# CVlab315/Domain-Adaptative-Hand-Pose-Estimation

Measured on AMD Instinct MI355X. Metric: images/sec (unique source+target images per A+B+C training iteration, 2*B*N/t_iter), higher is better.
Workload: dtype bf16; 1 GPU; RHD->H3D domain-adaptation iteration (steps A+B+C), resnet50 + 3-deconv neck + main head + 3 adversarial multiscale-fusion heads, 256x256, batch 64 source + 64 target per GPU, random init, synthetic batches; arch=resnet50, image_size=256, per_gpu_batch=64, global_batch=64, parallelism=dp1, hip_graphs=True, gradient_exchange=none (one rank)

## Files before the change

domain-adaptative-hand-pose-estimation_amd/csrc/bn.hip:

```cpp
#include "common.h"
#include "fp8_common.h"
#include <stdlib.h>
#include <string>

struct BnPlan { int cpr, TX, TY, colgroups, nslices, rows_per_slice; };

static BnPlan bn_plan(long rows, int C, int CH, long slice_cap_override = 0) {
  BnPlan p; p.cpr = C / CH;
  p.TX = p.cpr < 256 ? p.cpr : 256;
  while (256 % p.TX) --p.TX;
  p.TY = 256 / p.TX;
  p.colgroups = cdiv(p.cpr, p.TX);
  long want = rows / ((long)p.TY * 8); if (want < 1) want = 1;
  static const long slice_cap = getenv("MI355_BN_SLICES") ? atol(getenv("MI355_BN_SLICES")) : 1024;
  long cap = (slice_cap_override ? slice_cap_override : slice_cap) / p.colgroups; if (cap < 1) cap = 1;
  if (want > cap) want = cap;
  long rps = (rows + want - 1) / want; rps = ((rps + p.TY - 1) / p.TY) * p.TY;
  p.rows_per_slice = (int)rps; p.nslices = (int)((rows + rps - 1) / rps);
  return p;
}

static long bwd_slices() { static const long v = getenv("MI355_BN_BWD_SLICES") ? atol(getenv("MI355_BN_BWD_SLICES")) : 768; return v; }
extern "C" size_t mi355_bn_workspace(long rows, int C) {
  int ns = 0;
// ... 96 lines not shown
  }
  if (running_mean && repeats > 0) running_mean[c] = rm;
  if (running_var && repeats > 0) running_var[c] = rv;
  const float sc = g * invstd;
  scale_shift[c] = sc; scale_shift[C + c] = b - mean * sc;
}

__global__ __launch_bounds__(256) void bn_finalize_wide_kernel(const float* __restrict__ partial, int nslices, int C, const float* __restrict__ gamma,
                                        const float* __restrict__ beta, float* running_mean, float* running_var,
                                        int64_t* nbt, float* save_mean, float* save_invstd, float* scale_shift, float eps,
                                        float momentum, int repeats) {
  __shared__ float red[4][3];
  const int c = blockIdx.x, t = threadIdx.x, lane = t & 63, wave = t >> 6;
  if (c == 0 && t == 0 && nbt) *nbt += repeats;
  const float g = gamma[c], b = beta[c];
  float rm = running_mean ? running_mean[c] : 0.f, rv = running_var ? running_var[c] : 0.f;
  float n = 0.f, mean = 0.f, m2 = 0.f;
  for (int base = 0; base < nslices; base += 2048) {
    float qn[8], qm[8], qv[8];
#pragma unroll
    for (int j = 0; j < 8; ++j) {
      const int s = base + t + 256 * j;
      if (s < nslices) { const float* q = partial + ((size_t)s * C + c) * 3; qn[j] = q[0]; qm[j] = q[1]; qv[j] = q[2]; }
      else { qn[j] = 0.f; qm[j] = 0.f; qv[j] = 0.f; }
    }
#pragma unroll
    for (int j = 0; j < 8; ++j) chan_combine(n, mean, m2, qn[j], qm[j], qv[j]);
  }
#pragma unroll
  for (int o = 32; o > 0; o >>= 1) {
    const float nb = __shfl_down(n, o, 64), mb = __shfl_down(mean, o, 64), vb = __shfl_down(m2, o, 64);
    chan_combine(n, mean, m2, nb, mb, vb);
  }
  if (lane == 0) { red[wave][0] = n; red[wave][1] = mean; red[wave][2] = m2; }
  __syncthreads();
  if (t != 0) return;
  n = red[0][0]; mean = red[0][1]; m2 = red[0][2];
#pragma unroll
  for (int w = 1; w < 4; ++w) chan_combine(n, mean, m2, red[w][0], red[w][1], red[w][2]);
  const float var = m2 / n;
  const float invstd = 1.0f / sqrtf(var + eps);
  save_mean[c] = mean; save_invstd[c] = invstd;
  const float uvar = n > 1.f ? m2 / (n - 1.f) : var;
  for (int r = 0; r < repeats; ++r) {
    rm = (1.f - momentum) * rm + momentum * mean;
    rv = (1.f - momentum) * rv + momentum * uvar;
  }
  if (running_mean && repeats > 0) running_mean[c] = rm;
  if (running_var && repeats > 0) running_var[c] = rv;
  const float sc = g * invstd;
  scale_shift[c] = sc; scale_shift[C + c] = b - mean * sc;
}

template <typename T, bool EVAL, bool Q8 = false>
__global__ __launch_bounds__(256) void bn_apply_kernel(const T* __restrict__ x, const T* __restrict__ res, T* __restrict__ y,
                                                        const float* __restrict__ scale_shift, const float* __restrict__ gamma,
                                                        const float* __restrict__ beta, const float* __restrict__ rm,
                                                        const float* __restrict__ rv, float eps, long rows, int C, int TX, int relu,
                                                        unsigned char* __restrict__ mask, unsigned char* __restrict__ q8 = nullptr,
                                                        float* __restrict__ q8_state = nullptr) {
  constexpr int CH = Chunk<T>::N;
  static_assert(!Q8 || CH == 8, "fp8 side output: bf16 activations only");
  const int TY = 256 / TX;
  const int tx = threadIdx.x % TX, ty = threadIdx.x / TX;
  const int chunk = blockIdx.x * TX + tx;
  const bool colok = chunk * CH < C;
  if (!colok && !Q8) return;
  const int cpr = C / CH;
  float sc[CH], sh[CH];
#pragma unroll
  for (int e = 0; e < CH; ++e) {
    const int c = chunk * CH + e;
    if (!colok) { sc[e] = 0.f; sh[e] = 0.f; }
    else if (EVAL) { sc[e] = gamma[c] / sqrtf(rv[c] + eps); sh[e] = beta[c] - rm[c] * sc[e]; }
    else { sc[e] = scale_shift[c]; sh[e] = scale_shift[C + c]; }
  }
  float qscale = 0.f, amax = 0.f; unsigned seen = 0;
  if constexpr (Q8) { qscale = q8_state[0]; seen = fp8_amax_seen(q8_state); }
  for (long r = (long)blockIdx.y * TY + ty; colok && r < rows; r += (long)gridDim.y * TY) {
    const size_t off = (size_t)r * C + (size_t)chunk * CH;
    float v[CH]; Chunk<T>::load(x + off, v);
#pragma unroll
    for (int e = 0; e < CH; ++e) v[e] = v[e] * sc[e] + sh[e];
    if (res) { float w[CH]; Chunk<T>::load(res + off, w);
#pragma unroll
      for (int e = 0; e < CH; ++e) v[e] += w[e]; }
    if (mask) {
      unsigned m = 0;
#pragma unroll
      for (int e = 0; e < CH; ++e) m |= (v[e] > 0.f ? 1u : 0u) << e;
      mask[(size_t)r * cpr + chunk] = (unsigned char)m;
    }
    if (relu) {
#pragma unroll
      for (int e = 0; e < CH; ++e) v[e] = v[e] < 0.f ? 0.f : v[e]; }
    Chunk<T>::store(y + off, v);
    if constexpr (Q8) {
      float w[8];
#pragma unroll
      for (int e = 0; e < 8; ++e) { w[e] = (float)(T)v[e]; amax = fmaxf(amax, fabsf(w[e])); }
      const uint2 o = pack8_fp8<false>(w, qscale);
      const unsigned nx = __shfl_down(o.x, 1, 64), ny = __shfl_down(o.y, 1, 64);
      if ((tx & 1) == 0) *reinterpret_cast<uint4*>(q8 + off) = make_uint4(o.x, o.y, nx, ny);
    }
  }
  if constexpr (Q8) fp8_record_amax(amax, q8_state, seen);
}

template <typename T, bool XHAT, int RELU>
__global__ __launch_bounds__(256) void bn_bwd_reduce_kernel(const T* __restrict__ dy, const T* __restrict__ x, const T* __restrict__ y,
                                                             const float* __restrict__ mean, const float* __restrict__ invstd,
                                                             const float* __restrict__ gamma, const float* __restrict__ beta,
                                                             float* __restrict__ partial, long rows, int C, int TX, int rows_per_slice,
                                                             const unsigned char* __restrict__ mask) {
  constexpr int relu = RELU;
  constexpr int CH = Chunk<T>::N;
  __shared__ float sh[256 * CH * 2];
  const int cpr = C / CH;
  const int TY = 256 / TX;
  const int tx = threadIdx.x % TX, ty = threadIdx.x / TX;
  const int chunk = blockIdx.x * TX + tx;
  const bool colok = chunk * CH < C;
  const long r0 = (long)blockIdx.y * rows_per_slice;
  long r1 = r0 + rows_per_slice; if (r1 > rows) r1 = rows;
  float s1[CH], s2[CH], mu[CH], is[CH], sc[CH], sft[CH];
#pragma unroll
  for (int e = 0; e < CH; ++e) { s1[e] = 0.f; s2[e] = 0.f; mu[e] = 0.f; is[e] = 0.f; sc[e] = 0.f; sft[e] = 0.f; }
  if (colok && XHAT) {
#pragma unroll
    for (int e = 0; e < CH; ++e) { mu[e] = mean[chunk * CH + e]; is[e] = invstd[chunk * CH + e]; }
    if (relu == 2) {
#pragma unroll
      for (int e = 0; e < CH; ++e) { sc[e] = gamma[chunk * CH + e] * is[e]; sft[e] = beta[chunk * CH + e] - mu[e] * sc[e]; }
    }
  }
  auto fold = [&](float (&g)[CH], const float (&v)[CH], const float (&o)[CH], unsigned mb) {
    if (relu == 1) {
#pragma unroll
      for (int e = 0; e < CH; ++e) g[e] = o[e] > 0.f ? g[e] : 0.f; }
    else if (relu == 3) {
#pragma unroll
      for (int e = 0; e < CH; ++e) g[e] = ((mb >> e) & 1u) ? g[e] : 0.f; }
    if (XHAT) {
      if (relu == 2) {
#pragma unroll
        for (int e = 0; e < CH; ++e) g[e] = (v[e] * sc[e] + sft[e]) > 0.f ? g[e] : 0.f; }
#pragma unroll
      for (int e = 0; e < CH; ++e) { s1[e] += g[e]; s2[e] += g[e] * ((v[e] - mu[e]) * is[e]); }
    } else {
#pragma unroll
      for (int e = 0; e < CH; ++e) s1[e] += g[e];
    }
  };
  if (colok) {
    long r = r0 + ty;
    for (; r + TY < r1; r += 2 * TY) {
      const size_t off0 = (size_t)r * C + (size_t)chunk * CH, off1 = off0 + (size_t)TY * C;
      float g0[CH], v0[CH], o0[CH], g1[CH], v1[CH], o1[CH];
      Chunk<T>::load(dy + off0, g0); Chunk<T>::load(dy + off1, g1);
      if (XHAT) { Chunk<T>::load(x + off0, v0); Chunk<T>::load(x + off1, v1); }
      if (relu == 1) { Chunk<T>::load(y + off0, o0); Chunk<T>::load(y + off1, o1); }
      unsigned m0 = 0, m1 = 0;
      if (relu == 3) { m0 = mask[(size_t)r * cpr + chunk]; m1 = mask[(size_t)(r + TY) * cpr + chunk]; }
      fold(g0, v0, o0, m0); fold(g1, v1, o1, m1);
    }
    if (r < r1) {
      const size_t off = (size_t)r * C + (size_t)chunk * CH;
      float g[CH], v[CH], o[CH]; Chunk<T>::load(dy + off, g);
      if (XHAT) Chunk<T>::load(x + off, v);
      if (relu == 1) Chunk<T>::load(y + off, o);
      fold(g, v, o, relu == 3 ? (unsigned)mask[(size_t)r * cpr + chunk] : 0u);
    }
  }
#pragma unroll
  for (int e = 0; e < CH; ++e) { sh[threadIdx.x * CH + e] = s1[e]; sh[256 * CH + threadIdx.x * CH + e] = s2[e]; }
  __syncthreads();
  if (ty == 0 && colok) {
    for (int j = 1; j < TY; ++j) {
      const int o = j * TX + tx;
#pragma unroll
      for (int e = 0; e < CH; ++e) { s1[e] += sh[o * CH + e]; s2[e] += sh[256 * CH + o * CH + e]; }
    }
    float* out = partial + ((size_t)blockIdx.y * C + (size_t)chunk * CH) * 2;
#pragma unroll
    for (int e = 0; e < CH; ++e) { out[e * 2] = s1[e]; out[e * 2 + 1] = s2[e]; }
  }
}

__global__ __launch_bounds__(256) void bn_bwd_finalize_kernel(const float* __restrict__ partial, int nslices, int C, float inv_rows,
                                       const float* __restrict__ gamma, const float* __restrict__ invstd, float* dgamma,
                                       float* dbeta, int accumulate, float* coeff) {
  const int lane = threadIdx.x & 63;
  const int c = blockIdx.x * 4 + (threadIdx.x >> 6);
  if (c >= C) return;
  const float g = coeff ? gamma[c] : 0.f, is = coeff ? invstd[c] : 0.f;
  const float db0 = (accumulate && dbeta) ? dbeta[c] : 0.f, dg0 = (accumulate && dgamma) ? dgamma[c] : 0.f;
  float s1 = 0.f, s2 = 0.f;
  for (int base = 0; base < nslices; base += 1024) {
    float q1[16], q2[16];
#pragma unroll
    for (int j = 0; j < 16; ++j) {
      const int s = base + lane + 64 * j;
      if (s < nslices) { const float* q = partial + ((size_t)s * C + c) * 2; q1[j] = q[0]; q2[j] = q[1]; } else { q1[j] = 0.f; q2[j] = 0.f; }
    }
#pragma unroll
    for (int j = 0; j < 16; ++j) { s1 += q1[j]; s2 += q2[j]; }
  }
#pragma unroll
  for (int o = 32; o > 0; o >>= 1) { s1 += __shfl_down(s1, o, 64); s2 += __shfl_down(s2, o, 64); }
  if (lane != 0) return;
  if (dbeta) dbeta[c] = db0 + s1;
  if (dgamma) dgamma[c] = dg0 + s2;
  if (coeff) { coeff[c] = g * is; coeff[C + c] = s1 * inv_rows; coeff[2 * C + c] = s2 * inv_rows; }
}

template <typename T, int RELU, bool Q8 = false>
__global__ __launch_bounds__(256) void bn_bwd_apply_kernel(const T* __restrict__ dy, const T* __restrict__ x, const T* __restrict__ y,
                                                            const float* __restrict__ mean, const float* __restrict__ invstd,
                                                            const float* __restrict__ coeff, const float* __restrict__ beta,
                                                            T* __restrict__ dx, T* __restrict__ dres,
                                                            long rows, int C, int TX, const unsigned char* __restrict__ mask,
                                                            unsigned char* __restrict__ q8 = nullptr, float* __restrict__ q8_state = nullptr) {
  constexpr int CH = Chunk<T>::N;
  constexpr int relu = RELU;
  static_assert(!Q8 || CH == 8, "fp8 side output: bf16 gradients only");
  const int TY = 256 / TX;
  const int tx = threadIdx.x % TX, ty = threadIdx.x / TX;
  const int chunk = blockIdx.x * TX + tx;
  const bool colok = chunk * CH < C;
  if (!colok && !Q8) return;
  const int cpr = C / CH;
  float k0[CH], k1[CH], k2[CH], mu[CH], is[CH], sh[CH];
#pragma unroll
  for (int e = 0; e < CH; ++e) {
    const int c = colok ? chunk * CH + e : 0;
    k0[e] = coeff[c]; k1[e] = coeff[C + c]; k2[e] = coeff[2 * C + c]; mu[e] = mean[c]; is[e] = invstd[c];
    sh[e] = (relu == 2) ? beta[c] - mu[e] * k0[e] : 0.f;
  }
  float qscale = 0.f, amax = 0.f; unsigned seen = 0;
  if constexpr (Q8) { qscale = q8_state[0]; seen = fp8_amax_seen(q8_state); }
  auto finish = [&](size_t off, float (&g)[CH], float (&v)[CH], const float (&o)[CH], unsigned mb) {
    if (relu == 1) {
#pragma unroll
      for (int e = 0; e < CH; ++e) g[e] = o[e] > 0.f ? g[e] : 0.f; }
    else if (relu == 3) {
#pragma unroll
      for (int e = 0; e < CH; ++e) g[e] = ((mb >> e) & 1u) ? g[e] : 0.f; }
    else if (relu == 2) {
#pragma unroll
      for (int e = 0; e < CH; ++e) g[e] = (v[e] * k0[e] + sh[e]) > 0.f ? g[e] : 0.f; }
    if (dres) Chunk<T>::store(dres + off, g);
#pragma unroll
    for (int e = 0; e < CH; ++e) v[e] = k0[e] * (g[e] - k1[e] - (v[e] - mu[e]) * is[e] * k2[e]);
    Chunk<T>::store(dx + off, v);
    if constexpr (Q8) {
      float w[8];
#pragma unroll
      for (int e = 0; e < 8; ++e) { w[e] = (float)(T)v[e]; amax = fmaxf(amax, fabsf(w[e])); }
      const uint2 o = pack8_fp8<true>(w, qscale);
      const unsigned nx = __shfl_down(o.x, 1, 64), ny = __shfl_down(o.y, 1, 64);
      if ((tx & 1) == 0) *reinterpret_cast<uint4*>(q8 + off) = make_uint4(o.x, o.y, nx, ny);
    }
  };
  const long stride = (long)gridDim.y * TY;
  long r = colok ? (long)blockIdx.y * TY + ty : rows;
  for (; r + stride < rows; r += 2 * stride) {
    const size_t off0 = (size_t)r * C + (size_t)chunk * CH, off1 = (size_t)(r + stride) * C + (size_t)chunk * CH;
    float g0[CH], v0[CH], o0[CH], g1[CH], v1[CH], o1[CH];
    Chunk<T>::load(dy + off0, g0); Chunk<T>::load(x + off0, v0);
    Chunk<T>::load(dy + off1, g1); Chunk<T>::load(x + off1, v1);
    if (relu == 1) { Chunk<T>::load(y + off0, o0); Chunk<T>::load(y + off1, o1); }
    unsigned m0 = 0, m1 = 0;
    if (relu == 3) { m0 = mask[(size_t)r * cpr + chunk]; m1 = mask[(size_t)(r + stride) * cpr + chunk]; }
    finish(off0, g0, v0, o0, m0); finish(off1, g1, v1, o1, m1);
  }
  if (r < rows) {
    const size_t off = (size_t)r * C + (size_t)chunk * CH;
    float g[CH], v[CH], o[CH]; Chunk<T>::load(dy + off, g); Chunk<T>::load(x + off, v);
    if (relu == 1) Chunk<T>::load(y + off, o);
    finish(off, g, v, o, relu == 3 ? (unsigned)mask[(size_t)r * cpr + chunk] : 0u);
  }
  if constexpr (Q8) fp8_record_amax(amax, q8_state, seen);
}

struct BnResArgs {
  const void* dy; const void* x; const float* mean; const float* invstd; const float* gamma; const float* beta;
  void* dx; void* dres; float* dgamma; float* dbeta; const unsigned char* mask;
  long rows; int C, G, R, rpb, keep, accumulate; float inv_rows;
  unsigned spin_limit;
};
#define BN_RES_MAXBLK 256
#define BN_RES_GRAN 128
#define BN_RES_SW 8
#define BN_RES_KR 0
#define BN_RES_NT 1024
__device__ unsigned long long bn_res_gran[BN_RES_MAXBLK * BN_RES_GRAN];
__device__ unsigned bn_res_done[2][BN_RES_MAXBLK + 1];
__device__ unsigned bn_res_err[4];
static_assert(BN_RES_MAXBLK == 256, "a launch adds 256 to its completion count and the tag keeps 8 bits of n - 1");

#ifdef BN_RES_STAMPS
__device__ unsigned long long bn_res_stamp[BN_RES_MAXBLK * 8];
#define BN_STAMP(k) do { __builtin_amdgcn_sched_barrier(0); if (t == 0) bn_res_stamp[blockIdx.x * 8 + (k)] = wall_clock64(); \
                         __builtin_amdgcn_sched_barrier(0); } while (0)
extern "C" int mi355_bn_resident_stamps(unsigned long long* out) {
  return hipMemcpyFromSymbol(out, HIP_SYMBOL(bn_res_stamp), sizeof(unsigned long long) * BN_RES_MAXBLK * 8) == hipSuccess ? MI355_OK : MI355_ELAUNCH;
}
#else
#define BN_STAMP(k) do {} while (0)
#endif

template <typename T, int RELU, int KR, int NT>
__global__ __launch_bounds__(NT) void bn_bwd_resident_kernel(BnResArgs p) {
  constexpr int CH = Chunk<T>::N, GC = 8 * CH, RL = NT / 8, NW = NT / 64, NL = NT / (GC * 2), RR = KR * RL;
  extern __shared__ __attribute__((aligned(16))) char smem[];
  const int t = threadIdx.x, tx = t & 7, ty = t >> 3, lane = t & 63, wave = t >> 6;
  const int g = blockIdx.x % p.G, r = blockIdx.x / p.G;
  const long row0 = (long)r * p.rpb;
  long row1 = row0 + p.rpb; if (row1 > p.rows) row1 = p.rows;
  const int nrows = row1 > row0 ? (int)(row1 - row0) : 0;
  const int keep = p.keep;
  uint4* xs = reinterpret_cast<uint4*>(smem);
  uint4* ds = xs + (size_t)keep * 8;
  float* red = reinterpret_cast<float*>(ds + (size_t)keep * 8);
  float* grp = red + NW * GC * 2;
  float* tot = grp + NL * GC * 2;
  int* bar_ok = reinterpret_cast<int*>(tot + GC * 2);
  const T* __restrict__ X = reinterpret_cast<const T*>(p.x);
  const T* __restrict__ DY = reinterpret_cast<const T*>(p.dy);
  const int C = p.C, cpr = C / CH, c0 = g * GC + tx * CH, chunk = c0 / CH;
  BN_STAMP(0);
  const unsigned nblk = (unsigned)(p.G * p.R);
  unsigned* done = &bn_res_done[GC * 2 == BN_RES_GRAN ? 1 : 0][nblk];
  const unsigned tag = 0x80000000u | (GC * 2 == BN_RES_GRAN ? 0x40000000u : 0u) | ((nblk - 1u) << 22) |
                       ((__hip_atomic_load(done, __ATOMIC_RELAXED, __HIP_MEMORY_SCOPE_AGENT) >> 8) & 0x3fffffu);
  float mu[CH], is[CH], sc[CH], sft[CH], s1[CH], s2[CH];
#pragma unroll
  for (int e = 0; e < CH; ++e) {
    mu[e] = p.mean[c0 + e]; is[e] = p.invstd[c0 + e]; s1[e] = 0.f; s2[e] = 0.f;
    sc[e] = p.gamma[c0 + e] * is[e];
    sft[e] = (RELU == 2) ? p.beta[c0 + e] - mu[e] * sc[e] : 0.f;
  }
  auto mask_of = [&](int lr) -> unsigned { return (RELU == 3) ? (unsigned)p.mask[(size_t)(row0 + lr) * cpr + chunk] : 0u; };
  auto fold = [&](const uint4& qxv, const uint4& qdv, unsigned mb) {
    float v[CH], gq[CH]; Chunk<T>::unpack(qxv, v); Chunk<T>::unpack(qdv, gq);
#pragma unroll
    for (int e = 0; e < CH; ++e) {
      if (RELU == 2) gq[e] = (v[e] * sc[e] + sft[e]) > 0.f ? gq[e] : 0.f;
      if (RELU == 3) gq[e] = ((mb >> e) & 1u) ? gq[e] : 0.f;
      s1[e] += gq[e]; s2[e] += gq[e] * ((v[e] - mu[e]) * is[e]);
    }
  };
  uint4 rx[KR > 0 ? KR : 1], rd[KR > 0 ? KR : 1];
  {
    unsigned mk[KR > 0 ? KR : 1];
#pragma unroll
    for (int k = 0; k < KR; ++k) {
      const int lr = ty + k * RL;
      rx[k] = make_uint4(0, 0, 0, 0); rd[k] = make_uint4(0, 0, 0, 0); mk[k] = 0;
      if (lr < nrows) {
        const size_t off = (size_t)(row0 + lr) * C + c0;
        rx[k] = *reinterpret_cast<const uint4*>(X + off); rd[k] = *reinterpret_cast<const uint4*>(DY + off); mk[k] = mask_of(lr);
      }
    }
#pragma unroll
    for (int k = 0; k < KR; ++k)
      if (ty + k * RL < nrows) fold(rx[k], rd[k], mk[k]);
  }
  for (int base = RR + ty; base < nrows; base += 4 * RL) {
    uint4 qx[4], qd[4]; unsigned mk[4];
#pragma unroll
    for (int k = 0; k < 4; ++k) {
      const int lr = base + k * RL;
      if (lr < nrows) {
        const size_t off = (size_t)(row0 + lr) * C + c0;
        qx[k] = *reinterpret_cast<const uint4*>(X + off); qd[k] = *reinterpret_cast<const uint4*>(DY + off); mk[k] = mask_of(lr);
      }
    }
#pragma unroll
    for (int k = 0; k < 4; ++k) {
      const int lr = base + k * RL, li = lr - RR;
      if (lr < nrows) {
        if (li < keep) { xs[li * 8 + tx] = qx[k]; ds[li * 8 + tx] = qd[k]; }
        fold(qx[k], qd[k], mk[k]);
      }
    }
  }
#pragma unroll
  for (int o = 8; o < 64; o <<= 1) {
#pragma unroll
    for (int e = 0; e < CH; ++e) { s1[e] += __shfl_xor(s1[e], o, 64); s2[e] += __shfl_xor(s2[e], o, 64); }
  }
  if (lane < 8) {
#pragma unroll
    for (int e = 0; e < CH; ++e) { red[(wave * GC + tx * CH + e) * 2] = s1[e]; red[(wave * GC + tx * CH + e) * 2 + 1] = s2[e]; }
  }
  if (t == 0) *bar_ok = 1;
  BN_STAMP(1);
  __syncthreads();
  if (t < GC * 2) {
    float a = 0.f;
#pragma unroll
    for (int w = 0; w < NW; ++w) a += red[w * GC * 2 + t];
    __hip_atomic_store(bn_res_gran + (size_t)blockIdx.x * BN_RES_GRAN + t, ((unsigned long long)tag << 32) | __float_as_uint(a),
                       __ATOMIC_RELAXED, __HIP_MEMORY_SCOPE_AGENT);
  }
  BN_STAMP(2);
  {
    const int i = t % (GC * 2), s = t / (GC * 2);
    const __amdgpu_buffer_rsrc_t rs = __builtin_amdgcn_make_buffer_rsrc(bn_res_gran, 0, (unsigned)sizeof(bn_res_gran), 0x00020000);
    float a = 0.f;
    bool arrived = true;
    for (int rr0 = s; rr0 < p.R && arrived; rr0 += BN_RES_SW * NL) {
      float q[BN_RES_SW];
      for (unsigned spins = 0;;) {
        asm volatile("" ::: "memory");
        bool ok = true;
#pragma unroll
        for (int k = 0; k < BN_RES_SW; ++k) {
          const int rr = rr0 + k * NL;
          const auto gv = __builtin_amdgcn_raw_buffer_load_b64(rs, rr < p.R ? ((rr * p.G + g) * BN_RES_GRAN + i) * 8 : 0x7ffffff0, 0, 16);
          q[k] = rr < p.R ? __uint_as_float(gv[0]) : 0.f; ok &= (gv[1] == tag) | (rr >= p.R);
        }
        if (__all(ok)) break;
        if (++spins > p.spin_limit) { arrived = false; break; }
        __builtin_amdgcn_s_sleep(4);
      }
#pragma unroll
      for (int k = 0; k < BN_RES_SW; ++k) a += q[k];
    }
    grp[s * GC * 2 + i] = a;
    if (!arrived && lane == 0) *bar_ok = 0;
  }
  __syncthreads();
  const bool exchanged = *bar_ok != 0;
  if (!exchanged && t == 0) __hip_atomic_fetch_add(bn_res_err, 1u, __ATOMIC_RELAXED, __HIP_MEMORY_SCOPE_AGENT);
  if (t < GC * 2) {
    float a = 0.f;
#pragma unroll
    for (int s = 0; s < NL; ++s) a += grp[s * GC * 2 + t];
    tot[t] = a;
  }
  __syncthreads();
  BN_STAMP(3);
  float k1[CH], k2[CH];
#pragma unroll
  for (int e = 0; e < CH; ++e) {
    s1[e] = tot[(tx * CH + e) * 2]; s2[e] = tot[(tx * CH + e) * 2 + 1];
    if (!exchanged) { s1[e] = __builtin_nanf(""); s2[e] = __builtin_nanf(""); }
    k1[e] = s1[e] * p.inv_rows; k2[e] = s2[e] * p.inv_rows;
  }
  if (r == 0 && ty == 0) {
#pragma unroll
    for (int e = 0; e < CH; ++e) {
      if (p.dbeta) p.dbeta[c0 + e] = (p.accumulate ? p.dbeta[c0 + e] : 0.f) + s1[e];
      if (p.dgamma) p.dgamma[c0 + e] = (p.accumulate ? p.dgamma[c0 + e] : 0.f) + s2[e];
    }
  }
  T* __restrict__ DX = reinterpret_cast<T*>(p.dx);
  T* __restrict__ DR = reinterpret_cast<T*>(p.dres);
#ifdef BN_RES_STAMPS
  bool stamped = false;
#endif
  auto finish = [&](int lr, const uint4& qxv, const uint4& qdv, unsigned mb) {
    const size_t off = (size_t)(row0 + lr) * C + c0;
    float v[CH], gq[CH]; Chunk<T>::unpack(qxv, v); Chunk<T>::unpack(qdv, gq);
#pragma unroll
    for (int e = 0; e < CH; ++e) {
      if (RELU == 2) gq[e] = (v[e] * sc[e] + sft[e]) > 0.f ? gq[e] : 0.f;
      if (RELU == 3) gq[e] = ((mb >> e) & 1u) ? gq[e] : 0.f;
    }
    if (DR) Chunk<T>::store(DR + off, gq);
#pragma unroll
    for (int e = 0; e < CH; ++e) v[e] = sc[e] * (gq[e] - k1[e] - (v[e] - mu[e]) * is[e] * k2[e]);
    Chunk<T>::store(DX + off, v);
#ifdef BN_RES_STAMPS
    if (!stamped) { BN_STAMP(4); stamped = true; }
#endif
  };
#pragma unroll
  for (int k = 0; k < KR; ++k) {
    const int lr = ty + k * RL;
    if (lr < nrows) finish(lr, rx[k], rd[k], mask_of(lr));
  }
  const int nlds = nrows - RR < keep ? nrows - RR : keep;
  for (int li = ty; li < nlds; li += RL) finish(RR + li, xs[li * 8 + tx], ds[li * 8 + tx], mask_of(RR + li));
  for (int base = RR + keep + ty; base < nrows; base += 4 * RL) {
    uint4 qx[4], qd[4]; unsigned mk[4];
#pragma unroll
    for (int k = 0; k < 4; ++k) {
      const int lr = base + k * RL;
      if (lr < nrows) {
        const size_t off = (size_t)(row0 + lr) * C + c0;
        qx[k] = *reinterpret_cast<const uint4*>(X + off); qd[k] = *reinterpret_cast<const uint4*>(DY + off); mk[k] = mask_of(lr);
      }
    }
#pragma unroll
    for (int k = 0; k < 4; ++k) {
      const int lr = base + k * RL;
      if (lr < nrows) finish(lr, qx[k], qd[k], mk[k]);
    }
  }
  if (t == 0) __hip_atomic_fetch_add(done, blockIdx.x == 0 ? (unsigned)BN_RES_MAXBLK + 1u - nblk : 1u, __ATOMIC_RELAXED, __HIP_MEMORY_SCOPE_AGENT);
  BN_STAMP(5);
}

template <typename T>
__global__ __launch_bounds__(256) void apply_relu_mask_kernel(T* __restrict__ g, const unsigned char* __restrict__ mask, size_t nchunks) {
  constexpr int CH = Chunk<T>::N;
  for (size_t i = (size_t)blockIdx.x * 256 + threadIdx.x; i < nchunks; i += (size_t)gridDim.x * 256) {
    float v[CH]; Chunk<T>::load(g + i * CH, v);
    const unsigned mb = mask[i];
#pragma unroll
    for (int e = 0; e < CH; ++e) v[e] = ((mb >> e) & 1u) ? v[e] : 0.f;
    Chunk<T>::store(g + i * CH, v);
  }
}

template <typename T>
__global__ __launch_bounds__(256) void bn_relu_maxpool_kernel(const T* __restrict__ x, const float* __restrict__ scale_shift, T* __restrict__ y,
                                                               uint8_t* __restrict__ arg, int N, int H, int W, int C, int Ho, int Wo) {
  constexpr int CH = Chunk<T>::N;
  const int cpr = C / CH;
  const unsigned total = (unsigned)N * Ho * Wo * cpr;
  for (unsigned id = blockIdx.x * 256u + threadIdx.x; id < total; id += gridDim.x * 256u) {
    const int ch = (int)(id % (unsigned)cpr); unsigned r = id / (unsigned)cpr;
    const int ox = (int)(r % (unsigned)Wo); r /= (unsigned)Wo; const int oy = (int)(r % (unsigned)Ho); const int n = (int)(r / (unsigned)Ho);
    float sc[CH], sh[CH], best[CH]; int bi[CH]; bool first = true;
#pragma unroll
    for (int e = 0; e < CH; ++e) { sc[e] = scale_shift[ch * CH + e]; sh[e] = scale_shift[C + ch * CH + e]; best[e] = -INFINITY; bi[e] = 0; }
    for (int kh = 0; kh < 3; ++kh) {
      const int iy = 2 * oy - 1 + kh; if (iy < 0 || iy >= H) continue;
      for (int kw = 0; kw < 3; ++kw) {
        const int ix = 2 * ox - 1 + kw; if (ix < 0 || ix >= W) continue;
        float v[CH]; Chunk<T>::load(x + (((size_t)n * H + iy) * W + ix) * C + (size_t)ch * CH, v);
        const int code = kh * 3 + kw;
#pragma unroll
        for (int e = 0; e < CH; ++e) {
          float u = v[e] * sc[e] + sh[e];
          u = u < 0.f ? 0.f : u;
          u = (float)(T)u;
          if (first) bi[e] = code;
          if (u > best[e] || u != u) { best[e] = u; bi[e] = code; }
        }
        first = false;
      }
    }
    const size_t o = (((size_t)n * Ho + oy) * Wo + ox) * C + (size_t)ch * CH;
    Chunk<T>::store(y + o, best);
    store_bytes<CH>(arg + o, bi);
  }
// ... 20 lines not shown
  return 0;
}
static int bn_check(long rows, int C, int dtype, int* CH) {
  if (dtype != MI355_F32 && dtype != MI355_BF16) MI_FAIL(MI355_EINVAL, "bn: bad dtype");
  *CH = dtype == MI355_BF16 ? 8 : 4;
  if (rows < 1 || C < 1 || C % *CH) MI_FAIL(MI355_EINVAL, "bn: C=%d must be a positive multiple of %d (rows=%ld)", C, *CH, rows);
  return 0;
}
static dim3 apply_grid(const BnPlan& p, long rows, bool backward = false) {
  long gy = rows / ((long)p.TY * 4); if (gy < 1) gy = 1;
  static const long fwd_cap = getenv("MI355_BN_APPLY_CAP") ? atol(getenv("MI355_BN_APPLY_CAP")) : 2048;
  static const long bwd_cap = getenv("MI355_BN_BWD_CAP") ? atol(getenv("MI355_BN_BWD_CAP")) : 1024;
  long cap = (backward ? bwd_cap : fwd_cap) / p.colgroups; if (cap < 1) cap = 1;
  if (gy > cap) gy = cap;
  return dim3(p.colgroups, (unsigned)gy);
}

extern "C" int mi355_bn_train_fwd(const void* x, const void* residual, void* y, const float* gamma, const float* beta,
                                  float* running_mean, float* running_var, int64_t* nbt, float* save_mean, float* save_invstd,
                                  long rows, int C, float eps, float momentum, int stat_updates, int relu, int dtype, void* ws,
                                  size_t ws_bytes, void* relu_mask, void* q8_out, float* q8_state, void* stream) {
  int CH; if (int e = bn_check(rows, C, dtype, &CH)) return e;
  if (int e = q8_check(q8_out, q8_state, dtype, C)) return e;
  unsigned char* mk = reinterpret_cast<unsigned char*>(relu_mask);
  if (stat_updates < 0 || stat_updates > 8) MI_FAIL(MI355_EINVAL, "bn_train_fwd: stat_updates=%d", stat_updates);
  if (!ws || ws_bytes < mi355_bn_workspace(rows, C)) MI_FAIL(MI355_EWORKSPACE, "bn_train_fwd: workspace too small");
  hipStream_t st = as_stream(stream);
  BnPlan p = bn_plan(rows, C, CH);
  float* partial = reinterpret_cast<float*>(ws);
  float* ss = partial + (size_t)p.nslices * C * 3;
  dim3 g(p.colgroups, p.nslices);
  const double nb = (double)rows * C * (dtype == MI355_BF16 ? 2.0 : 4.0);
  char lab[96];
  if (prof_on()) snprintf(lab, sizeof(lab), "rows%ld C%d%s%s", rows, C, relu ? " relu" : "", residual ? " +res" : "");
  {
    ProfScope ps(st, 0.0, nb, 1, prof_on() ? (std::string("bn_stats ") + lab).c_str() : nullptr);
    if (dtype == MI355_BF16) hipLaunchKernelGGL(bn_stats_kernel<bf16_t>, g, dim3(256), 0, st, (const bf16_t*)x, partial, rows, C, p.TX, p.rows_per_slice);
    else hipLaunchKernelGGL(bn_stats_kernel<float>, g, dim3(256), 0, st, (const float*)x, partial, rows, C, p.TX, p.rows_per_slice);
  }
  {
    ProfScope ps(st, 0.0, 12.0 * p.nslices * C, 1, prof_on() ? (std::string("bn_finalize ") + lab).c_str() : nullptr);
    hipLaunchKernelGGL(bn_finalize_kernel, dim3(cdiv(C, 4)), dim3(256), 0, st, partial, p.nslices, C, gamma, beta, running_mean, running_var, nbt, save_mean, save_invstd, ss, eps, momentum, stat_updates);
  }
  dim3 ga = apply_grid(p, rows);
  const float* nf = nullptr;
  ProfScope ps(st, 0.0, nb * (residual ? 3 : 2), 1, prof_on() ? (std::string("bn_apply ") + lab).c_str() : nullptr);
  if (q8_out) hipLaunchKernelGGL((bn_apply_kernel<bf16_t, false, true>), ga, dim3(256), 0, st, (const bf16_t*)x, (const bf16_t*)residual, (bf16_t*)y, (const float*)ss, nf, nf, nf, nf, eps, rows, C, p.TX, relu, mk, (unsigned char*)q8_out, q8_state);
  else if (dtype == MI355_BF16) hipLaunchKernelGGL((bn_apply_kernel<bf16_t, false>), ga, dim3(256), 0, st, (const bf16_t*)x, (const bf16_t*)residual, (bf16_t*)y, (const float*)ss, nf, nf, nf, nf, eps, rows, C, p.TX, relu, mk);
  else hipLaunchKernelGGL((bn_apply_kernel<float, false>), ga, dim3(256), 0, st, (const float*)x, (const float*)residual, (float*)y, (const float*)ss, nf, nf, nf, nf, eps, rows, C, p.TX, relu, mk);
  MI_CHECK_LAUNCH("bn_train_fwd");
  return MI355_OK;
}

extern "C" int mi355_bn_train_fwd_partials(const void* x, const void* residual, void* y, const float* gamma, const float* beta,
                                           float* running_mean, float* running_var, int64_t* nbt, float* save_mean,
                                           float* save_invstd, long rows, int C, float eps, float momentum, int stat_updates,
                                           int relu, int dtype, const float* partial, int nslices, float* scale_shift,
                                           void* relu_mask, void* q8_out, float* q8_state, void* stream) {
  int CH; if (int e = bn_check(rows, C, dtype, &CH)) return e;
  if (int e = q8_check(q8_out, q8_state, dtype, C)) return e;
  unsigned char* mk = reinterpret_cast<unsigned char*>(relu_mask);
  if (stat_updates < 0 || stat_updates > 8) MI_FAIL(MI355_EINVAL, "bn_train_fwd_partials: stat_updates=%d", stat_updates);
  if (!partial || nslices < 1 || !scale_shift) MI_FAIL(MI355_EINVAL, "bn_train_fwd_partials: partial / scale_shift missing");
  hipStream_t st = as_stream(stream);
  BnPlan p = bn_plan(rows, C, CH);
  static const int wide_min = getenv("MI355_BN_WIDE_FINALIZE") ? atoi(getenv("MI355_BN_WIDE_FINALIZE")) : 512;
  const double nb = (double)rows * C * (dtype == MI355_BF16 ? 2.0 : 4.0);
  char lab[96];
  if (prof_on()) snprintf(lab, sizeof(lab), "rows%ld C%d ns%d%s%s", rows, C, nslices, relu ? " relu" : "", residual ? " +res" : "");
  {
    ProfScope ps(st, 0.0, 12.0 * nslices * C, 1, prof_on() ? (std::string("bn_finalize ") + lab).c_str() : nullptr);
    if (nslices >= wide_min) hipLaunchKernelGGL(bn_finalize_wide_kernel, dim3(C), dim3(256), 0, st, partial, nslices, C, gamma, beta, running_mean, running_var, nbt, save_mean, save_invstd, scale_shift, eps, momentum, stat_updates);
    else hipLaunchKernelGGL(bn_finalize_kernel, dim3(cdiv(C, 4)), dim3(256), 0, st, partial, nslices, C, gamma, beta, running_mean, running_var, nbt, save_mean, save_invstd, scale_shift, eps, momentum, stat_updates);
  }
  dim3 ga = apply_grid(p, rows);
  const float* nf = nullptr;
  ProfScope ps(st, 0.0, nb * (residual ? 3 : 2), 1, prof_on() ? (std::string("bn_apply ") + lab).c_str() : nullptr);
  if (q8_out) hipLaunchKernelGGL((bn_apply_kernel<bf16_t, false, true>), ga, dim3(256), 0, st, (const bf16_t*)x, (const bf16_t*)residual, (bf16_t*)y, (const float*)scale_shift, nf, nf, nf, nf, eps, rows, C, p.TX, relu, mk, (unsigned char*)q8_out, q8_state);
  else if (dtype == MI355_BF16) hipLaunchKernelGGL((bn_apply_kernel<bf16_t, false>), ga, dim3(256), 0, st, (const bf16_t*)x, (const bf16_t*)residual, (bf16_t*)y, (const float*)scale_shift, nf, nf, nf, nf, eps, rows, C, p.TX, relu, mk);
  else hipLaunchKernelGGL((bn_apply_kernel<float, false>), ga, dim3(256), 0, st, (const float*)x, (const float*)residual, (float*)y, (const float*)scale_shift, nf, nf, nf, nf, eps, rows, C, p.TX, relu, mk);
  MI_CHECK_LAUNCH("bn_train_fwd_partials");
  return MI355_OK;
}

extern "C" int mi355_bn_relu_maxpool_fwd_partials(const void* x, void* y_pool, uint8_t* argidx, const float* gamma, const float* beta,
                                                  float* running_mean, float* running_var, int64_t* nbt, float* save_mean,
                                                  float* save_invstd, int N, int H, int W, int C, float eps, float momentum,
                                                  int stat_updates, int dtype, const float* partial, int nslices, float* scale_shift,
                                                  void* stream) {
  const long rows = (long)N * H * W;
  int CH; if (int e = bn_check(rows, C, dtype, &CH)) return e;
  if (stat_updates < 0 || stat_updates > 8) MI_FAIL(MI355_EINVAL, "bn_relu_maxpool_fwd_partials: stat_updates=%d", stat_updates);
  if (!partial || nslices < 1 || !scale_shift || !argidx || !y_pool) MI_FAIL(MI355_EINVAL, "bn_relu_maxpool_fwd_partials: null argument");
  if (rows * (C / CH) >= (1L << 31)) MI_FAIL(MI355_EINVAL, "bn_relu_maxpool_fwd_partials: %ld chunks exceed the kernel's 32-bit index: split the batch", rows * (C / CH));
  hipStream_t st = as_stream(stream);
  static const int wide_min = getenv("MI355_BN_WIDE_FINALIZE") ? atoi(getenv("MI355_BN_WIDE_FINALIZE")) : 512;
  char lab[96];
  if (prof_on()) snprintf(lab, sizeof(lab), "rows%ld C%d ns%d", rows, C, nslices);
  {
    ProfScope ps(st, 0.0, 12.0 * nslices * C, 1, prof_on() ? (std::string("bn_finalize ") + lab).c_str() : nullptr);
    if (nslices >= wide_min) hipLaunchKernelGGL(bn_finalize_wide_kernel, dim3(C), dim3(256), 0, st, partial, nslices, C, gamma, beta, running_mean, running_var, nbt, save_mean, save_invstd, scale_shift, eps, momentum, stat_updates);
    else hipLaunchKernelGGL(bn_finalize_kernel, dim3(cdiv(C, 4)), dim3(256), 0, st, partial, nslices, C, gamma, beta, running_mean, running_var, nbt, save_mean, save_invstd, scale_shift, eps, momentum, stat_updates);
  }
  const int Ho = (H + 2 - 3) / 2 + 1, Wo = (W + 2 - 3) / 2 + 1;
  const long total = (long)N * Ho * Wo * (C / CH);
  int grid = (int)((total + 255) / 256); if (grid > 8192) grid = 8192;
  ProfScope ps(st, 0.0, (double)rows * C * (dtype == MI355_BF16 ? 2.0 : 4.0) * 1.25, 1, prof_on() ? (std::string("bn_relu_maxpool ") + lab).c_str() : nullptr);
  if (dtype == MI355_BF16) hipLaunchKernelGGL(bn_relu_maxpool_kernel<bf16_t>, dim3(grid), dim3(256), 0, st, (const bf16_t*)x, (const float*)scale_shift, (bf16_t*)y_pool, argidx, N, H, W, C, Ho, Wo);
  else hipLaunchKernelGGL(bn_relu_maxpool_kernel<float>, dim3(grid), dim3(256), 0, st, (const float*)x, (const float*)scale_shift, (float*)y_pool, argidx, N, H, W, C, Ho, Wo);
  MI_CHECK_LAUNCH("bn_relu_maxpool_fwd_partials");
  return MI355_OK;
}

extern "C" int mi355_bn_eval_fwd(const void* x, const void* residual, void* y, const float* gamma, const float* beta,
                                 const float* running_mean, const float* running_var, long rows, int C, float eps, int relu,
                                 int dtype, void* stream) {
  int CH; if (int e = bn_check(rows, C, dtype, &CH)) return e;
  hipStream_t st = as_stream(stream);
  BnPlan p = bn_plan(rows, C, CH);
  dim3 ga = apply_grid(p, rows);
  const float* nf = nullptr;
  if (dtype == MI355_BF16) hipLaunchKernelGGL((bn_apply_kernel<bf16_t, true>), ga, dim3(256), 0, st, (const bf16_t*)x, (const bf16_t*)residual, (bf16_t*)y, nf, gamma, beta, running_mean, running_var, eps, rows, C, p.TX, relu, (unsigned char*)nullptr);
  else hipLaunchKernelGGL((bn_apply_kernel<float, true>), ga, dim3(256), 0, st, (const float*)x, (const float*)residual, (float*)y, nf, gamma, beta, running_mean, running_var, eps, rows, C, p.TX, relu, (unsigned char*)nullptr);
  MI_CHECK_LAUNCH("bn_eval_fwd");
  return MI355_OK;
}

struct BnResPlan { int G, R, rpb, keep; size_t lds, max_lds; };
static int g_bn_resident = -1;
extern "C" int mi355_bn_set_resident(int on) {
  const int prev = g_bn_resident;
  g_bn_resident = on < 0 ? -1 : (on ? 1 : 0);
  return prev;
}
static bool bn_resident_plan(long rows, int C, int CH, BnResPlan* q) {
  static const bool env_on = !(getenv("MI355_BN_RESIDENT") && atoi(getenv("MI355_BN_RESIDENT")) == 0);
  if (g_bn_resident == 0 || (g_bn_resident < 0 && !env_on)) return false;
  static int ncu = 0; static size_t max_lds = 0;
  if (!ncu) {
    int dev = 0, v = 0;
    if (hipGetDevice(&dev) != hipSuccess) return false;
    if (hipDeviceGetAttribute(&v, hipDeviceAttributeMaxSharedMemoryPerBlock, dev) != hipSuccess) return false;
    max_lds = (size_t)v;
    if (hipDeviceGetAttribute(&v, hipDeviceAttributeMultiprocessorCount, dev) != hipSuccess) return false;
    ncu = v > BN_RES_MAXBLK ? BN_RES_MAXBLK : v;
  }
  const int GC = 8 * CH;
  if (C % GC) return false;
  static const long min_bytes = getenv("MI355_BN_RESIDENT_MIN") ? atol(getenv("MI355_BN_RESIDENT_MIN")) : 0;
  if (rows * C * (16 / CH) < min_bytes) return false;
  q->G = C / GC;
  if (q->G > ncu) return false;
  long R = ncu / q->G; if (R > rows) R = rows;
  q->rpb = (int)((rows + R - 1) / R);
  q->R = (int)((rows + q->rpb - 1) / q->rpb);
  static const long max_bytes = getenv("MI355_BN_RESIDENT_MAX") ? atol(getenv("MI355_BN_RESIDENT_MAX")) : (1L << 62);
  if (rows * C * (16 / CH) > max_bytes) return false;
  const size_t scratch = (size_t)(BN_RES_NT / 64 * GC * 2 + BN_RES_NT + GC * 2 + 4) * sizeof(float);
  long keep = (long)((max_lds - scratch) / 256);
  const long reg_rows = (long)BN_RES_KR * (BN_RES_NT / 8);
  const long rest = q->rpb > reg_rows ? q->rpb - reg_rows : 0;
  if (keep > rest) keep = rest;
  q->keep = (int)keep;
  q->lds = (size_t)keep * 256 + scratch;
  q->max_lds = max_lds;
  return (size_t)q->G * q->R <= (size_t)ncu && q->G * q->R <= BN_RES_MAXBLK;
}
static unsigned g_bn_res_spin = 1u << 19;
extern "C" int mi355_bn_resident_set_spin_limit(unsigned limit) {
  g_bn_res_spin = limit ? limit : (1u << 19);
  return MI355_OK;
}
#define BN_RES_NOT_RESIDENT 1
template <typename T, int RELU>
static int bn_resident_launch(const BnResArgs& a, size_t lds, size_t max_lds, hipStream_t st) {
  static int fits = -1;
  auto kern = bn_bwd_resident_kernel<T, RELU, BN_RES_KR, BN_RES_NT>;
  if (fits < 0) {
    if (hipFuncSetAttribute(reinterpret_cast<const void*>(kern), hipFuncAttributeMaxDynamicSharedMemorySize, (int)max_lds) != hipSuccess)
      MI_FAIL(MI355_ELAUNCH, "bn_bwd: cannot raise the dynamic LDS limit to %zu bytes", max_lds);
    int nb = 0;
    if (hipOccupancyMaxActiveBlocksPerMultiprocessor(&nb, kern, BN_RES_NT, max_lds) != hipSuccess) nb = 0;
    fits = nb >= 1 ? 1 : 0;
  }
  if (!fits) return BN_RES_NOT_RESIDENT;
  hipLaunchKernelGGL(kern, dim3(a.G * a.R), dim3(BN_RES_NT), lds, st, a);
  return MI355_OK;
}
extern "C" int mi355_bn_resident_timeouts(unsigned* out) {
  unsigned v[4] = {0, 0, 0, 0};
  if (!out) MI_FAIL(MI355_EINVAL, "bn_resident_timeouts: out is null");
  if (hipMemcpyFromSymbol(v, HIP_SYMBOL(bn_res_err), sizeof(v)) != hipSuccess) MI_FAIL(MI355_ELAUNCH, "bn_resident_timeouts: copy failed");
  *out = v[0];
  return MI355_OK;
}
extern "C" int mi355_bn_resident_reset(void) {
  static const unsigned zdone[2][BN_RES_MAXBLK + 1] = {{0}};
  static const unsigned zerr[4] = {0, 0, 0, 0};
  void* gran = nullptr;
  if (hipDeviceSynchronize() != hipSuccess) MI_FAIL(MI355_ELAUNCH, "bn_resident_reset: device synchronize failed");
  if (hipGetSymbolAddress(&gran, HIP_SYMBOL(bn_res_gran)) != hipSuccess || hipMemset(gran, 0, sizeof(bn_res_gran)) != hipSuccess ||
      hipMemcpyToSymbol(HIP_SYMBOL(bn_res_done), zdone, sizeof(zdone)) != hipSuccess ||
      hipMemcpyToSymbol(HIP_SYMBOL(bn_res_err), zerr, sizeof(zerr)) != hipSuccess) MI_FAIL(MI355_ELAUNCH, "bn_resident_reset: copy failed");
  if (hipDeviceSynchronize() != hipSuccess) MI_FAIL(MI355_ELAUNCH, "bn_resident_reset: device synchronize failed");
  return MI355_OK;
}

static void launch_bwd_apply(int dtype, int relu, dim3 ga, hipStream_t st, const void* dy, const void* x, const void* y, const float* save_mean,
                             const float* save_invstd, const float* coeff, const float* beta, void* dx, void* dresidual, long rows, int C,
                             int TX, const unsigned char* mk, void* q8_out, float* q8_state) {
#define MI_APP(T, R) hipLaunchKernelGGL((bn_bwd_apply_kernel<T, R>), ga, dim3(256), 0, st, (const T*)dy, (const T*)x, (const T*)y, save_mean, save_invstd, coeff, beta, (T*)dx, (T*)dresidual, rows, C, TX, mk)
#define MI_APQ(R) hipLaunchKernelGGL((bn_bwd_apply_kernel<bf16_t, R, true>), ga, dim3(256), 0, st, (const bf16_t*)dy, (const bf16_t*)x, (const bf16_t*)y, save_mean, save_invstd, coeff, beta, (bf16_t*)dx, (bf16_t*)dresidual, rows, C, TX, mk, (unsigned char*)q8_out, q8_state)
#define MI_APP4(T) do { if (relu == 0) MI_APP(T, 0); else if (relu == 1) MI_APP(T, 1); else if (relu == 2) MI_APP(T, 2); else MI_APP(T, 3); } while (0)
  if (q8_out) { if (relu == 0) MI_APQ(0); else if (relu == 1) MI_APQ(1); else if (relu == 2) MI_APQ(2); else MI_APQ(3); }
  else if (dtype == MI355_BF16) MI_APP4(bf16_t); else MI_APP4(float);
#undef MI_APP4
#undef MI_APQ
#undef MI_APP
}

extern "C" int mi355_bn_bwd(const void* dy, const void* x, const void* y, const float* gamma, const float* beta, const float* save_mean,
                            const float* save_invstd, void* dx, void* dresidual, float* dgamma, float* dbeta, int accumulate,
                            long rows, int C, int relu, int dtype, void* ws, size_t ws_bytes, const void* relu_mask, void* q8_out,
                            float* q8_state, void* stream) {
  int CH; if (int e = bn_check(rows, C, dtype, &CH)) return e;
  if (!ws || ws_bytes < mi355_bn_workspace(rows, C)) MI_FAIL(MI355_EWORKSPACE, "bn_bwd: workspace too small");
  const unsigned char* mk = reinterpret_cast<const unsigned char*>(relu_mask);
  if (relu) relu = mk ? 3 : (y ? 1 : 2);
  if (relu == 2 && !beta) MI_FAIL(MI355_EINVAL, "bn_bwd: relu without y needs beta");
  hipStream_t st = as_stream(stream);
  BnResPlan rp;
  if (relu != 1 && !q8_out && bn_resident_plan(rows, C, CH, &rp)) {
    BnResArgs a;
    a.dy = dy; a.x = x; a.mean = save_mean; a.invstd = save_invstd; a.gamma = gamma; a.beta = beta; a.dx = dx; a.dres = dresidual;
    a.dgamma = dgamma; a.dbeta = dbeta; a.mask = mk; a.rows = rows; a.C = C;
    a.G = rp.G; a.R = rp.R; a.rpb = rp.rpb; a.keep = rp.keep; a.accumulate = accumulate; a.inv_rows = 1.0f / (float)rows;
    a.spin_limit = g_bn_res_spin;
    int e;
    char lab[112];
    if (prof_on()) snprintf(lab, sizeof(lab), "bn_bwd_res rows%ld C%d relu%d%s keep%d/%d", rows, C, relu, dresidual ? " +dres" : "", rp.keep, rp.rpb);
    ProfScope ps(st, 0.0, (double)rows * C * (dtype == MI355_BF16 ? 2.0 : 4.0) * (dresidual ? 4 : 3), 1, prof_on() ? lab : nullptr);
    if (dtype == MI355_BF16) e = relu == 0 ? bn_resident_launch<bf16_t, 0>(a, rp.lds, rp.max_lds, st) : relu == 2 ? bn_resident_launch<bf16_t, 2>(a, rp.lds, rp.max_lds, st) : bn_resident_launch<bf16_t, 3>(a, rp.lds, rp.max_lds, st);
    else e = relu == 0 ? bn_resident_launch<float, 0>(a, rp.lds, rp.max_lds, st) : relu == 2 ? bn_resident_launch<float, 2>(a, rp.lds, rp.max_lds, st) : bn_resident_launch<float, 3>(a, rp.lds, rp.max_lds, st);
    if (e == MI355_OK) { MI_CHECK_LAUNCH("bn_bwd (resident)"); return MI355_OK; }
    if (e != BN_RES_NOT_RESIDENT) return e;
  }
  BnPlan p = bn_plan(rows, C, CH, bwd_slices());
  float* partial = reinterpret_cast<float*>(ws);
  float* coeff = partial + (size_t)p.nslices * C * 3;
  dim3 g(p.colgroups, p.nslices);
#define MI_RED(T, R) hipLaunchKernelGGL((bn_bwd_reduce_kernel<T, true, R>), g, dim3(256), 0, st, (const T*)dy, (const T*)x, (const T*)y, save_mean, save_invstd, gamma, beta, partial, rows, C, p.TX, p.rows_per_slice, mk)
#define MI_RED4(T) do { if (relu == 0) MI_RED(T, 0); else if (relu == 1) MI_RED(T, 1); else if (relu == 2) MI_RED(T, 2); else MI_RED(T, 3); } while (0)
  const double nb = (double)rows * C * (dtype == MI355_BF16 ? 2.0 : 4.0);
  char lab[96];
  if (prof_on()) snprintf(lab, sizeof(lab), "rows%ld C%d relu%d%s", rows, C, relu, dresidual ? " +dres" : "");
  {
    ProfScope ps(st, 0.0, nb * 2, 1, prof_on() ? (std::string("bn_bwd_reduce ") + lab).c_str() : nullptr);
    if (dtype == MI355_BF16) MI_RED4(bf16_t); else MI_RED4(float);
  }
#undef MI_RED4
#undef MI_RED
  {
    ProfScope ps(st, 0.0, 12.0 * p.nslices * C, 1, prof_on() ? (std::string("bn_bwd_finalize ") + lab).c_str() : nullptr);
    hipLaunchKernelGGL(bn_bwd_finalize_kernel, dim3(cdiv(C, 4)), dim3(256), 0, st, partial, p.nslices, C, 1.0f / (float)rows, gamma, save_invstd, dgamma, dbeta, accumulate, coeff);
  }
  dim3 ga = apply_grid(p, rows, true);
  if (int e = q8_check(q8_out, q8_state, dtype, C)) return e;
  ProfScope ps(st, 0.0, nb * (dresidual ? 4 : 3), 1, prof_on() ? (std::string("bn_bwd_apply ") + lab).c_str() : nullptr);
  launch_bwd_apply(dtype, relu, ga, st, dy, x, y, save_mean, save_invstd, coeff, beta, dx, dresidual, rows, C, p.TX, mk, q8_out, q8_state);
  MI_CHECK_LAUNCH("bn_bwd");
  return MI355_OK;
}

extern "C" int mi355_bn_bwd_partials(const void* dy, const void* x, const void* y, const float* gamma, const float* beta,
                                     const float* save_mean, const float* save_invstd, void* dx, void* dresidual, float* dgamma,
                                     float* dbeta, int accumulate, long rows, int C, int relu, int dtype, const float* partial,
                                     int nslices, float* coeff, const void* relu_mask, void* q8_out, float* q8_state, void* stream) {
  int CH; if (int e = bn_check(rows, C, dtype, &CH)) return e;
  if (!partial || nslices < 1 || !coeff) MI_FAIL(MI355_EINVAL, "bn_bwd_partials: partial / coeff missing");
  const unsigned char* mk = reinterpret_cast<const unsigned char*>(relu_mask);
  if (relu) relu = mk ? 3 : (y ? 1 : 2);
  if (relu == 2 && !beta) MI_FAIL(MI355_EINVAL, "bn_bwd_partials: relu without y needs beta");
  hipStream_t st = as_stream(stream);
  BnPlan p = bn_plan(rows, C, CH);
  hipLaunchKernelGGL(bn_bwd_finalize_kernel, dim3(cdiv(C, 4)), dim3(256), 0, st, partial, nslices, C, 1.0f / (float)rows, gamma, save_invstd, dgamma, dbeta, accumulate, coeff);
  dim3 ga = apply_grid(p, rows, true);
  if (int e = q8_check(q8_out, q8_state, dtype, C)) return e;
  launch_bwd_apply(dtype, relu, ga, st, dy, x, y, save_mean, save_invstd, coeff, beta, dx, dresidual, rows, C, p.TX, mk, q8_out, q8_state);
  MI_CHECK_LAUNCH("bn_bwd_partials");
  return MI355_OK;
}

extern "C" int mi355_apply_relu_mask(void* g, const void* relu_mask, long rows, int C, int dtype, void* stream) {
  int CH; if (int e = bn_check(rows, C, dtype, &CH)) return e;
  if (!g || !relu_mask) MI_FAIL(MI355_EINVAL, "apply_relu_mask: null pointer");
  const size_t nchunks = (size_t)rows * (C / CH);
  long grid = (long)((nchunks + 255) / 256); if (grid > 4096) grid = 4096;
  if (dtype == MI355_BF16) hipLaunchKernelGGL(apply_relu_mask_kernel<bf16_t>, dim3((unsigned)grid), dim3(256), 0, as_stream(stream), (bf16_t*)g, (const unsigned char*)relu_mask, nchunks);
  else hipLaunchKernelGGL(apply_relu_mask_kernel<float>, dim3((unsigned)grid), dim3(256), 0, as_stream(stream), (float*)g, (const unsigned char*)relu_mask, nchunks);
  MI_CHECK_LAUNCH("apply_relu_mask");
  return MI355_OK;
}

extern "C" int mi355_colsum(const void* dy, float* out, long rows, int C, int dtype, int accumulate, void* ws, size_t ws_bytes,
                            void* stream) {
  int CH; if (int e = bn_check(rows, C, dtype, &CH)) return e;
  if (!ws || ws_bytes < mi355_colsum_workspace(rows, C)) MI_FAIL(MI355_EWORKSPACE, "colsum: workspace too small");
  hipStream_t st = as_stream(stream);
  BnPlan p = bn_plan(rows, C, CH);
  float* partial = reinterpret_cast<float*>(ws);
  dim3 g(p.colgroups, p.nslices);
  if (dtype == MI355_BF16) hipLaunchKernelGGL((bn_bwd_reduce_kernel<bf16_t, false, 0>), g, dim3(256), 0, st, (const bf16_t*)dy, (const bf16_t*)nullptr, (const bf16_t*)nullptr, (const float*)nullptr, (const float*)nullptr, (const float*)nullptr, (const float*)nullptr, partial, rows, C, p.TX, p.rows_per_slice, (const unsigned char*)nullptr);
  else hipLaunchKernelGGL((bn_bwd_reduce_kernel<float, false, 0>), g, dim3(256), 0, st, (const float*)dy, (const float*)nullptr, (const float*)nullptr, (const float*)nullptr, (const float*)nullptr, (const float*)nullptr, (const float*)nullptr, partial, rows, C, p.TX, p.rows_per_slice, (const unsigned char*)nullptr);
  hipLaunchKernelGGL(colsum_finalize_kernel, dim3(cdiv(C, 4)), dim3(256), 0, st, partial, p.nslices, C, out, accumulate);
  MI_CHECK_LAUNCH("colsum");
  return MI355_OK;
}
```

domain-adaptative-hand-pose-estimation_amd/csrc/common.h:

```cpp
#pragma once
#include <stdint.h>
#include <stdio.h>
#include <string.h>
#include "../../include/mi355pose.h"

static inline int cdiv(long a, long b) { return (int)((a + b - 1) / b); }
static inline int ilog2_exact(int v) { int s = 0; while ((1 << s) < v) ++s; return ((1 << s) == v) ? s : -1; }

#ifdef __HIP__
#include <hip/hip_runtime.h>

typedef __bf16 bf16_t;
typedef __attribute__((ext_vector_type(8))) short bf16x8_t;
typedef __attribute__((ext_vector_type(4))) short bf16x4_t;
typedef __attribute__((ext_vector_type(16))) float f32x16_t;
typedef __attribute__((ext_vector_type(4))) float f32x4_t;

#define WAVE 64

void mi355_set_error(const char* fmt, ...);
#define MI_FAIL(code, ...) do { mi355_set_error(__VA_ARGS__); return (code); } while (0)
#define MI_CHECK_LAUNCH(name) do { hipError_t e_ = hipGetLastError(); \
  if (e_ != hipSuccess) MI_FAIL(MI355_ELAUNCH, "%s: %s", (name), hipGetErrorString(e_)); } while (0)

static inline hipStream_t as_stream(void* s) { return (hipStream_t)s; }

template <typename T> struct Elem;
template <> struct Elem<float> {
  static constexpr int kPerChunk = 4;
  __device__ static inline float ld(const float* p) { return *p; }
  __device__ static inline void st(float* p, float v) { *p = v; }
};
template <> struct Elem<bf16_t> {
  static constexpr int kPerChunk = 8;
  __device__ static inline float ld(const bf16_t* p) { return (float)*p; }
  __device__ static inline void st(bf16_t* p, float v) { *p = (bf16_t)v; }
};

__device__ inline float bf16_bits_to_f32(unsigned short b) { return __uint_as_float(((unsigned)b) << 16); }

template <typename T> struct Chunk;
template <> struct Chunk<float> {
  static constexpr int N = 4;
  __device__ static inline void load(const float* p, float (&v)[4]) {
    float4 q = *reinterpret_cast<const float4*>(p); v[0] = q.x; v[1] = q.y; v[2] = q.z; v[3] = q.w; }
  __device__ static inline void store(float* p, const float (&v)[4]) {
    *reinterpret_cast<float4*>(p) = make_float4(v[0], v[1], v[2], v[3]); }
  __device__ static inline void unpack(const uint4& q, float (&v)[4]) {
    v[0] = __uint_as_float(q.x); v[1] = __uint_as_float(q.y); v[2] = __uint_as_float(q.z); v[3] = __uint_as_float(q.w); }
};
template <> struct Chunk<bf16_t> {
  static constexpr int N = 8;
  __device__ static inline void unpack(const uint4& q, float (&v)[8]) {
    unsigned w[4] = {q.x, q.y, q.z, q.w};
#pragma unroll
    for (int i = 0; i < 4; ++i) { v[2 * i] = __uint_as_float(w[i] << 16); v[2 * i + 1] = __uint_as_float(w[i] & 0xffff0000u); }
  }
  __device__ static inline void load(const bf16_t* p, float (&v)[8]) { unpack(*reinterpret_cast<const uint4*>(p), v); }
  __device__ static inline void store(bf16_t* p, const float (&v)[8]) {
    union { bf16_t h[8]; uint4 q; } u;
#pragma unroll
    for (int i = 0; i < 8; ++i) u.h[i] = (bf16_t)v[i];
    *reinterpret_cast<uint4*>(p) = u.q;
  }
};

template <int CH> __device__ inline void load_bytes(const uint8_t* p, unsigned (&b)[CH]) {
  if constexpr (CH == 8) {
    const uint2 q = *reinterpret_cast<const uint2*>(p);
#pragma unroll
    for (int e = 0; e < 4; ++e) { b[e] = (q.x >> (8 * e)) & 0xffu; b[4 + e] = (q.y >> (8 * e)) & 0xffu; }
  } else {
    const unsigned q = *reinterpret_cast<const unsigned*>(p);
#pragma unroll
    for (int e = 0; e < 4; ++e) b[e] = (q >> (8 * e)) & 0xffu;
  }
}
template <int CH> __device__ inline void store_bytes(uint8_t* p, const int (&b)[CH]) {
  if constexpr (CH == 8) {
    uint2 q; q.x = 0u; q.y = 0u;
#pragma unroll
    for (int e = 0; e < 4; ++e) { q.x |= ((unsigned)b[e] & 0xffu) << (8 * e); q.y |= ((unsigned)b[4 + e] & 0xffu) << (8 * e); }
    *reinterpret_cast<uint2*>(p) = q;
  } else {
    unsigned q = 0u;
#pragma unroll
    for (int e = 0; e < 4; ++e) q |= ((unsigned)b[e] & 0xffu) << (8 * e);
    *reinterpret_cast<unsigned*>(p) = q;
  }
}

__device__ inline float wave_sum(float v) {
#pragma unroll
  for (int o = 32; o > 0; o >>= 1) v += __shfl_xor(v, o, 64);
  return v;
}
__device__ inline float wave_max(float v) {
#pragma unroll
  for (int o = 32; o > 0; o >>= 1) v = fmaxf(v, __shfl_xor(v, o, 64));
  return v;
}
template <int NW> __device__ inline float block_sum(float v, float* red) {
  v = wave_sum(v);
  __syncthreads();
  if ((threadIdx.x & 63) == 0) red[threadIdx.x >> 6] = v;
  __syncthreads();
  float r = 0.f;
#pragma unroll
  for (int i = 0; i < NW; ++i) r += red[i];
  return r;
}
template <int NW> __device__ inline float block_max(float v, float* red) {
  v = wave_max(v);
  __syncthreads();
  if ((threadIdx.x & 63) == 0) red[threadIdx.x >> 6] = v;
  __syncthreads();
  float r = red[0];
#pragma unroll
  for (int i = 1; i < NW; ++i) r = fmaxf(r, red[i]);
  return r;
}

struct FastDiv {
  unsigned mul, shr, d;
};
static inline FastDiv make_fastdiv(unsigned d) {
  FastDiv f; f.d = d;
  if (d == 1) { f.mul = 0; f.shr = 0; return f; }
  unsigned l = 0; while ((1ull << l) < d) ++l;
  unsigned long long m = ((1ull << 32) * ((1ull << l) - d)) / d + 1;
  f.mul = (unsigned)m; f.shr = l; return f;
}
__device__ inline unsigned fd_div(unsigned n, const FastDiv& f) {
  if (f.d == 1) return n;
  unsigned t = __umulhi(n, f.mul);
  return (t + ((n - t) >> 1)) >> (f.shr - 1);
}

struct ProfScope {
  hipStream_t s; bool on; int slot;
  ProfScope(hipStream_t st, double flops, double bytes = 0.0, int family = 0, const char* label = nullptr);
  ~ProfScope();
};
bool prof_on();
void prof_set_tag(const char* fmt, ...);
void prof_amend_label(const char* fmt, ...);
#endif
```

domain-adaptative-hand-pose-estimation_amd/csrc/pool_layout.hip:

```cpp
#include "common.h"

template <typename T>
__global__ __launch_bounds__(256) void maxpool_fwd_kernel(const T* __restrict__ x, T* __restrict__ y, uint8_t* __restrict__ arg,
                                                           int N, int H, int W, int C, int Ho, int Wo) {
  constexpr int CH = Chunk<T>::N;
  const int cpr = C / CH;
  const unsigned total = (unsigned)N * Ho * Wo * cpr;
  for (unsigned id = blockIdx.x * 256u + threadIdx.x; id < total; id += gridDim.x * 256u) {
    const int ch = (int)(id % (unsigned)cpr); unsigned r = id / (unsigned)cpr;
    const int ox = (int)(r % (unsigned)Wo); r /= (unsigned)Wo; const int oy = (int)(r % (unsigned)Ho); const int n = (int)(r / (unsigned)Ho);
    float best[CH]; int bi[CH]; bool first = true;
#pragma unroll
    for (int e = 0; e < CH; ++e) { best[e] = -INFINITY; bi[e] = 0; }
    for (int kh = 0; kh < 3; ++kh) {
      const int iy = 2 * oy - 1 + kh; if (iy < 0 || iy >= H) continue;
      for (int kw = 0; kw < 3; ++kw) {
        const int ix = 2 * ox - 1 + kw; if (ix < 0 || ix >= W) continue;
        float v[CH]; Chunk<T>::load(x + (((size_t)n * H + iy) * W + ix) * C + (size_t)ch * CH, v);
        const int code = kh * 3 + kw;
#pragma unroll
        for (int e = 0; e < CH; ++e) {
          if (first) bi[e] = code;
          if (v[e] > best[e] || v[e] != v[e]) { best[e] = v[e]; bi[e] = code; }
        }
        first = false;
      }
    }
    const size_t o = (((size_t)n * Ho + oy) * Wo + ox) * C + (size_t)ch * CH;
    Chunk<T>::store(y + o, best);
    store_bytes<CH>(arg + o, bi);
  }
}

template <typename T>
__global__ __launch_bounds__(256) void maxpool_bwd_kernel(const T* __restrict__ dy, const uint8_t* __restrict__ arg, T* __restrict__ dx,
                                                           int N, int H, int W, int C, int Ho, int Wo) {
  constexpr int CH = Chunk<T>::N;
  const int cpr = C / CH;
  const unsigned total = (unsigned)N * H * W * cpr;
  for (unsigned id = blockIdx.x * 256u + threadIdx.x; id < total; id += gridDim.x * 256u) {
    const int ch = (int)(id % (unsigned)cpr); unsigned r = id / (unsigned)cpr;
    const int ix = (int)(r % (unsigned)W); r /= (unsigned)W; const int iy = (int)(r % (unsigned)H); const int n = (int)(r / (unsigned)H);
    float g[CH];
#pragma unroll
    for (int e = 0; e < CH; ++e) g[e] = 0.f;
    const int oy0 = iy >> 1, ox0 = ix >> 1;
    const int khs[2] = {iy - 2 * oy0 + 1, 0}, kws[2] = {ix - 2 * ox0 + 1, 0};
    const bool vy[2] = {oy0 < Ho, (iy & 1) && oy0 + 1 < Ho}, vx[2] = {ox0 < Wo, (ix & 1) && ox0 + 1 < Wo};
#pragma unroll
    for (int a = 0; a < 2; ++a)
#pragma unroll
      for (int b = 0; b < 2; ++b) {
        if (vy[a] && vx[b]) {
          const size_t o = (((size_t)n * Ho + oy0 + a) * Wo + ox0 + b) * C + (size_t)ch * CH;
          float d[CH]; Chunk<T>::load(dy + o, d);
          unsigned ab[CH]; load_bytes<CH>(arg + o, ab);
          const unsigned code = (unsigned)(khs[a] * 3 + kws[b]);
#pragma unroll
          for (int e = 0; e < CH; ++e) if (ab[e] == code) g[e] += d[e];
        }
      }
    Chunk<T>::store(dx + (((size_t)n * H + iy) * W + ix) * C + (size_t)ch * CH, g);
  }
}

extern "C" int mi355_maxpool_fwd(const void* x, void* y, uint8_t* argidx, int N, int H, int W, int C, int dtype, void* stream) {
  const int CH = dtype == MI355_BF16 ? 8 : 4;
  if (C % CH || N < 1 || !argidx) MI_FAIL(MI355_EINVAL, "maxpool_fwd: bad args (C=%d)", C);
  if ((long)N * H * W * (C / CH) >= (1L << 31)) MI_FAIL(MI355_EINVAL, "maxpool_fwd: %ld chunks exceed the kernel's 32-bit index: split the batch", (long)N * H * W * (C / CH));
  const int Ho = (H + 2 - 3) / 2 + 1, Wo = (W + 2 - 3) / 2 + 1;
  long total = (long)N * Ho * Wo * (C / CH);
  int grid = (int)((total + 255) / 256); if (grid > 8192) grid = 8192;
  if (dtype == MI355_BF16) hipLaunchKernelGGL(maxpool_fwd_kernel<bf16_t>, dim3(grid), dim3(256), 0, as_stream(stream), (const bf16_t*)x, (bf16_t*)y, argidx, N, H, W, C, Ho, Wo);
  else hipLaunchKernelGGL(maxpool_fwd_kernel<float>, dim3(grid), dim3(256), 0, as_stream(stream), (const float*)x, (float*)y, argidx, N, H, W, C, Ho, Wo);
  MI_CHECK_LAUNCH("maxpool_fwd");
  return MI355_OK;
}

extern "C" int mi355_maxpool_bwd(const void* dy, const uint8_t* argidx, void* dx, int N, int H, int W, int C, int dtype, void* stream) {
  const int CH = dtype == MI355_BF16 ? 8 : 4;
  if (C % CH || N < 1 || !argidx) MI_FAIL(MI355_EINVAL, "maxpool_bwd: bad args (C=%d)", C);
  if ((long)N * H * W * (C / CH) >= (1L << 31)) MI_FAIL(MI355_EINVAL, "maxpool_bwd: %ld chunks exceed the kernel's 32-bit index: split the batch", (long)N * H * W * (C / CH));
  const int Ho = (H + 2 - 3) / 2 + 1, Wo = (W + 2 - 3) / 2 + 1;
  long total = (long)N * H * W * (C / CH);
  int grid = (int)((total + 255) / 256); if (grid > 8192) grid = 8192;
  if (dtype == MI355_BF16) hipLaunchKernelGGL(maxpool_bwd_kernel<bf16_t>, dim3(grid), dim3(256), 0, as_stream(stream), (const bf16_t*)dy, argidx, (bf16_t*)dx, N, H, W, C, Ho, Wo);
  else hipLaunchKernelGGL(maxpool_bwd_kernel<float>, dim3(grid), dim3(256), 0, as_stream(stream), (const float*)dy, argidx, (float*)dx, N, H, W, C, Ho, Wo);
  MI_CHECK_LAUNCH("maxpool_bwd");
  return MI355_OK;
}

template <typename T>
__global__ __launch_bounds__(256) void nchw_to_nhwc_kernel(const float* __restrict__ x, T* __restrict__ y, int N, int C, int HW, int Cpad) {
  constexpr int CH = Chunk<T>::N;
  const int cpr = Cpad / CH;
  const long total = (long)N * HW * cpr;
  for (long id = (long)blockIdx.x * 256 + threadIdx.x; id < total; id += (long)gridDim.x * 256) {
    const int p = (int)(id % HW); long r = id / HW; const int ch = (int)(r % cpr); const int n = (int)(r / cpr);
    float v[CH];
#pragma unroll
    for (int e = 0; e < CH; ++e) { const int c = ch * CH + e; v[e] = c < C ? x[((size_t)n * C + c) * HW + p] : 0.f; }
    Chunk<T>::store(y + ((size_t)n * HW + p) * Cpad + (size_t)ch * CH, v);
  }
}

template <typename T>
__global__ __launch_bounds__(256) void nhwc_to_nchw_kernel(const T* __restrict__ x, float* __restrict__ y, int N, int C, int HW) {
  __shared__ float tile[32][33];
  const int n = blockIdx.z, p0 = blockIdx.x * 32, c0 = blockIdx.y * 32;
  const int tx = threadIdx.x & 31, ty = threadIdx.x >> 5;
  for (int r = ty; r < 32; r += 8) {
    const int p = p0 + r, c = c0 + tx;
    tile[r][tx] = (p < HW && c < C) ? Elem<T>::ld(x + ((size_t)n * HW + p) * C + c) : 0.f;
  }
  __syncthreads();
// ... 99 lines not shown
```

domain-adaptative-hand-pose-estimation_amd/mi355/__init__.py:

```python
import ctypes
import os
import threading

import torch

F32, BF16, FP8 = 0, 1, 2
_HERE = os.path.dirname(os.path.abspath(__file__))
LIB_PATH = os.environ.get('MI355_LIB') or os.path.join(os.path.dirname(_HERE), 'libmi355pose.so')

_lib = None
_lock = threading.Lock()


class Mi355Error(RuntimeError):
    pass


class ConvDesc(ctypes.Structure):
    _fields_ = [(n, ctypes.c_int) for n in
                ('N', 'Hi', 'Wi', 'Ci', 'Ho', 'Wo', 'Co', 'kh', 'kw', 'stride', 'pad', 'dtype')]


class WgradItem(ctypes.Structure):
    _fields_ = [('d', ConvDesc), ('x', ctypes.c_void_p), ('dy', ctypes.c_void_p), ('dw', ctypes.c_void_p),
                ('accumulate', ctypes.c_int), ('pad_', ctypes.c_int)]


class BnBwdSrc(ctypes.Structure):
    _fields_ = [('x', ctypes.c_void_p), ('y', ctypes.c_void_p), ('gamma', ctypes.c_void_p), ('beta', ctypes.c_void_p),
                ('save_mean', ctypes.c_void_p), ('save_invstd', ctypes.c_void_p), ('relu', ctypes.c_int)]


_P, _I, _L, _F, _Z = ctypes.c_void_p, ctypes.c_int, ctypes.c_long, ctypes.c_float, ctypes.c_size_t
_D = ctypes.POINTER(ConvDesc)
SIGNATURES = {
    'mi355_version': (_I, []),
    'mi355_last_error': (ctypes.c_char_p, []),
    'mi355_conv_fwd': (_I, [_D, _P, _P, _P, _P, _P, _P]),
    'mi355_conv_dgrad': (_I, [_D, _P, _P, _P, _P, _I, _P, _P]),
    'mi355_conv_stats_bytes': (_Z, [_L, _I]),
    'mi355_conv_fwd_stats': (_I, [_D, _P, _P, _P, _P, _P, _Z, _P, _P]),
    'mi355_conv_dgrad_stats': (_I, [_D, _P, _P, _P, _P, _Z, _P, _P]),
    'mi355_conv_fwd_cat': (_I, [_D, _P, _P, _P, _P, _P, _P, _I, _P, _P, _Z, _P, _P]),
    'mi355_conv_dgrad_bnbwd': (_I, [_D, _P, _P, _P, _I, _P, _P, _P, _Z, _P, _P]),
    'mi355_conv_fwd_bnbwd': (_I, [_D, _P, _P, _P, _P, _P, _Z, _P, _P]),
    'mi355_fp8_quantize': (_I, [_P, _P, _P, _L, _I, _I, _I, _P]),
    'mi355_fp8_update_scale': (_I, [_P, _I, _I, _I, _I, _P]),
    'mi355_pack_weights_fp8': (_I, [_P, _P, _P, _P, _I, _I, _I, _I, _P]),
    'mi355_pack_weights_fp8_batched': (_I, [_P, _I, _I, _P]),
    'mi355_conv_fwd_fp8': (_I, [_D, _P, _I, _P, _P, _P, _P, _P, _P, _P, _Z, _P, _P]),
    'mi355_conv_dgrad_fp8': (_I, [_D, _P, _I, _P, _P, _P, _P, _I, _P, _P, _Z, _P, _P]),
    'mi355_mx_quantize': (_I, [_P, _P, _P, _L, _I, _I, _P]),
    'mi355_pack_weights_mx': (_I, [_P, _P, _P, _P, _P, _I, _I, _I, _P]),
    'mi355_pack_weights_mx_batched': (_I, [_P, _I, _I, _P]),
    'mi355_conv_fwd_mx': (_I, [_D, _P, _P, _P, _P, _P, _P, _P, _P, _Z, _P, _P]),
    'mi355_conv_dgrad_mx': (_I, [_D, _P, _P, _P, _P, _P, _I, _P, _P, _Z, _P, _P]),
    'mi355_conv_fwd_mx_act': (_I, [_D, _P, _P, _P, _P, _P, _P, _I, _P, _P, _P, _P]),
    'mi355_conv_dgrad_mx_act': (_I, [_D, _P, _P, _P, _P, _P, _I, _P, _P, _P, _P]),
    'mi355_conv_wgrad_workspace': (_Z, [_D]),
    'mi355_conv_wgrad_fp8_workspace': (_Z, [_D]),
    'mi355_conv_wgrad_fp8': (_I, [_D, _P, _I, _P, _I, _P, _P, _P, _I, _P, _Z, _P]),
    'mi355_conv_wgrad': (_I, [_D, _P, _P, _P, _I, _P, _Z, _P]),
    'mi355_conv_wgrad_grouped_workspace': (_Z, [_P, _I]),
    'mi355_conv_wgrad_grouped': (_I, [_P, _I, _P, _Z, _P]),
    'mi355_pack_weights': (_I, [_P, _P, _P, _I, _I, _I, _I, _I, _P]),
    'mi355_pack_weights_batched': (_I, [_P, _I, _I, _I, _P]),
    'mi355_colsum_workspace': (_Z, [_L, _I]),
    'mi355_colsum': (_I, [_P, _P, _L, _I, _I, _I, _P, _Z, _P]),
    'mi355_bn_workspace': (_Z, [_L, _I]),
    'mi355_bn_train_fwd': (_I, [_P, _P, _P, _P, _P, _P, _P, _P, _P, _P, _L, _I, _F, _F, _I, _I, _I, _P, _Z, _P, _P, _P, _P]),
    'mi355_bn_train_fwd_partials': (_I, [_P, _P, _P, _P, _P, _P, _P, _P, _P, _P, _L, _I, _F, _F, _I, _I, _I, _P, _I, _P, _P, _P, _P, _P]),
    'mi355_bn_eval_fwd': (_I, [_P, _P, _P, _P, _P, _P, _P, _L, _I, _F, _I, _I, _P]),
    'mi355_bn_bwd_partials': (_I, [_P, _P, _P, _P, _P, _P, _P, _P, _P, _P, _P, _I, _L, _I, _I, _I, _P, _I, _P, _P, _P, _P, _P]),
    'mi355_bn_bwd': (_I, [_P, _P, _P, _P, _P, _P, _P, _P, _P, _P, _P, _I, _L, _I, _I, _I, _P, _Z, _P, _P, _P, _P]),
    'mi355_bn_resident_timeouts': (_I, [_P]),
    'mi355_bn_resident_reset': (_I, []),
    'mi355_bn_resident_set_spin_limit': (_I, [ctypes.c_uint]),
    'mi355_bn_set_resident': (_I, [_I]),
    'mi355_set_pgemm': (_I, [_I]),
    'mi355_set_fp8_kw3': (_L, [_L]),
    'mi355_apply_relu_mask': (_I, [_P, _P, _L, _I, _I, _P]),
    'mi355_conv_dgrad_masked_acc': (_I, [_P, _P, _P, _P, _P, _P, _P]),
    'mi355_conv_fwd_act': (_I, [_P, _P, _P, _P, _P, _I, _P, _P]),
    'mi355_conv_dgrad_act': (_I, [_P, _P, _P, _P, _I, _P, _P]),
    'mi355_bn_relu_maxpool_fwd_partials': (_I, [_P, _P, _P, _P, _P, _P, _P, _P, _P, _P, _I, _I, _I, _I, _F, _F, _I, _I, _P, _I, _P, _P]),
    'mi355_maxpool_fwd': (_I, [_P, _P, _P, _I, _I, _I, _I, _I, _P]),
    'mi355_maxpool_bwd': (_I, [_P, _P, _P, _I, _I, _I, _I, _I, _P]),
    'mi355_nchw_to_nhwc': (_I, [_P, _P, _I, _I, _I, _I, _I, _I, _P]),
    'mi355_nchw_to_s2d': (_I, [_P, _P, _I, _I, _I, _I, _P]),
    'mi355_stem_s2d_pack': (_I, [_P, _P, _I, _I, _P]),
    'mi355_stem_s2d_unpack_grad': (_I, [_P, _P, _I, _I, _P]),
    'mi355_nhwc_to_nchw': (_I, [_P, _P, _I, _I, _I, _I, _I, _P]),
    'mi355_conv1x1_heatmap': (_I, [_P, _P, _P, _P, _I, _I, _I, _I, _I, _P]),
    'mi355_pw_c2k': (_I, [_P, _P, _P, _P, _I, _I, _I, _I, _I, _I, _P]),
    'mi355_pw_k2c': (_I, [_P, _P, _P, _P, _P, _P, _I, _I, _I, _I, _I, _I, _P]),
    'mi355_pw_k2c_stats': (_I, [_P, _P, _P, _P, _P, _P, _I, _I, _I, _I, _I, _I, _P, _Z, _P, _P]),
    'mi355_pw_wgrad_workspace': (_Z, [_I, _I, _I, _I]),
    'mi355_pw_wgrad': (_I, [_P, _P, _P, _I, _I, _I, _I, _I, _I, _I, _P, _Z, _P]),
    'mi355_hm_rowsum': (_I, [_P, _P, _I, _I, _I, _I, _P, _Z, _P]),
    'mi355_argmax2d': (_I, [_P, _P, _P, _P, _I, _I, _I, _P]),
    'mi355_softargmax': (_I, [_P, _P, _I, _I, _I, _F, _F, _P]),
    'mi355_kl_heatmap': (_I, [_P, _P, _P, _F, _P, _P, _I, _I, _F, _P]),
    'mi355_reduce_sum': (_I, [_P, _P, _I, _F, _P]),
    'mi355_scale_by_dev': (_I, [_P, _P, _P, _L, _P]),
    'mi355_scale_feature': (_I, [_P, _P, _P, _L, _I, _P]),
    'mi355_pseudo_label': (_I, [_P, _P, _I, _I, _I, _I, _P, _I, _P, _P, _I, _I, _P]),
    'mi355_bilinear_up': (_I, [_P, _P, _I, _I, _I, _I, _I, _F, _I, _P]),
    'mi355_pck_dists': (_I, [_P, _P, _P, _I, _F, _F, _P]),
    'mi355_upsample_argmax': (_I, [_P, _P, _P, _P, _I, _I, _I, _I, _I, _P]),
    'mi355_pose_metrics': (_I, [_P, _P, _P, _P, _I, _I, _I, _P, _P, _P, _P]),
    'mi355_sgd_nesterov': (_I, [_P, _P, _P, _L, _P, _F, _F, _I, _P, _P]),
    'mi355_cast_f32': (_I, [_P, _P, _L, _I, _P]),
    'mi355_ema_update': (_I, [_P, _P, _L, _P, _P]),
    'mi355_ema_update_batched': (_I, [_P, _I, _I, _P, _P]),
    'mi355_bn_fold_batched': (_I, [_P, _P, _I, _I, _P]),
    'mi355_mse_heatmap': (_I, [_P, _P, _P, _P, _P, _I, _I, _I, _P]),
    'mi355_augment_workspace': (_Z, [_I, _I]),
    'mi355_augment': (_I, [_P, ctypes.c_int64, _P, _P, _I, _I, _P, _P, _P, _P, _Z, _P]),
    'mi355_resize_normalize': (_I, [_P, ctypes.c_int64, _P, _P, _I, _I, _P, _P, _P]),
    'mi355_prof_enable': (_I, [_I]),
    'mi355_spin_us': (_I, [_L, _P]),
    'mi355_prof_read_split': (_I, [ctypes.c_double, ctypes.POINTER(ctypes.c_double)]),
    'mi355_prof_event_overhead_us': (_I, [_I, _P, ctypes.POINTER(ctypes.c_double)]),
    'mi355_prof_reset': (_I, []),
    'mi355_prof_launch_count': (_I, [ctypes.POINTER(ctypes.c_long)]),
    'mi355_prof_read_launch': (_I, [_L, ctypes.POINTER(ctypes.c_int), ctypes.POINTER(ctypes.c_double), ctypes.POINTER(ctypes.c_double),
                                    ctypes.POINTER(ctypes.c_double), ctypes.c_char_p, _I]),
    'mi355_prof_read': (_I, [ctypes.POINTER(ctypes.c_double), ctypes.POINTER(ctypes.c_long),
                             ctypes.POINTER(ctypes.c_double), ctypes.POINTER(ctypes.c_double)]),
}


def load(path=None):
    global _lib
    with _lock:
        if _lib is not None:
            return _lib
        path = path or LIB_PATH
# ... 215 lines not shown
```

domain-adaptative-hand-pose-estimation_amd/mi355/nn.py:

```python
import math
import os as _os

import torch
import torch.nn as nn

import mi355 as _rt
from . import Mi355Error, compute_dtype
from . import ops


def _same_layout(g, p):
    return all(n == 1 or a == b for n, a, b in zip(p.shape, g.stride(), p.stride()))


def grad_slot(p):
    p._mi_slot = True
    if p.grad is not None and not _same_layout(p.grad, p):
        g = torch.empty_strided(p.shape, p.stride(), dtype=p.dtype, device=p.device)
        g.copy_(p.grad)
        p.grad = g
    if p.grad is None:
        p.grad = torch.empty_strided(p.shape, p.stride(), dtype=p.dtype, device=p.device)
        p._mi_fresh = False
        return p.grad, False
# ... 56 lines not shown
        self.pin = None

    def get(self, conv, bn, dtype, deconv, s2d=False):
        pin = self.pin
        if pin is not None and pin[0] == (id(bn), dtype, bool(deconv), bool(s2d)):
            return pin[1], pin[2]
        if _FOLD_TRACE is not None:
            _FOLD_TRACE.append((self, conv, bn, dtype, bool(deconv), bool(s2d)))
        key = _fold_key(conv, bn) + (dtype, s2d)
        if key != self.key:
            with torch.no_grad():
                scale, shift = _fold_scale_shift(conv, bn)
                wm = conv.weight.detach().permute(0, 2, 3, 1)
                if getattr(conv, 'groups', 1) > 1:
                    wm = _dense_from_grouped(conv.weight, conv.groups)
                k2 = conv.kernel_size[0] * conv.kernel_size[1]
                if deconv:
                    wm = (wm * scale.view(1, 1, 1, -1)).contiguous()
                    _, self.w = ops.pack_weights(wm, conv.in_channels, k2, conv.out_channels, conv.out_channels, dtype, want_f=False, want_t=True)
                elif s2d:
                    self.w = ops.stem_s2d_pack((wm * scale.view(-1, 1, 1, 1)).contiguous(), dtype)
                else:
                    wm = (wm * scale.view(-1, 1, 1, 1)).contiguous()
                    self.w, _ = ops.pack_weights(wm, conv.out_channels, k2, conv.in_channels, conv._cin_pad(dtype), dtype, want_f=True, want_t=False)
                self.bias = shift.contiguous()
            self.key = key
        return self.w, self.bias


class _FoldedMx:

    def __init__(self):
        self.key, self.bias = None, None
        self.packs = (None, None, None, None)

    def get(self, conv, bn, deconv):
        key = _fold_key(conv, bn) + (conv.weight.device,)
        if key != self.key:
            with torch.no_grad():
                scale, shift = _fold_scale_shift(conv, bn)
                wm = conv.weight.detach().float().permute(0, 2, 3, 1)
                k2 = conv.kernel_size[0] * conv.kernel_size[1]
                if deconv:
                    wm, O, I = (wm * scale.view(1, 1, 1, -1)).contiguous(), conv.in_channels, conv.out_channels
                else:
                    wm, O, I = (wm * scale.view(-1, 1, 1, 1)).contiguous(), conv.out_channels, conv.in_channels
                self.packs = ops.pack_weights_mx(wm, O, k2, I, *self.packs)
                self.bias = shift.contiguous()
            self.key = key
        wf, sf, wt, st = self.packs
        return (wt, st, self.bias) if deconv else (wf, sf, self.bias)


def _lazy_ok(mod, residual=None):
    return (_EVAL_FOLD and mod.bn_follows and not mod.training and not torch.is_grad_enabled() and residual is None and
            getattr(mod, 'mode', 'mfma') == 'mfma' and not (_rt.fp8_convs() and _FP8_EVAL))


def _as_feature(x, dtype):
    if isinstance(x, _LazyConv):
        x = x.materialize()
    if ops.is_nhwc(x) and x.dtype == dtype:
        return x
    if not x.is_cuda:
        raise Mi355Error('mi355 layers need CUDA/HIP tensors; there is no CPU fallback')
    if x.dtype == torch.float32 and x.is_contiguous():
        return ops.to_nhwc(x, dtype)
    return x.to(dtype).contiguous(memory_format=torch.channels_last)


_LAZY_MASK = {}
_LAZY_RES = _os.environ.get('MI355_BN_LAZY_DRES', '1') == '1'
_ZERO_BN_BIAS_GRAD = _os.environ.get('MI355_ZERO_BN_BIAS_GRAD', '1') == '1'
_STEM_S2D = _os.environ.get('MI355_STEM_S2D', '1') == '1'
_BN_POOL_FUSE = _os.environ.get('MI355_BN_POOL_FUSE', '1') == '1'


def _take_lazy(g):
    if not _LAZY_MASK or g is None:
        return None
    ent = _LAZY_MASK.get(g.data_ptr())
    if ent is None or ent[0] is not g:
        return None
    del _LAZY_MASK[g.data_ptr()]
    return ent[1]


def _as_grad(dy, dtype):
    mask = _take_lazy(dy)
    if mask is not None:
        ops.apply_relu_mask(dy, mask)
    if ops.is_nhwc(dy) and dy.dtype == dtype:
        return dy
    return dy.to(dtype).contiguous(memory_format=torch.channels_last)


def _convform_param(Co, Ci, kh, kw):
    return nn.Parameter(torch.empty(Co, kh, kw, Ci).permute(0, 3, 1, 2))


class _PackedWeights:

    def __init__(self):
        self.key = None
        self.wf = self.wt = None

    def get(self, weight, O, T, I, Ipad, dtype):
        key = (_param_version(weight), dtype, Ipad)
        if key != self.key:
            if self.wf is None or self.wf.dtype != dtype or self.wf.numel() != O * T * Ipad or \
                    self.wf.device != weight.device:
                self.wf = torch.empty(O * T * Ipad, dtype=dtype, device=weight.device)
                self.wt = torch.empty(O * T * Ipad, dtype=dtype, device=weight.device)
# ... 466 lines not shown
                y, mod._last_partial = y
            ctx.desc8 = desc8
        else:
            desc, wf, wt = mod._plan(x)
            if mod._want_stats():
                y, mod._last_partial = ops.conv_dgrad_stats(desc, x, wt)
            else:
                y = ops.conv_dgrad(desc, x, wt)
        ctx.mod, ctx.desc = mod, desc
        ctx.bn_src = mod._in_bn_src; mod._in_bn_src = None
        ctx.save_for_backward(x, weight)
        return y

    @staticmethod
    def backward(ctx, dy):
        x, weight = ctx.saved_tensors
        mod, desc = ctx.mod, ctx.desc
        dy = _as_grad(dy, x.dtype)
        dx = None
        x8 = getattr(ctx, 'x8', None) if ctx.fp8 else None
        if ctx.needs_input_grad[1] and x8 is not None:
            g, acc = grad_slot(weight)
            dy8, sdy = mod._q_dy.quantize(dy)
            ops.conv_wgrad_fp8(ctx.desc8, dy8, sdy, x8[0], x8[1], g, acc, dy_fmt=ops.E4M3, x_fmt=_GRAD_FMT)
            ctx.x8 = None
        elif ctx.needs_input_grad[1]:
            g, acc = grad_slot(weight)
            if _rt.grouping_wgrads():
                _rt.group_wgrad(desc, dy, x, g, acc)
            else:
                ops.conv_wgrad(desc, dy, x, g, acc)
        if ctx.needs_input_grad[0] and ctx.mx:
            _, _, wfm, sfm, _, _ = mod._plan_mx(x)
            dym, sdym = _mx_copy(dy)
            dx = ops.conv_fwd_mx(ctx.desc8, dym, sdym, wfm, sfm)
        elif ctx.needs_input_grad[0] and ctx.fp8:
            _, _, wf8, _, sw = mod._plan_fp8(x)
            dy8, sdy = mod._q_dy.quantize(dy)
            dx = ops.conv_fwd_fp8(ctx.desc8, dy8, sdy, wf8, sw, x_fmt=_GRAD_FMT)
        elif ctx.needs_input_grad[0]:
            _, wf, _ = mod._plan(x)
            if ctx.bn_src is None:
                dx = ops.conv_fwd(desc, dy, wf)
            else:
                xb, need_y, gamma, beta, mean, invstd, relu = ctx.bn_src
                dx, part = ops.conv_fwd_bnbwd(desc, dy, wf, (xb, x if need_y else None, gamma, beta, mean, invstd, relu))
                if part is not None:
                    _BWD_PARTIALS[dx.data_ptr()] = (dx, part)
        return dx, None, None


class _BnFn(torch.autograd.Function):
    @staticmethod
    def forward(ctx, x, gamma, beta, residual, mod, relu, partial=None, lazy_ok=False, tag_dx=False):
        ctx.tag_dx = bool(tag_dx)
        q8 = None
        emit = _FP8_BN_SIDE and _rt.fp8_convs() and x.dtype == torch.bfloat16 and mod.num_features % 128 == 0
        if emit and mod._q_out.ready(x.device):
            q8 = (torch.empty_like(x, dtype=torch.uint8), mod._q_out.state)
        ctx.emit = emit
        keep_y = relu and (_MASK_FROM_Y or (residual is not None and (_FUSE_BNBWD or not _RELU_BITMASK)))
        mask = ops.bn_relu_mask(x) if (relu and residual is not None and not keep_y and
                                       (x.requires_grad or gamma.requires_grad)) else None
        _BN_GEN[0] += 1
        y, mean, invstd = ops.bn_train_fwd(x, residual, gamma, beta, mod.running_mean, mod.running_var,
                                           mod.num_batches_tracked, mod.eps, mod.momentum, relu, _rt.bn_stat_updates,
                                           partial=partial, relu_mask=mask, q8=q8)
        mod._last_q8 = q8 if q8 is not None else ('jit' if emit else None)
        ctx.relu = relu
        ctx.mask = mask
        ctx.lazy_ok = bool(lazy_ok) and _LAZY_RES and mask is not None
        ctx.mod = mod
        ctx.save_for_backward(x, y if keep_y else None, mean, invstd, gamma, beta)
        mod._last_src = (x, bool(keep_y), gamma, beta, mean, invstd, bool(relu))
        return y

    @staticmethod
    def backward(ctx, dy):
        x, y, mean, invstd, gamma, beta = ctx.saved_tensors
        lazy = _take_lazy(dy) if (not ctx.relu and ctx.mask is None and ops.is_nhwc(dy) and dy.dtype == x.dtype) else None
        dy = _as_grad(dy, x.dtype)
        dg = db = None
        acc = False
        if ctx.needs_input_grad[1]:
            dg, acc = grad_slot(gamma)
        if ctx.needs_input_grad[2]:
            db, acc_b = grad_slot(beta)
            acc = acc_b if dg is None else acc
        ent = _BWD_PARTIALS.pop(dy.data_ptr(), None)
        partial = ent[1] if (ent is not None and ent[0].shape == dy.shape and ent[0].dtype == dy.dtype) else None
        q8, stream = None, ctx.mod._q_dx
        emit = ctx.emit and _rt.fp8_convs() and ctx.needs_input_grad[0]
        if emit and stream.ready(x.device):
            q8 = (torch.empty_like(x, dtype=torch.uint8), stream.state)
        hand_on = ctx.lazy_ok and ctx.needs_input_grad[3] and lazy is None and partial is None
        if lazy is not None and partial is None:
            dx, dres = ops.bn_bwd(dy, x, None, gamma, mean, invstd, dg, db, acc, True, False, beta=beta, relu_mask=lazy, q8=q8)
        else:
            if lazy is not None:
                ops.apply_relu_mask(dy, lazy)
            dx, dres = ops.bn_bwd(dy, x, y, gamma, mean, invstd, dg, db, acc, ctx.relu, ctx.needs_input_grad[3] and not hand_on,
                                  beta=beta, partial=partial, relu_mask=ctx.mask, q8=q8)
        if hand_on:
            dres = dy
            _LAZY_MASK[dy.data_ptr()] = (dy, ctx.mask)
        if ctx.tag_dx and ctx.needs_input_grad[0]:
            _BN_DX[dx.data_ptr()] = dx
        if emit:
            if q8 is None:
                q8 = stream.quantize(dx)
            _GRAD_Q8[dx.data_ptr()] = (dx, q8[0], q8[1], ops.E5M2, dx._version)
        return (dx if ctx.needs_input_grad[0] else None), None, None, dres, None, None, None, None, None


class _BnReluPoolFn(torch.autograd.Function):

    @staticmethod
    def forward(ctx, x, gamma, beta, mod, partial):
        _BN_GEN[0] += 1
        y, arg, mean, invstd = ops.bn_relu_maxpool_fwd(x, gamma, beta, mod.running_mean, mod.running_var, mod.num_batches_tracked,
                                                       mod.eps, mod.momentum, _rt.bn_stat_updates, partial)
        ctx.in_shape = tuple(x.shape)
        ctx.save_for_backward(x, arg, mean, invstd, gamma, beta)
        return y

    @staticmethod
    def backward(ctx, dpool):
        x, arg, mean, invstd, gamma, beta = ctx.saved_tensors
        dy = ops.maxpool_bwd(_as_grad(dpool, x.dtype), arg, ctx.in_shape)
        dg = db = None
        acc = False
        if ctx.needs_input_grad[1]:
            dg, acc = grad_slot(gamma)
        if ctx.needs_input_grad[2]:
            db, acc_b = grad_slot(beta)
            acc = acc_b if dg is None else acc
        dx, _ = ops.bn_bwd(dy, x, None, gamma, mean, invstd, dg, db, acc, True, False, beta=beta)
        return (dx if ctx.needs_input_grad[0] else None), None, None, None, None


class _MaxPoolFn(torch.autograd.Function):
    @staticmethod
    def forward(ctx, x):
        y, arg = ops.maxpool_fwd(x)
        ctx.in_shape = tuple(x.shape)
        ctx.save_for_backward(arg)
        return y

    @staticmethod
    def backward(ctx, dy):
        arg, = ctx.saved_tensors
        return ops.maxpool_bwd(dy.contiguous(memory_format=torch.channels_last), arg, ctx.in_shape)


_PW_MFMA = _os.environ.get('MI355_PW_MFMA', '1') != '0'


class _CastCopy:

    def __init__(self, transposed=False):
        self.key, self.buf = None, None
        self.transposed = transposed

    def get(self, w, dtype):
        if dtype == torch.float32 and not self.transposed:
            return w.detach()
        key = (_param_version(w), dtype)
        if key != self.key:
            if self.transposed:
                w2 = w.detach().reshape(w.shape[0], -1)
                if self.buf is None or self.buf.device != w.device or self.buf.dtype != dtype:
                    self.buf = torch.empty(w2.shape[1], w2.shape[0], dtype=dtype, device=w.device)
                self.buf.copy_(w2.t())
            else:
                if self.buf is None or self.buf.device != w.device:
                    self.buf = torch.empty(w.numel(), dtype=dtype, device=w.device)
                ops.cast_f32(w.detach(), self.buf)
            self.key = key
        return self.buf


def _pw_wgrad_mfma(feat, hm, g, acc, kc_layout, K=None):
    N, C, H, W = feat.shape
    K = hm.shape[1] if K is None else K
    hm32 = ops.to_nhwc(hm, feat.dtype, 32)
    tmp = torch.empty(32 * C, dtype=torch.float32, device=feat.device)
    if kc_layout:
        ops.conv_wgrad(ops.make_desc(N, H, W, C, 32, 1, 1, 1, 0, feat.dtype), feat, hm32, tmp, False)
        src = tmp.view(32, C)[:K]
    else:
# ... 88 lines not shown
        w2, _ = hmod._packed.get(wh, hmod.out_channels, 1, K, 32, x.dtype)
        w2 = w2.view(hmod.out_channels, 32)
        want = hmod._want_stats()
        if want:
            y, part = ops.conv_fwd_cat(desc, x, wpk, bf, hm32, w2, bh, want_stats=True)
        else:
            y, part = ops.conv_fwd_cat(desc, x, wpk, bf, hm32, w2, bh), None
        ctx.mod, ctx.desc, ctx.hmod, ctx.K = fmod, desc, hmod, K
        ctx.fp8, ctx.bn_src = False, None
        ctx.fan, ctx.scale_dev = fan, scale_dev
        ctx.has_bias = bf is not None or bh is not None
        ctx.save_for_backward(x, hm32, wf, bf, wh, bh)
        hmod._last_partial = part
        hmod._last_bias_ctx = ctx if (part is not None and ctx.has_bias) else None
        return y

    @staticmethod
    def backward(ctx, dout):
        x, hm32, wf, bf, wh, bh = ctx.saved_tensors
        fmod, hmod, K = ctx.mod, ctx.hmod, ctx.K
        dout = _as_grad(dout, x.dtype)
        ent = _BN_DX.pop(dout.data_ptr(), None)
        from_bn = ent is not None and ent.shape == dout.shape and ent.dtype == dout.dtype
        zero = getattr(ctx, 'bias_grad_zero', False) and from_bn and _ZERO_BN_BIAS_GRAD
        for i, b in ((3, bf), (5, bh)):
            if b is not None and ctx.needs_input_grad[i]:
                g, acc = grad_slot(b)
                if zero:
                    if not acc:
                        _zero_grad_once(g)
                else:
                    _unmark_zeroed(g)
                    ops.colsum(dout, g, acc)
        if ctx.needs_input_grad[2]:
            _conv_wgrad(ctx, x, dout, wf)
        if ctx.needs_input_grad[4]:
            g, acc = grad_slot(wh)
            _pw_wgrad_mfma(dout, hm32, g, acc, False, K=K)
        dx = dhm = None
        if ctx.needs_input_grad[0]:
            fan = ctx.fan
            onto = fan is not None and fan.buf is not None and fan.buf.shape == x.shape and fan.buf.dtype == x.dtype
            dx = _conv_dgrad(ctx, x, dout, scale_dev=ctx.scale_dev, out=fan.buf if onto else None, accumulate=onto)
            if onto:
                dx = None
            elif fan is not None:
                fan.buf = dx
        if ctx.needs_input_grad[1]:
            _, wt = hmod._packed.get(wh, hmod.out_channels, 1, K, 32, dout.dtype)
            dhm = ops.conv1x1_heatmap(dout, wt, None, K)
        return dx, dhm, None, None, None, None, None, None, None, None


_HANDOFF_SLOTS = frozenset(('_last_bias_ctx', '_last_partial', '_in_bn_src', '_last_q8', '_last_src', '_stem_tmp'))


class _FastSlots:
    def __setattr__(self, name, value):
        if name in _HANDOFF_SLOTS:
            object.__setattr__(self, name, value)
        else:
            super().__setattr__(name, value)


class Conv2d(_FastSlots, nn.Module):

    def __init__(self, in_channels, out_channels, kernel_size, stride=1, padding=0, bias=True, groups=1):
        super().__init__()
        k = kernel_size if isinstance(kernel_size, int) else kernel_size[0]
        if groups < 1 or in_channels % groups or out_channels % groups:
            raise ValueError('in_channels and out_channels must be divisible by groups')
        self.in_channels, self.out_channels, self.groups = in_channels, out_channels, groups
        self.kernel_size, self.stride, self.padding = (k, k), (stride, stride), (padding, padding)
        self.weight = _convform_param(out_channels, in_channels // groups, k, k)
        self._packed_g = _PackedGrouped() if groups > 1 else None
        self._g_tmp = None
        self.bias = nn.Parameter(torch.empty(out_channels)) if bias else None
        self._packed = _PackedWeights()
        self._packed8, self._q_in, self._q_dy = _PackedFp8(), _Fp8Stream(ops.E4M3), _Fp8Stream(_GRAD_FMT)
        self._packedmx = _PackedMx()
        self._cast = _CastCopy()
        self._cast_t = _CastCopy(transposed=True)
        self._folded, self._folded_mx = _FoldedBn(), _FoldedMx()
        self._stem_tmp = None
        self._last_partial = None
        self._in_bn_src = None
        self.bn_follows = False
        self._s2d = _STEM_S2D and in_channels == 3 and k == 7 and stride == 2 and padding == 3
        self._packed_s2d = _PackedS2d() if self._s2d else None
        self.reset_parameters()

    def _s2d_ok(self, x):
        return self._s2d and x.shape[1] == 3 and x.shape[2] % 2 == 0 and x.shape[3] % 2 == 0

    def reset_parameters(self):
        nn.init.kaiming_uniform_(self.weight, a=math.sqrt(5))
        if self.bias is not None:
            fan_in = self.in_channels // self.groups * self.kernel_size[0] * self.kernel_size[1]
            bound = 1 / math.sqrt(fan_in) if fan_in > 0 else 0
            nn.init.uniform_(self.bias, -bound, bound)

    def extra_repr(self):
        return ('{in_channels}, {out_channels}, kernel_size={kernel_size}, stride={stride}, padding={padding}'.format(**self.__dict__) +
                (', groups=%d' % self.groups if self.groups > 1 else ''))

    @property
    def mode(self):
# ... 278 lines not shown
        if C != self.in_channels:
            raise Mi355Error('deconv expects %d input channels, got %d' % (self.in_channels, C))
        Hi, Wi = (H - 1) * s - 2 * p + k, (W - 1) * s - 2 * p + k
        _chk_convform(self.weight)
        desc = ops.make_desc(N, Hi, Wi, self.out_channels, self.in_channels, k, k, s, p, x.dtype)
        wf, wt = self._packed.get(self.weight, self.in_channels, k * k, self.out_channels, self.out_channels, x.dtype)
        return desc, wf, wt

    def forward(self, x, _lazy=True):
        if _lazy and _lazy_ok(self) and not isinstance(x, _LazyConv):
            return _LazyConv(self, x)
        x = _as_feature(x, compute_dtype())
        self._in_bn_src = _bn_src_of(x)
        return _take_partial(self, _DeconvFn.apply(x, self.weight, self))

    def forward_folded(self, x, bn, residual, relu):
        dtype = compute_dtype()
        x = _as_feature(x, dtype)
        if residual is not None:
            return ops.bn_eval_fwd(self(x, _lazy=False), _as_feature(residual, dtype), bn.weight, bn.bias, bn.running_mean, bn.running_var, bn.eps, relu)
        if self._mx_eval_ok(x):
            N, C, H, W = x.shape
            k, s, p = self.kernel_size[0], self.stride[0], self.padding[0]
            if C != self.in_channels:
                raise Mi355Error('deconv expects %d input channels, got %d' % (self.in_channels, C))
            _chk_convform(self.weight)
            desc8 = ops.make_desc_fp8(N, (H - 1) * s - 2 * p + k, (W - 1) * s - 2 * p + k, self.out_channels, self.in_channels, k, k, s, p)
            wt, st, bias = self._folded_mx.get(self, bn, True)
            x8, sx = _mx_copy(x)
            if not _mx_wants_copy(self):
                return ops.conv_dgrad_mx_act(desc8, x8, sx, wt, st, bias, relu=bool(relu))
            y, y8, sy = ops.conv_dgrad_mx_act(desc8, x8, sx, wt, st, bias, relu=bool(relu), want_copy=True)
            y._mi_mx = (y8, sy, y._version)
            return y
        desc, _, _ = self._plan(x)
        wt, bias = self._folded.get(self, bn, dtype, True)
        return ops.deconv_fwd_act(desc, x, wt, bias, relu=bool(relu))

    def _want_stats(self):
        return _FUSE_STATS and self.training and self.bn_follows


class BatchNorm2d(_FastSlots, nn.Module):
    def __init__(self, num_features, eps=1e-5, momentum=0.1):
        super().__init__()
        self.num_features, self.eps, self.momentum = num_features, eps, momentum
        self.weight = nn.Parameter(torch.ones(num_features))
        self.bias = nn.Parameter(torch.zeros(num_features))
        self.register_buffer('running_mean', torch.zeros(num_features))
        self.register_buffer('running_var', torch.ones(num_features))
        self.register_buffer('num_batches_tracked', torch.tensor(0, dtype=torch.long))
        self._q_out, self._q_dx = _Fp8Stream(ops.E4M3), _Fp8Stream(ops.E5M2)
        self._last_q8 = None

    def extra_repr(self):
        return '{num_features}, eps={eps}, momentum={momentum}'.format(num_features=self.num_features, eps=self.eps, momentum=self.momentum)

    def forward_relu_maxpool(self, x, pool):
        dtype = compute_dtype()
        tag = None if isinstance(x, _LazyConv) else getattr(x, '_mi_bn_partial', None)
        if (_BN_POOL_FUSE and self.training and tag is not None and ops.is_nhwc(x) and x.dtype == dtype and x._version == tag[1] and
                x.shape[1] == self.num_features and not (_FP8_BN_SIDE and _rt.fp8_convs()) and isinstance(pool, MaxPool2d)):
            return _BnReluPoolFn.apply(x, self.weight, self.bias, self, tag[0])
        return pool(self(x, relu=True))

    def forward(self, x, residual=None, relu=False):
        if isinstance(x, _LazyConv):
            if not self.training and not torch.is_grad_enabled() and x.conv.weight.shape[0 if isinstance(x.conv, Conv2d) else 1] == self.num_features:
                return x.conv.forward_folded(x.x, self, residual, relu)
            x = x.materialize()
        x = _as_feature(x, compute_dtype())
        if self.training:
            tag = getattr(x, '_mi_bn_partial', None)
            partial = None
            tag_dx = False
            if tag is not None:
                partial, ver, cctx = tag
                if x._version != ver:
                    raise Mi355Error('the conv output was modified in place before its BatchNorm: the statistics fused into '
                                     'the conv epilogue are stale (use an out-of-place op, or set MI355_BN_STATS_FUSE=0)')
                if x.shape[1] != self.num_features or not ops.is_nhwc(x):
                    partial = None
                elif cctx is not None:
                    cctx.bias_grad_zero = True
                    tag_dx = bool(getattr(cctx, 'has_bias', False))
            fn = getattr(residual, 'grad_fn', None) if residual is not None else None
            lazy_ok = fn is not None and type(fn).__name__ in ('_ConvSkipFnBackward', '_BnFnBackward')
            y = _BnFn.apply(x, self.weight, self.bias, residual, self, bool(relu), partial, lazy_ok, tag_dx)
            y._mi_bn_src, self._last_src = self._last_src, None
            q8, self._last_q8 = self._last_q8, None
            if q8 == 'jit':
                self._q_out.quantize(y)
            elif q8 is not None:
                y._mi_q8 = (q8[0], q8[1], ops.E4M3, y._version)
            return y
        if torch.is_grad_enabled() and (x.requires_grad or self.weight.requires_grad):
            raise Mi355Error('BatchNorm2d in eval mode is forward-only on this path (wrap it in torch.no_grad())')
        return ops.bn_eval_fwd(x, residual, self.weight, self.bias, self.running_mean, self.running_var, self.eps, relu)


class ReLU(nn.Module):

    def __init__(self, inplace=False):
        super().__init__()
        self.inplace = inplace

    def forward(self, x):
        raise Mi355Error('a bare ReLU is not built on this path: it is always fused into the BatchNorm before it')


class MaxPool2d(nn.Module):
    def __init__(self, kernel_size=3, stride=2, padding=1):
        super().__init__()
        if (kernel_size, stride, padding) != (3, 2, 1):
            raise NotImplementedError('only the 3x3 s2 p1 stem pool is built')

    def forward(self, x):
        return _MaxPoolFn.apply(_as_feature(x, compute_dtype()))


def link_conv_bn(module):
    kids = list(module.children())
    for a, b in zip(kids, kids[1:]):
        if isinstance(a, (Conv2d, ConvTranspose2d)) and isinstance(b, BatchNorm2d):
            a.bn_follows = getattr(a, 'mode', 'mfma') == 'mfma'


def link_mx_consumer(producer, consumer):
    if isinstance(producer, nn.Sequential):
        kids = list(producer)
        while kids and isinstance(kids[-1], (BatchNorm2d, ReLU)):
            kids.pop()
        producer = kids[-1] if kids else None
    if isinstance(consumer, nn.Sequential):
        consumer = consumer[0] if len(consumer) else None
    if isinstance(producer, (Conv2d, ConvTranspose2d)) and isinstance(consumer, (Conv2d, ConvTranspose2d)):
        object.__setattr__(producer, '_mx_next', consumer)


def _link_mx_runs(seq):
    kids = list(seq)
# ... 29 lines not shown
```

domain-adaptative-hand-pose-estimation_amd/mi355/ops.py:

```python
import ctypes

import torch

from . import (BnBwdSrc, ConvDesc, FP8, Mi355Error, WgradItem, call, compute_dtype, dtype_code, load, ptr, stream_ptr, workspace)


def nhwc_empty(N, C, H, W, dtype, device):
    return torch.empty((N, H, W, C), dtype=dtype, device=device).permute(0, 3, 1, 2)


def is_nhwc(x):
    return x.dim() == 4 and x.permute(0, 2, 3, 1).is_contiguous()


def _chk_room(what, t, need):
    if t is not None and t.numel() < need:
        raise Mi355Error('%s: buffer of %d elements, the launch writes %d' % (what, t.numel(), need))


def _chk_dev(*ts):
    for t in ts:
        if t is not None and not t.is_cuda:
            raise Mi355Error('mi355 ops need CUDA/HIP tensors (got a %s tensor); there is no CPU fallback' % t.device)

# ... 392 lines not shown
         ptr(dx), ptr(partial), nbytes, ctypes.byref(ns) if want_stats else None, stream_ptr())
    if want_stats:
        return dx, ((partial, ns.value) if ns.value > 0 else None)
    return dx


def conv_fwd_mx_act(desc, x8, sx, w8, sw, bias=None, residual=None, relu=False, want_copy=False, out=None, out8=None, out_scales=None):
    _chk_dev(x8, sx, w8, sw)
    nx, nw, ny = desc.N * desc.Hi * desc.Wi * desc.Ci, desc.Co * desc.kh * desc.kw * desc.Ci, desc.N * desc.Ho * desc.Wo * desc.Co
    want_copy = bool(want_copy) or out8 is not None or out_scales is not None
    for what, t, need in (('x8', x8, nx), ('sx', sx, nx // MX_BLOCK), ('w8', w8, nw), ('sw', sw, nw // MX_BLOCK),
                          ('residual', residual, ny), ('bias', bias, desc.Co), ('out', out, ny), ('out8', out8, ny),
                          ('out_scales', out_scales, ny // MX_BLOCK)):
        _chk_room('conv_fwd_mx_act ' + what, t, need)
    y = out if out is not None else nhwc_empty(desc.N, desc.Co, desc.Ho, desc.Wo, torch.bfloat16, x8.device)
    y8 = sy = None
    if want_copy:
        if desc.Co % MX_BLOCK:
            raise Mi355Error('conv_fwd_mx_act: an MX copy of the output needs a multiple of %d output channels (%d)' % (MX_BLOCK, desc.Co))
        y8 = out8 if out8 is not None else torch.empty_strided(y.shape, y.stride(), dtype=torch.uint8, device=y.device)
        sy = out_scales if out_scales is not None else torch.empty(ny // MX_BLOCK, dtype=torch.uint8, device=y.device)
        _chk_dev(y8, sy)
    call('mi355_conv_fwd_mx_act', ctypes.byref(desc), ptr(x8), ptr(sx), ptr(w8), ptr(sw), ptr(bias), ptr(residual), int(bool(relu)),
         ptr(y), ptr(y8), ptr(sy), stream_ptr())
    return (y, y8, sy) if want_copy else y


def conv_dgrad_mx_act(desc, dy8, sdy, wT8, swT, bias=None, relu=False, want_copy=False, out=None, out8=None, out_scales=None):
    _chk_dev(dy8, sdy, wT8, swT)
    ndy, nw, nx = desc.N * desc.Ho * desc.Wo * desc.Co, desc.Co * desc.kh * desc.kw * desc.Ci, desc.N * desc.Ci * desc.Hi * desc.Wi
    want_copy = bool(want_copy) or out8 is not None or out_scales is not None
    for what, t, need in (('dy8', dy8, ndy), ('sdy', sdy, ndy // MX_BLOCK), ('wT8', wT8, nw), ('swT', swT, nw // MX_BLOCK),
                          ('bias', bias, desc.Ci), ('out', out, nx), ('out8', out8, nx), ('out_scales', out_scales, nx // MX_BLOCK)):
        _chk_room('conv_dgrad_mx_act ' + what, t, need)
    dx = out if out is not None else nhwc_empty(desc.N, desc.Ci, desc.Hi, desc.Wi, torch.bfloat16, dy8.device)
    dx8 = sdx = None
    if want_copy:
        if desc.Ci % MX_BLOCK:
            raise Mi355Error('conv_dgrad_mx_act: an MX copy of the output needs a multiple of %d output channels (%d)' % (MX_BLOCK, desc.Ci))
        dx8 = out8 if out8 is not None else torch.empty_strided(dx.shape, dx.stride(), dtype=torch.uint8, device=dx.device)
        sdx = out_scales if out_scales is not None else torch.empty(nx // MX_BLOCK, dtype=torch.uint8, device=dx.device)
        _chk_dev(dx8, sdx)
    call('mi355_conv_dgrad_mx_act', ctypes.byref(desc), ptr(dy8), ptr(sdy), ptr(wT8), ptr(swT), ptr(bias), int(bool(relu)),
         ptr(dx), ptr(dx8), ptr(sdx), stream_ptr())
    return (dx, dx8, sdx) if want_copy else dx


def bn_relu_mask(x):
    per = 8 if x.dtype == torch.bfloat16 else 4
    return torch.empty(x.numel() // per, dtype=torch.uint8, device=x.device)


def bn_train_fwd(x, residual, gamma, beta, running_mean, running_var, nbt, eps, momentum, relu, stat_updates=1,
                 partial=None, relu_mask=None, q8=None):
    q8_out, q8_state = q8 if q8 is not None else (None, None)
    _chk_dev(x, gamma)
    N, C, H, W = x.shape
    rows = N * H * W
    y = nhwc_empty(N, C, H, W, x.dtype, x.device)
    mean = torch.empty(C, dtype=torch.float32, device=x.device)
    invstd = torch.empty(C, dtype=torch.float32, device=x.device)
    if partial is not None:
        buf, ns = partial
        ss = torch.empty(2 * C, dtype=torch.float32, device=x.device)
        call('mi355_bn_train_fwd_partials', ptr(x), ptr(residual), ptr(y), ptr(gamma), ptr(beta), ptr(running_mean),
             ptr(running_var), ptr(nbt), ptr(mean), ptr(invstd), rows, C, float(eps), float(momentum), int(stat_updates),
             int(relu), dtype_code(x.dtype), ptr(buf), int(ns), ptr(ss), ptr(relu_mask), ptr(q8_out), ptr(q8_state), stream_ptr())
        return y, mean, invstd
    ws = workspace(load().mi355_bn_workspace(rows, C), x.device)
    call('mi355_bn_train_fwd', ptr(x), ptr(residual), ptr(y), ptr(gamma), ptr(beta), ptr(running_mean),
         ptr(running_var), ptr(nbt), ptr(mean), ptr(invstd), rows, C, float(eps), float(momentum), int(stat_updates), int(relu),
         dtype_code(x.dtype), ptr(ws), ws.numel(), ptr(relu_mask), ptr(q8_out), ptr(q8_state), stream_ptr())
    return y, mean, invstd


def bn_relu_maxpool_fwd(x, gamma, beta, running_mean, running_var, nbt, eps, momentum, stat_updates, partial):
    _chk_dev(x, gamma)
    N, C, H, W = x.shape
    Ho, Wo = (H + 2 - 3) // 2 + 1, (W + 2 - 3) // 2 + 1
    y = nhwc_empty(N, C, Ho, Wo, x.dtype, x.device)
    arg = torch.empty((N, Ho, Wo, C), dtype=torch.uint8, device=x.device)
    mean = torch.empty(C, dtype=torch.float32, device=x.device)
    invstd = torch.empty(C, dtype=torch.float32, device=x.device)
    ss = torch.empty(2 * C, dtype=torch.float32, device=x.device)
    buf, ns = partial
    call('mi355_bn_relu_maxpool_fwd_partials', ptr(x), ptr(y), ptr(arg), ptr(gamma), ptr(beta), ptr(running_mean), ptr(running_var),
         ptr(nbt), ptr(mean), ptr(invstd), N, H, W, C, float(eps), float(momentum), int(stat_updates), dtype_code(x.dtype), ptr(buf),
         int(ns), ptr(ss), stream_ptr())
    return y, arg, mean, invstd


def bn_eval_fwd(x, residual, gamma, beta, running_mean, running_var, eps, relu):
    _chk_dev(x, gamma)
    N, C, H, W = x.shape
    y = nhwc_empty(N, C, H, W, x.dtype, x.device)
    call('mi355_bn_eval_fwd', ptr(x), ptr(residual), ptr(y), ptr(gamma), ptr(beta), ptr(running_mean),
         ptr(running_var), N * H * W, C, float(eps), int(relu), dtype_code(x.dtype), stream_ptr())
    return y


def bn_bwd(dy, x, y, gamma, mean, invstd, dgamma, dbeta, accumulate, relu, want_dres, beta=None, partial=None, relu_mask=None,
           q8=None):
    q8_out, q8_state = q8 if q8 is not None else (None, None)
    N, C, H, W = x.shape
    rows = N * H * W
    dx = nhwc_empty(N, C, H, W, x.dtype, x.device)
    dres = nhwc_empty(N, C, H, W, x.dtype, x.device) if want_dres else None
    if partial is not None:
        buf, ns = partial
        coeff = torch.empty(3 * C, dtype=torch.float32, device=x.device)
        call('mi355_bn_bwd_partials', ptr(dy), ptr(x), ptr(y), ptr(gamma), ptr(beta), ptr(mean), ptr(invstd), ptr(dx),
             ptr(dres), ptr(dgamma), ptr(dbeta), int(accumulate), rows, C, int(relu), dtype_code(x.dtype), ptr(buf), int(ns),
             ptr(coeff), ptr(relu_mask), ptr(q8_out), ptr(q8_state), stream_ptr())
        return dx, dres
    ws = workspace(load().mi355_bn_workspace(rows, C), x.device)
    call('mi355_bn_bwd', ptr(dy), ptr(x), ptr(y), ptr(gamma), ptr(beta), ptr(mean), ptr(invstd), ptr(dx), ptr(dres),
         ptr(dgamma), ptr(dbeta), int(accumulate), rows, C, int(relu), dtype_code(x.dtype), ptr(ws), ws.numel(),
         ptr(relu_mask), ptr(q8_out), ptr(q8_state), stream_ptr())
    return dx, dres


def bn_resident_timeouts():
    n = ctypes.c_uint(0)
    call('mi355_bn_resident_timeouts', ctypes.byref(n))
    return n.value


def bn_resident_reset():
    call('mi355_bn_resident_reset')


def bn_set_resident(on):
    return int(load().mi355_bn_set_resident(int(on)))


def bn_resident_set_spin_limit(limit):
    call('mi355_bn_resident_set_spin_limit', int(limit))


def bn_resident_check(where=''):
    n = bn_resident_timeouts()
    if n:
        load().mi355_bn_set_resident(0)
        bn_resident_reset()
        raise Mi355Error('%d grid-barrier give-up(s) in the one-launch BatchNorm backward%s: another kernel or process held CUs while '
                         'it ran, the gradients of those launches are NaN.  The one-launch form is now off for this process '
                         '(MI355_BN_RESIDENT=0 makes that the default); redo the affected steps.' % (n, (' (' + where + ')') if where else ''))


def maxpool_fwd(x):
    N, C, H, W = x.shape
    Ho, Wo = (H - 1) // 2 + 1, (W - 1) // 2 + 1
    y = nhwc_empty(N, C, Ho, Wo, x.dtype, x.device)
    arg = torch.empty((N, Ho, Wo, C), dtype=torch.uint8, device=x.device)
    call('mi355_maxpool_fwd', ptr(x), ptr(y), ptr(arg), N, H, W, C, dtype_code(x.dtype), stream_ptr())
    return y, arg


def maxpool_bwd(dy, arg, in_shape):
    N, C, H, W = in_shape
    dx = nhwc_empty(N, C, H, W, dy.dtype, dy.device)
    call('mi355_maxpool_bwd', ptr(dy), ptr(arg), ptr(dx), N, H, W, C, dtype_code(dy.dtype), stream_ptr())
    return dx


def conv1x1_heatmap(x, w_packed, bias, K):
    N, C, H, W = x.shape
    y = torch.empty((N, K, H, W), dtype=torch.float32, device=x.device)
    call('mi355_conv1x1_heatmap', ptr(x), ptr(w_packed), ptr(bias), ptr(y), N, H * W, C, K, dtype_code(x.dtype), stream_ptr())
    return y


# ... 350 lines not shown
```

domain-adaptative-hand-pose-estimation_amd/uda/model/resnet.py:

```python
import copy
import os
import warnings

import torch
import torch.nn as nn

from mi355.nn import Conv2d, BatchNorm2d, ReLU, MaxPool2d, FusedSequential, link_conv_bn

__all__ = ['ResNet', 'resnet18', 'resnet34', 'resnet50', 'resnet101', 'resnet152', 'resnext50_32x4d', 'resnext101_32x8d',
           'wide_resnet50_2', 'wide_resnet101_2']


class BasicBlock(nn.Module):
    expansion = 1

    def __init__(self, inplanes, planes, stride=1, downsample=None, groups=1, base_width=64):
        super().__init__()
        if groups != 1 or base_width != 64:
            raise ValueError('BasicBlock only supports groups=1 and base_width=64')
        self.conv1 = Conv2d(inplanes, planes, 3, stride, 1, bias=False)
        self.bn1 = BatchNorm2d(planes)
        self.relu = ReLU(inplace=True)
        self.conv2 = Conv2d(planes, planes, 3, 1, 1, bias=False)
        self.bn2 = BatchNorm2d(planes)
        self.downsample = downsample
        self.stride = stride
        link_conv_bn(self)

    def forward(self, x):
        out, skip = self.conv1.forward_skip(x)
        identity = skip if self.downsample is None else self.downsample(skip)
        out = self.bn1(out, relu=True)
        return self.bn2(self.conv2(out), residual=identity, relu=True)


class Bottleneck(nn.Module):
    expansion = 4

    def __init__(self, inplanes, planes, stride=1, downsample=None, groups=1, base_width=64):
        super().__init__()
        width = int(planes * (base_width / 64.)) * groups
        self.conv1 = Conv2d(inplanes, width, 1, 1, 0, bias=False)
        self.bn1 = BatchNorm2d(width)
        self.conv2 = Conv2d(width, width, 3, stride, 1, bias=False, groups=groups)
        self.bn2 = BatchNorm2d(width)
        self.conv3 = Conv2d(width, planes * 4, 1, 1, 0, bias=False)
        self.bn3 = BatchNorm2d(planes * 4)
        self.relu = ReLU(inplace=True)
        self.downsample = downsample
        self.stride = stride
        link_conv_bn(self)

    def forward(self, x):
        out, skip = self.conv1.forward_skip(x)
        identity = skip if self.downsample is None else self.downsample(skip)
        out = self.bn1(out, relu=True)
        out = self.bn2(self.conv2(out), relu=True)
        return self.bn3(self.conv3(out), residual=identity, relu=True)


class ResNet(nn.Module):

    def __init__(self, block, layers, num_classes=1000, groups=1, width_per_group=64):
        super().__init__()
        self.inplanes = 64
        self.groups, self.base_width = groups, width_per_group
        self.conv1 = Conv2d(3, 64, 7, 2, 3, bias=False)
        self.bn1 = BatchNorm2d(64)
        self.relu = ReLU(inplace=True)
        self.maxpool = MaxPool2d(3, 2, 1)
        self.layer1 = self._make_layer(block, 64, layers[0])
        self.layer2 = self._make_layer(block, 128, layers[1], stride=2)
        self.layer3 = self._make_layer(block, 256, layers[2], stride=2)
        self.layer4 = self._make_layer(block, 512, layers[3], stride=2)
        self.avgpool = nn.AdaptiveAvgPool2d((1, 1))
        self.fc = nn.Linear(512 * block.expansion, num_classes)
        for m in self.modules():
            if isinstance(m, Conv2d):
                nn.init.kaiming_normal_(m.weight, mode='fan_out', nonlinearity='relu')
            elif isinstance(m, BatchNorm2d):
                nn.init.constant_(m.weight, 1)
                nn.init.constant_(m.bias, 0)
        self._out_features = self.fc.in_features
        link_conv_bn(self)

    def _make_layer(self, block, planes, blocks, stride=1):
        downsample = None
        if stride != 1 or self.inplanes != planes * block.expansion:
            downsample = FusedSequential(Conv2d(self.inplanes, planes * block.expansion, 1, stride, 0, bias=False),
                                         BatchNorm2d(planes * block.expansion))
        layers = [block(self.inplanes, planes, stride, downsample, self.groups, self.base_width)]
        self.inplanes = planes * block.expansion
        for _ in range(1, blocks):
            layers.append(block(self.inplanes, planes, groups=self.groups, base_width=self.base_width))
        return nn.Sequential(*layers)

    def forward(self, x):
        x = self.bn1.forward_relu_maxpool(self.conv1(x), self.maxpool)
        x = self.layer1(x)
        x = self.layer2(x)
        x = self.layer3(x)
        x = self.layer4(x)
        return x

# ... 63 lines not shown
```

include/mi355pose.h:

```cpp
#ifndef MI355POSE_H
#define MI355POSE_H
#include <stddef.h>
#include <stdint.h>

#ifdef __cplusplus
extern "C" {
#endif

#define MI355_F32 0
#define MI355_BF16 1
#define MI355_FP8 2

#define MI355_OK 0
#define MI355_EINVAL (-1)
#define MI355_ELAUNCH (-2)
#define MI355_EWORKSPACE (-3)

typedef struct {
  int N, Hi, Wi, Ci;
  int Ho, Wo, Co;
  int kh, kw, stride, pad;
  int dtype;
} mi355_conv_desc;

// ... 30 lines not shown
                         float* partial, size_t partial_bytes, int* nslices, void* stream);
int mi355_fp8_quantize(const void* x, void* q, float* state, long n, int src_dtype, int fmt, int write, void* stream);
int mi355_fp8_update_scale(float* states, int n, int stride_floats, int fmt, int margin, void* stream);
int mi355_pack_weights_fp8(const float* w, void* wf, void* wt, float* state, int O, int T, int I, int margin, void* stream);
typedef struct mi355_pack8_item { const float* w; void* wf; void* wt; float* state; int O, T, I, blk0; } mi355_pack8_item;
int mi355_pack_weights_fp8_batched(const mi355_pack8_item* items_dev, int nitems, int total_blocks, void* stream);
int mi355_conv_fwd_fp8(const mi355_conv_desc* d, const void* x8, int x_fmt, const void* w8, const float* descale_x,
                       const float* descale_w, const float* bias, const void* residual, void* y, float* partial,
                       size_t partial_bytes, int* nslices, void* stream);
int mi355_conv_dgrad_fp8(const mi355_conv_desc* d, const void* dy8, int dy_fmt, const void* wT8, const float* descale_dy,
                         const float* descale_w, const float* scale_dev, int accumulate, void* dx, float* partial,
                         size_t partial_bytes, int* nslices, void* stream);
int mi355_mx_quantize(const void* x, void* q, void* scales, long rows, int C, int src_dtype, void* stream);
int mi355_pack_weights_mx(const float* w, void* wf, void* sf, void* wt, void* st, int O, int T, int I, void* stream);
typedef struct mi355_packmx_item { const float* w; void* wf; void* sf; void* wt; void* st; int O, T, I, blk0; } mi355_packmx_item;
int mi355_pack_weights_mx_batched(const mi355_packmx_item* items_dev, int nitems, int total_blocks, void* stream);
int mi355_conv_fwd_mx(const mi355_conv_desc* d, const void* x8, const void* sx, const void* w8, const void* sw, const float* bias,
                      const void* residual, void* y, float* partial, size_t partial_bytes, int* nslices, void* stream);
int mi355_conv_dgrad_mx(const mi355_conv_desc* d, const void* dy8, const void* sdy, const void* wT8, const void* swT,
                        const float* scale_dev, int accumulate, void* dx, float* partial, size_t partial_bytes, int* nslices,
                        void* stream);
int mi355_conv_fwd_mx_act(const mi355_conv_desc* d, const void* x8, const void* sx, const void* w8, const void* sw, const float* bias,
                          const void* residual, int relu, void* y, void* y8, void* sy, void* stream);
int mi355_conv_dgrad_mx_act(const mi355_conv_desc* d, const void* dy8, const void* sdy, const void* wT8, const void* swT,
                            const float* bias, int relu, void* dx, void* dx8, void* sdx, void* stream);
long mi355_set_fp8_kw3(long min_tiles);
size_t mi355_conv_wgrad_fp8_workspace(const mi355_conv_desc* d);
int mi355_conv_wgrad_fp8(const mi355_conv_desc* d, const void* x8, int x_fmt, const void* dy8, int dy_fmt, const float* descale_x,
                         const float* descale_dy, float* dw, int accumulate, void* ws, size_t ws_bytes, void* stream);
size_t mi355_conv_wgrad_workspace(const mi355_conv_desc* d);
int mi355_conv_wgrad(const mi355_conv_desc* d, const void* x, const void* dy, float* dw, int accumulate,
                     void* ws, size_t ws_bytes, void* stream);
typedef struct mi355_wgrad_item { mi355_conv_desc d; const void* x; const void* dy; float* dw; int accumulate; int pad_; } mi355_wgrad_item;
size_t mi355_conv_wgrad_grouped_workspace(const mi355_wgrad_item* items, int n);
int mi355_conv_wgrad_grouped(const mi355_wgrad_item* items, int n, void* ws, size_t ws_bytes, void* stream);
int mi355_pack_weights(const float* w, void* wf, void* wt, int O, int T, int I, int Ipad, int dtype, void* stream);
typedef struct mi355_pack_item { const float* w; void* wf; void* wt; int O, T, I, Ipad, blk0, pad_; } mi355_pack_item;
int mi355_pack_weights_batched(const mi355_pack_item* items_dev, int nitems, int total_blocks, int dtype, void* stream);
size_t mi355_colsum_workspace(long rows, int C);
int mi355_colsum(const void* dy, float* out, long rows, int C, int dtype, int accumulate, void* ws,
                 size_t ws_bytes, void* stream);

size_t mi355_bn_workspace(long rows, int C);
int mi355_bn_train_fwd(const void* x, const void* residual, void* y, const float* gamma, const float* beta,
                       float* running_mean, float* running_var, int64_t* num_batches_tracked,
                       float* save_mean, float* save_invstd, long rows, int C, float eps, float momentum,
                       int stat_updates, int relu, int dtype, void* ws, size_t ws_bytes, void* relu_mask, void* q8_out,
                       float* q8_state, void* stream);
int mi355_bn_train_fwd_partials(const void* x, const void* residual, void* y, const float* gamma, const float* beta,
                                float* running_mean, float* running_var, int64_t* num_batches_tracked,
                                float* save_mean, float* save_invstd, long rows, int C, float eps, float momentum,
                                int stat_updates, int relu, int dtype, const float* partial, int nslices,
                                float* scale_shift, void* relu_mask, void* q8_out, float* q8_state, void* stream);
int mi355_bn_eval_fwd(const void* x, const void* residual, void* y, const float* gamma, const float* beta,
                      const float* running_mean, const float* running_var, long rows, int C, float eps,
                      int relu, int dtype, void* stream);
int mi355_bn_bwd_partials(const void* dy, const void* x, const void* y, const float* gamma, const float* beta,
                          const float* save_mean, const float* save_invstd, void* dx, void* dresidual, float* dgamma,
                          float* dbeta, int accumulate, long rows, int C, int relu, int dtype, const float* partial,
                          int nslices, float* coeff, const void* relu_mask, void* q8_out, float* q8_state, void* stream);
int mi355_bn_bwd(const void* dy, const void* x, const void* y, const float* gamma, const float* beta,
                 const float* save_mean, const float* save_invstd, void* dx, void* dresidual, float* dgamma, float* dbeta,
                 int accumulate, long rows, int C, int relu, int dtype, void* ws, size_t ws_bytes,
                 const void* relu_mask, void* q8_out, float* q8_state, void* stream);
int mi355_bn_resident_timeouts(unsigned* out);
int mi355_bn_resident_reset(void);
int mi355_bn_resident_set_spin_limit(unsigned limit);
int mi355_bn_set_resident(int on);
int mi355_apply_relu_mask(void* g, const void* relu_mask, long rows, int C, int dtype, void* stream);

int mi355_bn_relu_maxpool_fwd_partials(const void* x, void* y_pool, uint8_t* argidx, const float* gamma, const float* beta,
                                       float* running_mean, float* running_var, int64_t* nbt, float* save_mean,
                                       float* save_invstd, int N, int H, int W, int C, float eps, float momentum,
                                       int stat_updates, int dtype, const float* partial, int nslices, float* scale_shift,
                                       void* stream);

int mi355_maxpool_fwd(const void* x, void* y, uint8_t* argidx, int N, int H, int W, int C, int dtype,
                      void* stream);
int mi355_maxpool_bwd(const void* dy, const uint8_t* argidx, void* dx, int N, int H, int W, int C, int dtype,
                      void* stream);

int mi355_nchw_to_nhwc(const float* x, void* y, int N, int C, int H, int W, int Cpad, int dtype, void* stream);
int mi355_nchw_to_s2d(const float* x, void* y, int N, int H, int W, int dtype, void* stream);
int mi355_stem_s2d_pack(const float* w, void* out, int Co, int dtype, void* stream);
int mi355_stem_s2d_unpack_grad(const float* gs, float* g, int Co, int accumulate, void* stream);
int mi355_nhwc_to_nchw(const void* x, float* y, int N, int C, int H, int W, int dtype, void* stream);

int mi355_conv1x1_heatmap(const void* x, const void* w, const float* bias, float* y, int N, int HW, int C, int K,
                          int dtype, void* stream);
int mi355_pw_c2k(const void* x, const float* w, const float* bias, float* y, int N, int HW, int C, int K,
                 int w_transposed, int dtype, void* stream);
int mi355_pw_k2c(const float* y, const float* w, const float* bias, const void* residual,
                 const float* scale_dev, void* out, int N, int HW, int C, int K, int w_transposed, int dtype,
                 void* stream);
int mi355_pw_k2c_stats(const float* y, const float* w, const float* bias, const void* residual, const float* scale_dev,
                       void* out, int N, int HW, int C, int K, int w_transposed, int dtype, float* partial,
                       size_t partial_bytes, int* nslices, void* stream);
size_t mi355_pw_wgrad_workspace(int N, int HW, int C, int K);
int mi355_pw_wgrad(const void* x, const float* y, float* dw, int kc_layout, int accumulate, int N, int HW,
                   int C, int K, int dtype, void* ws, size_t ws_bytes, void* stream);
int mi355_hm_rowsum(const float* y, float* out, int accumulate, int N, int K, int HW, void* ws, size_t ws_bytes,
                    void* stream);

int mi355_argmax2d(const float* hm, int32_t* idx, float* xy, float* maxval, int rows, int H, int W,
                   void* stream);
int mi355_softargmax(const float* hm, float* uv, int rows, int H, int W, float beta, float out_scale,
                     void* stream);
int mi355_kl_heatmap(const float* pred, const float* target, const float* weight, float eps,
                     float* loss_rows, float* unit_grad, int rows, int HW, float inv_count, void* stream);
int mi355_reduce_sum(const float* in, float* out, int n, float scale, void* stream);
int mi355_scale_by_dev(const float* in, const float* g_dev, float* out, long n, void* stream);
int mi355_scale_feature(const void* in, const float* g_dev, void* out, long n, int dtype, void* stream);
int mi355_pseudo_label(const float* xy, const float* patch, int radius, int div, int S, int kind,
                       const float* extra, int normalise, float* gt, float* gf, int B, int K, void* stream);
int mi355_bilinear_up(const float* in, float* out, int rows, int h, int w, int H, int W, float alpha,
                      int accumulate, void* stream);
int mi355_pck_dists(const float* pred_xy, const float* tgt_xy, float* dists, int rows, float norm_x,
                    float norm_y, void* stream);

int mi355_upsample_argmax(const float* hm, int32_t* idx, float* xy, float* maxval, int rows, int h, int w, int H, int W,
                          void* stream);
int mi355_pose_metrics(const float* pred_xy, const float* gt_xy, const float* vis, const float* thr, int T, int B, int K,
                       double* sum_err, int32_t* count, int32_t* hits, void* stream);

int mi355_sgd_nesterov(float* p, const float* g, float* buf, long n, const float* lr_dev, float momentum,
                       float wd, int nesterov, void* p_lowp, void* stream);
int mi355_cast_f32(const float* in, void* out, long n, int dtype, void* stream);
int mi355_ema_update(float* e, const float* p, long n, const float* coef_dev, void* stream);
// ... 51 lines not shown
```

Before: 4338 images/s.

## Fuse downsample BN into residual apply and maxpool-unpool into stem BN backward

```diff
diff --git a/domain-adaptative-hand-pose-estimation_amd/csrc/bn.hip b/domain-adaptative-hand-pose-estimation_amd/csrc/bn.hip
--- a/domain-adaptative-hand-pose-estimation_amd/csrc/bn.hip
+++ b/domain-adaptative-hand-pose-estimation_amd/csrc/bn.hip
@@ -172,15 +172,16 @@
   scale_shift[c] = sc; scale_shift[C + c] = b - mean * sc;
 }
 
-template <typename T, bool EVAL, bool Q8 = false>
+template <typename T, bool EVAL, bool Q8 = false, bool RSS = false>
 __global__ __launch_bounds__(256) void bn_apply_kernel(const T* __restrict__ x, const T* __restrict__ res, T* __restrict__ y,
                                                         const float* __restrict__ scale_shift, const float* __restrict__ gamma,
                                                         const float* __restrict__ beta, const float* __restrict__ rm,
                                                         const float* __restrict__ rv, float eps, long rows, int C, int TX, int relu,
                                                         unsigned char* __restrict__ mask, unsigned char* __restrict__ q8 = nullptr,
-                                                        float* __restrict__ q8_state = nullptr) {
+                                                        float* __restrict__ q8_state = nullptr, const float* __restrict__ res_ss = nullptr) {
   constexpr int CH = Chunk<T>::N;
   static_assert(!Q8 || CH == 8, "fp8 side output: bf16 activations only");
+  static_assert(!RSS || (!EVAL && !Q8), "residual normalised on load: training apply without the fp8 side output");
   const int TY = 256 / TX;
   const int tx = threadIdx.x % TX, ty = threadIdx.x / TX;
   const int chunk = blockIdx.x * TX + tx;
@@ -195,6 +196,11 @@
     else if (EVAL) { sc[e] = gamma[c] / sqrtf(rv[c] + eps); sh[e] = beta[c] - rm[c] * sc[e]; }
     else { sc[e] = scale_shift[c]; sh[e] = scale_shift[C + c]; }
   }
+  float rsc[RSS ? CH : 1], rsh[RSS ? CH : 1];
+  if constexpr (RSS) {
+#pragma unroll
+    for (int e = 0; e < CH; ++e) { rsc[e] = res_ss[chunk * CH + e]; rsh[e] = res_ss[C + chunk * CH + e]; }
+  }
   float qscale = 0.f, amax = 0.f; unsigned seen = 0;
   if constexpr (Q8) { qscale = q8_state[0]; seen = fp8_amax_seen(q8_state); }
   for (long r = (long)blockIdx.y * TY + ty; colok && r < rows; r += (long)gridDim.y * TY) {
@@ -203,6 +209,10 @@
 #pragma unroll
     for (int e = 0; e < CH; ++e) v[e] = v[e] * sc[e] + sh[e];
     if (res) { float w[CH]; Chunk<T>::load(res + off, w);
+      if constexpr (RSS) {
+#pragma unroll
+        for (int e = 0; e < CH; ++e) w[e] = (float)(T)(w[e] * rsc[e] + rsh[e]);
+      }
 #pragma unroll
       for (int e = 0; e < CH; ++e) v[e] += w[e]; }
     if (mask) {
@@ -227,14 +237,15 @@
   if constexpr (Q8) fp8_record_amax(amax, q8_state, seen);
 }
 
-template <typename T, bool XHAT, int RELU>
+template <typename T, bool XHAT, int RELU, int SRC = 0>
 __global__ __launch_bounds__(256) void bn_bwd_reduce_kernel(const T* __restrict__ dy, const T* __restrict__ x, const T* __restrict__ y,
                                                              const float* __restrict__ mean, const float* __restrict__ invstd,
                                                              const float* __restrict__ gamma, const float* __restrict__ beta,
                                                              float* __restrict__ partial, long rows, int C, int TX, int rows_per_slice,
-                                                             const unsigned char* __restrict__ mask) {
+                                                             const unsigned char* __restrict__ mask, UnpoolSrc up = UnpoolSrc()) {
   constexpr int relu = RELU;
   constexpr int CH = Chunk<T>::N;
+  static_assert(SRC == 0 || (XHAT && RELU == 2), "unpool source: the stem's mode only");
   __shared__ float sh[256 * CH * 2];
   const int cpr = C / CH;
   const int TY = 256 / TX;
@@ -243,6 +254,10 @@
   const bool colok = chunk * CH < C;
   const long r0 = (long)blockIdx.y * rows_per_slice;
   long r1 = r0 + rows_per_slice; if (r1 > rows) r1 = rows;
+  auto load_dy = [&](long row, size_t off, float (&g)[CH]) {
+    if constexpr (SRC == 1) Chunk<T>::unpack(unpool_row<T>(up, (unsigned)row, chunk, C), g);
+    else Chunk<T>::load(dy + off, g);
+  };
   float s1[CH], s2[CH], mu[CH], is[CH], sc[CH], sft[CH];
 #pragma unroll
   for (int e = 0; e < CH; ++e) { s1[e] = 0.f; s2[e] = 0.f; mu[e] = 0.f; is[e] = 0.f; sc[e] = 0.f; sft[e] = 0.f; }
@@ -277,7 +292,7 @@
     for (; r + TY < r1; r += 2 * TY) {
       const size_t off0 = (size_t)r * C + (size_t)chunk * CH, off1 = off0 + (size_t)TY * C;
       float g0[CH], v0[CH], o0[CH], g1[CH], v1[CH], o1[CH];
-      Chunk<T>::load(dy + off0, g0); Chunk<T>::load(dy + off1, g1);
+      load_dy(r, off0, g0); load_dy(r + TY, off1, g1);
       if (XHAT) { Chunk<T>::load(x + off0, v0); Chunk<T>::load(x + off1, v1); }
       if (relu == 1) { Chunk<T>::load(y + off0, o0); Chunk<T>::load(y + off1, o1); }
       unsigned m0 = 0, m1 = 0;
@@ -286,7 +301,7 @@
     }
     if (r < r1) {
       const size_t off = (size_t)r * C + (size_t)chunk * CH;
-      float g[CH], v[CH], o[CH]; Chunk<T>::load(dy + off, g);
+      float g[CH], v[CH], o[CH]; load_dy(r, off, g);
       if (XHAT) Chunk<T>::load(x + off, v);
       if (relu == 1) Chunk<T>::load(y + off, o);
       fold(g, v, o, relu == 3 ? (unsigned)mask[(size_t)r * cpr + chunk] : 0u);
@@ -334,16 +349,18 @@
   if (coeff) { coeff[c] = g * is; coeff[C + c] = s1 * inv_rows; coeff[2 * C + c] = s2 * inv_rows; }
 }
 
-template <typename T, int RELU, bool Q8 = false>
+template <typename T, int RELU, bool Q8 = false, int SRC = 0>
 __global__ __launch_bounds__(256) void bn_bwd_apply_kernel(const T* __restrict__ dy, const T* __restrict__ x, const T* __restrict__ y,
                                                             const float* __restrict__ mean, const float* __restrict__ invstd,
                                                             const float* __restrict__ coeff, const float* __restrict__ beta,
                                                             T* __restrict__ dx, T* __restrict__ dres,
                                                             long rows, int C, int TX, const unsigned char* __restrict__ mask,
-                                                            unsigned char* __restrict__ q8 = nullptr, float* __restrict__ q8_state = nullptr) {
+                                                            unsigned char* __restrict__ q8 = nullptr, float* __restrict__ q8_state = nullptr,
+                                                            UnpoolSrc up = UnpoolSrc()) {
   constexpr int CH = Chunk<T>::N;
   constexpr int relu = RELU;
   static_assert(!Q8 || CH == 8, "fp8 side output: bf16 gradients only");
+  static_assert(SRC == 0 || (RELU == 2 && !Q8), "unpool source: the stem's mode only");
   const int TY = 256 / TX;
   const int tx = threadIdx.x % TX, ty = threadIdx.x / TX;
   const int chunk = blockIdx.x * TX + tx;
@@ -359,6 +376,10 @@
   }
   float qscale = 0.f, amax = 0.f; unsigned seen = 0;
   if constexpr (Q8) { qscale = q8_state[0]; seen = fp8_amax_seen(q8_state); }
+  auto load_dy = [&](long row, size_t off, float (&g)[CH]) {
+    if constexpr (SRC == 1) Chunk<T>::unpack(unpool_row<T>(up, (unsigned)row, chunk, C), g);
+    else Chunk<T>::load(dy + off, g);
+  };
   auto finish = [&](size_t off, float (&g)[CH], float (&v)[CH], const float (&o)[CH], unsigned mb) {
     if (relu == 1) {
 #pragma unroll
@@ -387,8 +408,8 @@
   for (; r + stride < rows; r += 2 * stride) {
     const size_t off0 = (size_t)r * C + (size_t)chunk * CH, off1 = (size_t)(r + stride) * C + (size_t)chunk * CH;
     float g0[CH], v0[CH], o0[CH], g1[CH], v1[CH], o1[CH];
-    Chunk<T>::load(dy + off0, g0); Chunk<T>::load(x + off0, v0);
-    Chunk<T>::load(dy + off1, g1); Chunk<T>::load(x + off1, v1);
+    load_dy(r, off0, g0); Chunk<T>::load(x + off0, v0);
+    load_dy(r + stride, off1, g1); Chunk<T>::load(x + off1, v1);
     if (relu == 1) { Chunk<T>::load(y + off0, o0); Chunk<T>::load(y + off1, o1); }
     unsigned m0 = 0, m1 = 0;
     if (relu == 3) { m0 = mask[(size_t)r * cpr + chunk]; m1 = mask[(size_t)(r + stride) * cpr + chunk]; }
@@ -396,7 +417,7 @@
   }
   if (r < rows) {
     const size_t off = (size_t)r * C + (size_t)chunk * CH;
-    float g[CH], v[CH], o[CH]; Chunk<T>::load(dy + off, g); Chunk<T>::load(x + off, v);
+    float g[CH], v[CH], o[CH]; load_dy(r, off, g); Chunk<T>::load(x + off, v);
     if (relu == 1) Chunk<T>::load(y + off, o);
     finish(off, g, v, o, relu == 3 ? (unsigned)mask[(size_t)r * cpr + chunk] : 0u);
   }
@@ -408,6 +429,7 @@
   void* dx; void* dres; float* dgamma; float* dbeta; const unsigned char* mask;
   long rows; int C, G, R, rpb, keep, accumulate; float inv_rows;
   unsigned spin_limit;
+  UnpoolSrc up;
 };
 #define BN_RES_MAXBLK 256
 #define BN_RES_GRAN 128
@@ -430,9 +452,11 @@
 #define BN_STAMP(k) do {} while (0)
 #endif
 
-template <typename T, int RELU, int KR, int NT>
+template <typename T, int RELU, int KR, int NT, int SRC = 0>
 __global__ __launch_bounds__(NT) void bn_bwd_resident_kernel(BnResArgs p) {
   constexpr int CH = Chunk<T>::N, GC = 8 * CH, RL = NT / 8, NW = NT / 64, NL = NT / (GC * 2), RR = KR * RL;
+  constexpr int NF = 4;
+  static_assert(SRC == 0 || RELU == 2, "unpool source: the stem's mode only");
   extern __shared__ __attribute__((aligned(16))) char smem[];
   const int t = threadIdx.x, tx = t & 7, ty = t >> 3, lane = t & 63, wave = t >> 6;
   const int g = blockIdx.x % p.G, r = blockIdx.x / p.G;
@@ -462,6 +486,10 @@
     sft[e] = (RELU == 2) ? p.beta[c0 + e] - mu[e] * sc[e] : 0.f;
   }
   auto mask_of = [&](int lr) -> unsigned { return (RELU == 3) ? (unsigned)p.mask[(size_t)(row0 + lr) * cpr + chunk] : 0u; };
+  auto dy_of = [&](int lr, size_t off) -> uint4 {
+    if constexpr (SRC == 1) return unpool_row<T>(p.up, (unsigned)(row0 + lr), chunk, C);
+    else return *reinterpret_cast<const uint4*>(DY + off);
+  };
   auto fold = [&](const uint4& qxv, const uint4& qdv, unsigned mb) {
     float v[CH], gq[CH]; Chunk<T>::unpack(qxv, v); Chunk<T>::unpack(qdv, gq);
 #pragma unroll
@@ -480,25 +508,40 @@
       rx[k] = make_uint4(0, 0, 0, 0); rd[k] = make_uint4(0, 0, 0, 0); mk[k] = 0;
       if (lr < nrows) {
         const size_t off = (size_t)(row0 + lr) * C + c0;
-        rx[k] = *reinterpret_cast<const uint4*>(X + off); rd[k] = *reinterpret_cast<const uint4*>(DY + off); mk[k] = mask_of(lr);
+        rx[k] = *reinterpret_cast<const uint4*>(X + off); rd[k] = dy_of(lr, off); mk[k] = mask_of(lr);
       }
     }
 #pragma unroll
     for (int k = 0; k < KR; ++k)
       if (ty + k * RL < nrows) fold(rx[k], rd[k], mk[k]);
   }
-  for (int base = RR + ty; base < nrows; base += 4 * RL) {
-    uint4 qx[4], qd[4]; unsigned mk[4];
-#pragma unroll
-    for (int k = 0; k < 4; ++k) {
+  auto x_of = [&](int lr) -> uint4 {
+    return lr < nrows ? *reinterpret_cast<const uint4*>(X + (size_t)(row0 + lr) * C + c0) : make_uint4(0, 0, 0, 0);
+  };
+  if constexpr (SRC == 1) {
+    uint4 qx = x_of(RR + ty);
+    for (int base = RR + ty; base < nrows; base += RL) {
+      const uint4 qd = dy_of(base, 0);
+      const uint4 nx = x_of(base + RL);
+      const int li = base - RR;
+      if (li < keep) { xs[li * 8 + tx] = qx; ds[li * 8 + tx] = qd; }
+      fold(qx, qd, 0u);
+      qx = nx;
+    }
+  }
+  else
+  for (int base = RR + ty; base < nrows; base += NF * RL) {
+    uint4 qx[NF], qd[NF]; unsigned mk[NF];
+#pragma unroll
+    for (int k = 0; k < NF; ++k) {
       const int lr = base + k * RL;
       if (lr < nrows) {
         const size_t off = (size_t)(row0 + lr) * C + c0;
-        qx[k] = *reinterpret_cast<const uint4*>(X + off); qd[k] = *reinterpret_cast<const uint4*>(DY + off); mk[k] = mask_of(lr);
+        qx[k] = *reinterpret_cast<const uint4*>(X + off); qd[k] = dy_of(lr, off); mk[k] = mask_of(lr);
       }
     }
 #pragma unroll
-    for (int k = 0; k < 4; ++k) {
+    for (int k = 0; k < NF; ++k) {
       const int lr = base + k * RL, li = lr - RR;
       if (lr < nrows) {
         if (li < keep) { xs[li * 8 + tx] = qx[k]; ds[li * 8 + tx] = qd[k]; }
@@ -605,18 +648,28 @@
   }
   const int nlds = nrows - RR < keep ? nrows - RR : keep;
   for (int li = ty; li < nlds; li += RL) finish(RR + li, xs[li * 8 + tx], ds[li * 8 + tx], mask_of(RR + li));
-  for (int base = RR + keep + ty; base < nrows; base += 4 * RL) {
-    uint4 qx[4], qd[4]; unsigned mk[4];
-#pragma unroll
-    for (int k = 0; k < 4; ++k) {
+  if constexpr (SRC == 1) {
+    uint4 qx = x_of(RR + keep + ty);
+    for (int base = RR + keep + ty; base < nrows; base += RL) {
+      const uint4 qd = dy_of(base, 0);
+      const uint4 nx = x_of(base + RL);
+      finish(base, qx, qd, 0u);
+      qx = nx;
+    }
+  }
+  else
+  for (int base = RR + keep + ty; base < nrows; base += NF * RL) {
+    uint4 qx[NF], qd[NF]; unsigned mk[NF];
+#pragma unroll
+    for (int k = 0; k < NF; ++k) {
       const int lr = base + k * RL;
       if (lr < nrows) {
         const size_t off = (size_t)(row0 + lr) * C + c0;
-        qx[k] = *reinterpret_cast<const uint4*>(X + off); qd[k] = *reinterpret_cast<const uint4*>(DY + off); mk[k] = mask_of(lr);
+        qx[k] = *reinterpret_cast<const uint4*>(X + off); qd[k] = dy_of(lr, off); mk[k] = mask_of(lr);
       }
     }
 #pragma unroll
-    for (int k = 0; k < 4; ++k) {
+    for (int k = 0; k < NF; ++k) {
       const int lr = base + k * RL;
       if (lr < nrows) finish(lr, qx[k], qd[k], mk[k]);
     }
@@ -743,6 +796,36 @@
   return MI355_OK;
 }
 
+static void launch_finalize_partials(hipStream_t st, const char* lab, const float* partial, int nslices, int C, const float* gamma,
+                                     const float* beta, float* running_mean, float* running_var, int64_t* nbt, float* save_mean,
+                                     float* save_invstd, float* scale_shift, float eps, float momentum, int stat_updates) {
+  static const int wide_min = getenv("MI355_BN_WIDE_FINALIZE") ? atoi(getenv("MI355_BN_WIDE_FINALIZE")) : 512;
+  ProfScope ps(st, 0.0, 12.0 * nslices * C, 1, prof_on() ? (std::string("bn_finalize ") + lab).c_str() : nullptr);
+  if (nslices >= wide_min) hipLaunchKernelGGL(bn_finalize_wide_kernel, dim3(C), dim3(256), 0, st, partial, nslices, C, gamma, beta, running_mean, running_var, nbt, save_mean, save_invstd, scale_shift, eps, momentum, stat_updates);
+  else hipLaunchKernelGGL(bn_finalize_kernel, dim3(cdiv(C, 4)), dim3(256), 0, st, partial, nslices, C, gamma, beta, running_mean, running_var, nbt, save_mean, save_invstd, scale_shift, eps, momentum, stat_updates);
+}
+static void launch_apply_train(hipStream_t st, const char* lab, const void* x, const void* residual, const float* res_ss, void* y,
+                               const float* scale_shift, long rows, int C, int CH, int relu, int dtype, unsigned char* mk,
+                               void* q8_out, float* q8_state) {
+  BnPlan p = bn_plan(rows, C, CH);
+  dim3 ga = apply_grid(p, rows);
+  const float* nf = nullptr;
+  const float eps = 0.f;
+  const double nb = (double)rows * C * (dtype == MI355_BF16 ? 2.0 : 4.0);
+  ProfScope ps(st, 0.0, nb * (residual ? 3 : 2), 1, prof_on() ? (std::string("bn_apply ") + lab).c_str() : nullptr);
+  if (res_ss) {
+    if (dtype == MI355_BF16) hipLaunchKernelGGL((bn_apply_kernel<bf16_t, false, false, true>), ga, dim3(256), 0, st, (const bf16_t*)x, (const bf16_t*)residual, (bf16_t*)y, scale_shift, nf, nf, nf, nf, eps, rows, C, p.TX, relu, mk, (unsigned char*)nullptr, (float*)nullptr, res_ss);
+    else hipLaunchKernelGGL((bn_apply_kernel<float, false, false, true>), ga, dim3(256), 0, st, (const float*)x, (const float*)residual, (float*)y, scale_shift, nf, nf, nf, nf, eps, rows, C, p.TX, relu, mk, (unsigned char*)nullptr, (float*)nullptr, res_ss);
+  }
+  else if (q8_out) hipLaunchKernelGGL((bn_apply_kernel<bf16_t, false, true>), ga, dim3(256), 0, st, (const bf16_t*)x, (const bf16_t*)residual, (bf16_t*)y, scale_shift, nf, nf, nf, nf, eps, rows, C, p.TX, relu, mk, (unsigned char*)q8_out, q8_state);
+  else if (dtype == MI355_BF16) hipLaunchKernelGGL((bn_apply_kernel<bf16_t, false>), ga, dim3(256), 0, st, (const bf16_t*)x, (const bf16_t*)residual, (bf16_t*)y, scale_shift, nf, nf, nf, nf, eps, rows, C, p.TX, relu, mk);
+  else hipLaunchKernelGGL((bn_apply_kernel<float, false>), ga, dim3(256), 0, st, (const float*)x, (const float*)residual, (float*)y, scale_shift, nf, nf, nf, nf, eps, rows, C, p.TX, relu, mk);
+}
+static int bn_partials_check(const char* who, int stat_updates, const float* partial, int nslices, const float* scale_shift) {
+  if (stat_updates < 0 || stat_updates > 8) MI_FAIL(MI355_EINVAL, "%s: stat_updates=%d", who, stat_updates);
+  if (!partial || nslices < 1 || !scale_shift) MI_FAIL(MI355_EINVAL, "%s: partial / scale_shift missing", who);
+  return 0;
+}
 extern "C" int mi355_bn_train_fwd_partials(const void* x, const void* residual, void* y, const float* gamma, const float* beta,
                                            float* running_mean, float* running_var, int64_t* nbt, float* save_mean,
                                            float* save_invstd, long rows, int C, float eps, float momentum, int stat_updates,
@@ -750,27 +833,56 @@
                                            void* relu_mask, void* q8_out, float* q8_state, void* stream) {
   int CH; if (int e = bn_check(rows, C, dtype, &CH)) return e;
   if (int e = q8_check(q8_out, q8_state, dtype, C)) return e;
-  unsigned char* mk = reinterpret_cast<unsigned char*>(relu_mask);
-  if (stat_updates < 0 || stat_updates > 8) MI_FAIL(MI355_EINVAL, "bn_train_fwd_partials: stat_updates=%d", stat_updates);
-  if (!partial || nslices < 1 || !scale_shift) MI_FAIL(MI355_EINVAL, "bn_train_fwd_partials: partial / scale_shift missing");
+  if (int e = bn_partials_check("bn_train_fwd_partials", stat_updates, partial, nslices, scale_shift)) return e;
   hipStream_t st = as_stream(stream);
-  BnPlan p = bn_plan(rows, C, CH);
-  static const int wide_min = getenv("MI355_BN_WIDE_FINALIZE") ? atoi(getenv("MI355_BN_WIDE_FINALIZE")) : 512;
-  const double nb = (double)rows * C * (dtype == MI355_BF16 ? 2.0 : 4.0);
-  char lab[96];
+  char lab[96] = "";
   if (prof_on()) snprintf(lab, sizeof(lab), "rows%ld C%d ns%d%s%s", rows, C, nslices, relu ? " relu" : "", residual ? " +res" : "");
-  {
-    ProfScope ps(st, 0.0, 12.0 * nslices * C, 1, prof_on() ? (std::string("bn_finalize ") + lab).c_str() : nullptr);
-    if (nslices >= wide_min) hipLaunchKernelGGL(bn_finalize_wide_kernel, dim3(C), dim3(256), 0, st, partial, nslices, C, gamma, beta, running_mean, running_var, nbt, save_mean, save_invstd, scale_shift, eps, momentum, stat_updates);
-    else hipLaunchKernelGGL(bn_finalize_kernel, dim3(cdiv(C, 4)), dim3(256), 0, st, partial, nslices, C, gamma, beta, running_mean, running_var, nbt, save_mean, save_invstd, scale_shift, eps, momentum, stat_updates);
-  }
-  dim3 ga = apply_grid(p, rows);
-  const float* nf = nullptr;
-  ProfScope ps(st, 0.0, nb * (residual ? 3 : 2), 1, prof_on() ? (std::string("bn_apply ") + lab).c_str() : nullptr);
-  if (q8_out) hipLaunchKernelGGL((bn_apply_kernel<bf16_t, false, true>), ga, dim3(256), 0, st, (const bf16_t*)x, (const bf16_t*)residual, (bf16_t*)y, (const float*)scale_shift, nf, nf, nf, nf, eps, rows, C, p.TX, relu, mk, (unsigned char*)q8_out, q8_state);
-  else if (dtype == MI355_BF16) hipLaunchKernelGGL((bn_apply_kernel<bf16_t, false>), ga, dim3(256), 0, st, (const bf16_t*)x, (const bf16_t*)residual, (bf16_t*)y, (const float*)scale_shift, nf, nf, nf, nf, eps, rows, C, p.TX, relu, mk);
-  else hipLaunchKernelGGL((bn_apply_kernel<float, false>), ga, dim3(256), 0, st, (const float*)x, (const float*)residual, (float*)y, (const float*)scale_shift, nf, nf, nf, nf, eps, rows, C, p.TX, relu, mk);
+  launch_finalize_partials(st, lab, partial, nslices, C, gamma, beta, running_mean, running_var, nbt, save_mean, save_invstd, scale_shift, eps, momentum, stat_updates);
+  launch_apply_train(st, lab, x, residual, nullptr, y, scale_shift, rows, C, CH, relu, dtype, reinterpret_cast<unsigned char*>(relu_mask), q8_out, q8_state);
   MI_CHECK_LAUNCH("bn_train_fwd_partials");
+  return MI355_OK;
+}
+
+extern "C" int mi355_bn_finalize_partials(const float* gamma, const float* beta, float* running_mean, float* running_var,
+                                          int64_t* nbt, float* save_mean, float* save_invstd, long rows, int C, float eps,
+                                          float momentum, int stat_updates, const float* partial, int nslices,
+                                          float* scale_shift, void* stream) {
+  if (rows < 1 || C < 1 || !gamma || !beta || !save_mean || !save_invstd) MI_FAIL(MI355_EINVAL, "bn_finalize_partials: bad argument (rows=%ld C=%d)", rows, C);
+  if (int e = bn_partials_check("bn_finalize_partials", stat_updates, partial, nslices, scale_shift)) return e;
+  hipStream_t st = as_stream(stream);
+  char lab[96] = "";
+  if (prof_on()) snprintf(lab, sizeof(lab), "rows%ld C%d ns%d", rows, C, nslices);
+  launch_finalize_partials(st, lab, partial, nslices, C, gamma, beta, running_mean, running_var, nbt, save_mean, save_invstd, scale_shift, eps, momentum, stat_updates);
+  MI_CHECK_LAUNCH("bn_finalize_partials");
+  return MI355_OK;
+}
+
+extern "C" int mi355_bn_train_fwd_partials_res(const void* x, const void* residual, const float* res_scale_shift, void* y,
+                                               const float* gamma, const float* beta, float* running_mean, float* running_var,
+                                               int64_t* nbt, float* save_mean, float* save_invstd, long rows, int C, float eps,
+                                               float momentum, int stat_updates, int relu, int dtype, const float* partial,
+                                               int nslices, float* scale_shift, void* relu_mask, void* stream) {
+  int CH; if (int e = bn_check(rows, C, dtype, &CH)) return e;
+  if (int e = bn_partials_check("bn_train_fwd_partials_res", stat_updates, partial, nslices, scale_shift)) return e;
+  if (!residual || !res_scale_shift) MI_FAIL(MI355_EINVAL, "bn_train_fwd_partials_res: residual / res_scale_shift missing");
+  hipStream_t st = as_stream(stream);
+  char lab[96] = "";
+  if (prof_on()) snprintf(lab, sizeof(lab), "rows%ld C%d ns%d%s +bnres", rows, C, nslices, relu ? " relu" : "");
+  launch_finalize_partials(st, lab, partial, nslices, C, gamma, beta, running_mean, running_var, nbt, save_mean, save_invstd, scale_shift, eps, momentum, stat_updates);
+  launch_apply_train(st, lab, x, residual, res_scale_shift, y, scale_shift, rows, C, CH, relu, dtype, reinterpret_cast<unsigned char*>(relu_mask), nullptr, nullptr);
+  MI_CHECK_LAUNCH("bn_train_fwd_partials_res");
+  return MI355_OK;
+}
+
+extern "C" int mi355_bn_apply_fwd(const void* x, const void* residual, void* y, const float* scale_shift, long rows, int C,
+                                  int relu, int dtype, void* relu_mask, void* stream) {
+  int CH; if (int e = bn_check(rows, C, dtype, &CH)) return e;
+  if (!x || !y || !scale_shift) MI_FAIL(MI355_EINVAL, "bn_apply_fwd: null argument");
+  hipStream_t st = as_stream(stream);
+  char lab[96] = "";
+  if (prof_on()) snprintf(lab, sizeof(lab), "rows%ld C%d%s%s", rows, C, relu ? " relu" : "", residual ? " +res" : "");
+  launch_apply_train(st, lab, x, residual, nullptr, y, scale_shift, rows, C, CH, relu, dtype, reinterpret_cast<unsigned char*>(relu_mask), nullptr, nullptr);
+  MI_CHECK_LAUNCH("bn_apply_fwd");
   return MI355_OK;
 }
 
@@ -863,10 +975,10 @@
   return MI355_OK;
 }
 #define BN_RES_NOT_RESIDENT 1
-template <typename T, int RELU>
+template <typename T, int RELU, int SRC = 0>
 static int bn_resident_launch(const BnResArgs& a, size_t lds, size_t max_lds, hipStream_t st) {
   static int fits = -1;
-  auto kern = bn_bwd_resident_kernel<T, RELU, BN_RES_KR, BN_RES_NT>;
+  auto kern = bn_bwd_resident_kernel<T, RELU, BN_RES_KR, BN_RES_NT, SRC>;
   if (fits < 0) {
     if (hipFuncSetAttribute(reinterpret_cast<const void*>(kern), hipFuncAttributeMaxDynamicSharedMemorySize, (int)max_lds) != hipSuccess)
       MI_FAIL(MI355_ELAUNCH, "bn_bwd: cannot raise the dynamic LDS limit to %zu bytes", max_lds);
@@ -910,16 +1022,18 @@
 #undef MI_APP
 }
 
-extern "C" int mi355_bn_bwd(const void* dy, const void* x, const void* y, const float* gamma, const float* beta, const float* save_mean,
-                            const float* save_invstd, void* dx, void* dresidual, float* dgamma, float* dbeta, int accumulate,
-                            long rows, int C, int relu, int dtype, void* ws, size_t ws_bytes, const void* relu_mask, void* q8_out,
-                            float* q8_state, void* stream) {
+static int bn_bwd_run(const char* who, const void* dy, const void* x, const void* y, const float* gamma, const float* beta,
+                      const float* save_mean, const float* save_invstd, void* dx, void* dresidual, float* dgamma, float* dbeta,
+                      int accumulate, long rows, int C, int relu, int dtype, void* ws, size_t ws_bytes, const void* relu_mask,
+                      void* q8_out, float* q8_state, void* stream, const UnpoolSrc* up) {
   int CH; if (int e = bn_check(rows, C, dtype, &CH)) return e;
-  if (!ws || ws_bytes < mi355_bn_workspace(rows, C)) MI_FAIL(MI355_EWORKSPACE, "bn_bwd: workspace too small");
+  if (!ws || ws_bytes < mi355_bn_workspace(rows, C)) MI_FAIL(MI355_EWORKSPACE, "%s: workspace too small", who);
   const unsigned char* mk = reinterpret_cast<const unsigned char*>(relu_mask);
   if (relu) relu = mk ? 3 : (y ? 1 : 2);
-  if (relu == 2 && !beta) MI_FAIL(MI355_EINVAL, "bn_bwd: relu without y needs beta");
+  if (relu == 2 && !beta) MI_FAIL(MI355_EINVAL, "%s: relu without y needs beta", who);
   hipStream_t st = as_stream(stream);
+  const UnpoolSrc u = up ? *up : UnpoolSrc();
+  const char* src = up ? " unpool" : "";
   BnResPlan rp;
   if (relu != 1 && !q8_out && bn_resident_plan(rows, C, CH, &rp)) {
     BnResArgs a;
@@ -927,11 +1041,13 @@
     a.dgamma = dgamma; a.dbeta = dbeta; a.mask = mk; a.rows = rows; a.C = C;
     a.G = rp.G; a.R = rp.R; a.rpb = rp.rpb; a.keep = rp.keep; a.accumulate = accumulate; a.inv_rows = 1.0f / (float)rows;
     a.spin_limit = g_bn_res_spin;
+    a.up = u;
     int e;
     char lab[112];
-    if (prof_on()) snprintf(lab, sizeof(lab), "bn_bwd_res rows%ld C%d relu%d%s keep%d/%d", rows, C, relu, dresidual ? " +dres" : "", rp.keep, rp.rpb);
+    if (prof_on()) snprintf(lab, sizeof(lab), "bn_bwd_res rows%ld C%d relu%d%s%s keep%d/%d", rows, C, relu, dresidual ? " +dres" : "", src, rp.keep, rp.rpb);
     ProfScope ps(st, 0.0, (double)rows * C * (dtype == MI355_BF16 ? 2.0 : 4.0) * (dresidual ? 4 : 3), 1, prof_on() ? lab : nullptr);
-    if (dtype == MI355_BF16) e = relu == 0 ? bn_resident_launch<bf16_t, 0>(a, rp.lds, rp.max_lds, st) : relu == 2 ? bn_resident_launch<bf16_t, 2>(a, rp.lds, rp.max_lds, st) : bn_resident_launch<bf16_t, 3>(a, rp.lds, rp.max_lds, st);
+    if (up) e = dtype == MI355_BF16 ? bn_resident_launch<bf16_t, 2, 1>(a, rp.lds, rp.max_lds, st) : bn_resident_launch<float, 2, 1>(a, rp.lds, rp.max_lds, st);
+    else if (dtype == MI355_BF16) e = relu == 0 ? bn_resident_launch<bf16_t, 0>(a, rp.lds, rp.max_lds, st) : relu == 2 ? bn_resident_launch<bf16_t, 2>(a, rp.lds, rp.max_lds, st) : bn_resident_launch<bf16_t, 3>(a, rp.lds, rp.max_lds, st);
     else e = relu == 0 ? bn_resident_launch<float, 0>(a, rp.lds, rp.max_lds, st) : relu == 2 ? bn_resident_launch<float, 2>(a, rp.lds, rp.max_lds, st) : bn_resident_launch<float, 3>(a, rp.lds, rp.max_lds, st);
     if (e == MI355_OK) { MI_CHECK_LAUNCH("bn_bwd (resident)"); return MI355_OK; }
     if (e != BN_RES_NOT_RESIDENT) return e;
@@ -942,13 +1058,16 @@
   dim3 g(p.colgroups, p.nslices);
 #define MI_RED(T, R) hipLaunchKernelGGL((bn_bwd_reduce_kernel<T, true, R>), g, dim3(256), 0, st, (const T*)dy, (const T*)x, (const T*)y, save_mean, save_invstd, gamma, beta, partial, rows, C, p.TX, p.rows_per_slice, mk)
 #define MI_RED4(T) do { if (relu == 0) MI_RED(T, 0); else if (relu == 1) MI_RED(T, 1); else if (relu == 2) MI_RED(T, 2); else MI_RED(T, 3); } while (0)
+#define MI_REDU(T) hipLaunchKernelGGL((bn_bwd_reduce_kernel<T, true, 2, 1>), g, dim3(256), 0, st, (const T*)nullptr, (const T*)x, (const T*)nullptr, save_mean, save_invstd, gamma, beta, partial, rows, C, p.TX, p.rows_per_slice, mk, u)
   const double nb = (double)rows * C * (dtype == MI355_BF16 ? 2.0 : 4.0);
   char lab[96];
-  if (prof_on()) snprintf(lab, sizeof(lab), "rows%ld C%d relu%d%s", rows, C, relu, dresidual ? " +dres" : "");
+  if (prof_on()) snprintf(lab, sizeof(lab), "rows%ld C%d relu%d%s%s", rows, C, relu, dresidual ? " +dres" : "", src);
   {
     ProfScope ps(st, 0.0, nb * 2, 1, prof_on() ? (std::string("bn_bwd_reduce ") + lab).c_str() : nullptr);
-    if (dtype == MI355_BF16) MI_RED4(bf16_t); else MI_RED4(float);
-  }
+    if (up) { if (dtype == MI355_BF16) MI_REDU(bf16_t); else MI_REDU(float); }
+    else if (dtype == MI355_BF16) MI_RED4(bf16_t); else MI_RED4(float);
+  }
+#undef MI_REDU
 #undef MI_RED4
 #undef MI_RED
   {
@@ -958,9 +1077,37 @@
   dim3 ga = apply_grid(p, rows, true);
   if (int e = q8_check(q8_out, q8_state, dtype, C)) return e;
   ProfScope ps(st, 0.0, nb * (dresidual ? 4 : 3), 1, prof_on() ? (std::string("bn_bwd_apply ") + lab).c_str() : nullptr);
-  launch_bwd_apply(dtype, relu, ga, st, dy, x, y, save_mean, save_invstd, coeff, beta, dx, dresidual, rows, C, p.TX, mk, q8_out, q8_state);
-  MI_CHECK_LAUNCH("bn_bwd");
-  return MI355_OK;
+  if (up) {
+    if (dtype == MI355_BF16) hipLaunchKernelGGL((bn_bwd_apply_kernel<bf16_t, 2, false, 1>), ga, dim3(256), 0, st, (const bf16_t*)nullptr, (const bf16_t*)x, (const bf16_t*)nullptr, save_mean, save_invstd, coeff, beta, (bf16_t*)dx, (bf16_t*)nullptr, rows, C, p.TX, mk, (unsigned char*)nullptr, (float*)nullptr, u);
+    else hipLaunchKernelGGL((bn_bwd_apply_kernel<float, 2, false, 1>), ga, dim3(256), 0, st, (const float*)nullptr, (const float*)x, (const float*)nullptr, save_mean, save_invstd, coeff, beta, (float*)dx, (float*)nullptr, rows, C, p.TX, mk, (unsigned char*)nullptr, (float*)nullptr, u);
+  }
+  else launch_bwd_apply(dtype, relu, ga, st, dy, x, y, save_mean, save_invstd, coeff, beta, dx, dresidual, rows, C, p.TX, mk, q8_out, q8_state);
+  MI_CHECK_LAUNCH(who);
+  return MI355_OK;
+}
+
+extern "C" int mi355_bn_bwd(const void* dy, const void* x, const void* y, const float* gamma, const float* beta, const float* save_mean,
+                            const float* save_invstd, void* dx, void* dresidual, float* dgamma, float* dbeta, int accumulate,
+                            long rows, int C, int relu, int dtype, void* ws, size_t ws_bytes, const void* relu_mask, void* q8_out,
+                            float* q8_state, void* stream) {
+  return bn_bwd_run("bn_bwd", dy, x, y, gamma, beta, save_mean, save_invstd, dx, dresidual, dgamma, dbeta, accumulate, rows, C, relu,
+                    dtype, ws, ws_bytes, relu_mask, q8_out, q8_state, stream, nullptr);
+}
+
+extern "C" int mi355_bn_bwd_unpool(const void* dpool, const uint8_t* argidx, const void* x, const float* gamma, const float* beta,
+                                   const float* save_mean, const float* save_invstd, void* dx, float* dgamma, float* dbeta,
+                                   int accumulate, int N, int H, int W, int C, int dtype, void* ws, size_t ws_bytes, void* stream) {
+  if (!dpool || !argidx || !x || !dx || N < 1 || H < 1 || W < 1) MI_FAIL(MI355_EINVAL, "bn_bwd_unpool: bad args");
+  const long rows = (long)N * H * W;
+  int CH; if (int e = bn_check(rows, C, dtype, &CH)) return e;
+  if (rows * (C / CH) >= (1L << 31)) MI_FAIL(MI355_EINVAL, "bn_bwd_unpool: %ld chunks exceed the kernels' 32-bit row index: split the batch", rows * (C / CH));
+  const int Ho = (H + 2 - 3) / 2 + 1, Wo = (W + 2 - 3) / 2 + 1;
+  if ((long)N * Ho * Wo * C * (dtype == MI355_BF16 ? 2 : 4) >= (1L << 32)) MI_FAIL(MI355_EINVAL, "bn_bwd_unpool: the pooled gradient exceeds the kernels' 32-bit byte offsets: split the batch");
+  UnpoolSrc u;
+  u.dy = dpool; u.arg = argidx; u.H = H; u.W = W; u.Ho = Ho; u.Wo = Wo;
+  u.fw = make_fastdiv((unsigned)W); u.fh = make_fastdiv((unsigned)H);
+  return bn_bwd_run("bn_bwd_unpool", nullptr, x, nullptr, gamma, beta, save_mean, save_invstd, dx, nullptr, dgamma, dbeta, accumulate, rows, C, 1,
+                    dtype, ws, ws_bytes, nullptr, nullptr, nullptr, stream, &u);
 }
 
 extern "C" int mi355_bn_bwd_partials(const void* dy, const void* x, const void* y, const float* gamma, const float* beta,
diff --git a/domain-adaptative-hand-pose-estimation_amd/csrc/common.h b/domain-adaptative-hand-pose-estimation_amd/csrc/common.h
--- a/domain-adaptative-hand-pose-estimation_amd/csrc/common.h
+++ b/domain-adaptative-hand-pose-estimation_amd/csrc/common.h
@@ -48,6 +48,8 @@
     *reinterpret_cast<float4*>(p) = make_float4(v[0], v[1], v[2], v[3]); }
   __device__ static inline void unpack(const uint4& q, float (&v)[4]) {
     v[0] = __uint_as_float(q.x); v[1] = __uint_as_float(q.y); v[2] = __uint_as_float(q.z); v[3] = __uint_as_float(q.w); }
+  __device__ static inline uint4 pack(const float (&v)[4]) {
+    return make_uint4(__float_as_uint(v[0]), __float_as_uint(v[1]), __float_as_uint(v[2]), __float_as_uint(v[3])); }
 };
 template <> struct Chunk<bf16_t> {
   static constexpr int N = 8;
@@ -57,12 +59,13 @@
     for (int i = 0; i < 4; ++i) { v[2 * i] = __uint_as_float(w[i] << 16); v[2 * i + 1] = __uint_as_float(w[i] & 0xffff0000u); }
   }
   __device__ static inline void load(const bf16_t* p, float (&v)[8]) { unpack(*reinterpret_cast<const uint4*>(p), v); }
-  __device__ static inline void store(bf16_t* p, const float (&v)[8]) {
+  __device__ static inline uint4 pack(const float (&v)[8]) {
     union { bf16_t h[8]; uint4 q; } u;
 #pragma unroll
     for (int i = 0; i < 8; ++i) u.h[i] = (bf16_t)v[i];
-    *reinterpret_cast<uint4*>(p) = u.q;
+    return u.q;
   }
+  __device__ static inline void store(bf16_t* p, const float (&v)[8]) { *reinterpret_cast<uint4*>(p) = pack(v); }
 };
 
 template <int CH> __device__ inline void load_bytes(const uint8_t* p, unsigned (&b)[CH]) {
@@ -137,6 +140,48 @@
   return (t + ((n - t) >> 1)) >> (f.shr - 1);
 }
 
+template <typename T, typename IDX = size_t>
+__device__ __forceinline__ uint4 unpool_chunk(const T* __restrict__ dy, const uint8_t* __restrict__ arg, int n, int iy, int ix, int ch,
+                                              int Ho, int Wo, int C) {
+  constexpr int CH = Chunk<T>::N;
+  const int oy0 = iy >> 1, ox0 = ix >> 1;
+  const int khs[2] = {iy - 2 * oy0 + 1, 0}, kws[2] = {ix - 2 * ox0 + 1, 0};
+  const bool vy[2] = {oy0 < Ho, (iy & 1) && oy0 + 1 < Ho}, vx[2] = {ox0 < Wo, (ix & 1) && ox0 + 1 < Wo};
+  const int oys[2] = {oy0 < Ho ? oy0 : Ho - 1, vy[1] ? oy0 + 1 : (oy0 < Ho ? oy0 : Ho - 1)};
+  const int oxs[2] = {ox0 < Wo ? ox0 : Wo - 1, vx[1] ? ox0 + 1 : (ox0 < Wo ? ox0 : Wo - 1)};
+  uint4 dq[4]; unsigned ab[4][CH];
+#pragma unroll
+  for (int a = 0; a < 2; ++a)
+#pragma unroll
+    for (int b = 0; b < 2; ++b) {
+      const IDX o = (((IDX)n * Ho + oys[a]) * Wo + oxs[b]) * C + (IDX)ch * CH;
+      dq[a * 2 + b] = *reinterpret_cast<const uint4*>(reinterpret_cast<const char*>(dy) + (size_t)(IDX)(o * (IDX)sizeof(T)));
+      load_bytes<CH>(arg + (size_t)o, ab[a * 2 + b]);
+    }
+  float g[CH];
+#pragma unroll
+  for (int e = 0; e < CH; ++e) g[e] = 0.f;
+#pragma unroll
+  for (int a = 0; a < 2; ++a)
+#pragma unroll
+    for (int b = 0; b < 2; ++b) {
+      float d[CH]; Chunk<T>::unpack(dq[a * 2 + b], d);
+      const unsigned code = (unsigned)(khs[a] * 3 + kws[b]);
+      const bool ok = vy[a] && vx[b];
+#pragma unroll
+      for (int e = 0; e < CH; ++e) if (ok && ab[a * 2 + b][e] == code) g[e] += d[e];
+    }
+  return Chunk<T>::pack(g);
+}
+struct UnpoolSrc {
+  const void* dy; const uint8_t* arg; int H, W, Ho, Wo; FastDiv fw, fh;
+};
+template <typename T>
+__device__ __forceinline__ uint4 unpool_row(const UnpoolSrc& u, unsigned row, int ch, int C) {
+  const unsigned t = fd_div(row, u.fw), n = fd_div(t, u.fh);
+  return unpool_chunk<T, unsigned>(reinterpret_cast<const T*>(u.dy), u.arg, (int)n, (int)(t - n * (unsigned)u.H), (int)(row - t * (unsigned)u.W), ch, u.Ho, u.Wo, C);
+}
+
 struct ProfScope {
   hipStream_t s; bool on; int slot;
   ProfScope(hipStream_t st, double flops, double bytes = 0.0, int family = 0, const char* label = nullptr);
diff --git a/domain-adaptative-hand-pose-estimation_amd/csrc/pool_layout.hip b/domain-adaptative-hand-pose-estimation_amd/csrc/pool_layout.hip
--- a/domain-adaptative-hand-pose-estimation_amd/csrc/pool_layout.hip
+++ b/domain-adaptative-hand-pose-estimation_amd/csrc/pool_layout.hip
@@ -41,26 +41,7 @@
   for (unsigned id = blockIdx.x * 256u + threadIdx.x; id < total; id += gridDim.x * 256u) {
     const int ch = (int)(id % (unsigned)cpr); unsigned r = id / (unsigned)cpr;
     const int ix = (int)(r % (unsigned)W); r /= (unsigned)W; const int iy = (int)(r % (unsigned)H); const int n = (int)(r / (unsigned)H);
-    float g[CH];
-#pragma unroll
-    for (int e = 0; e < CH; ++e) g[e] = 0.f;
-    const int oy0 = iy >> 1, ox0 = ix >> 1;
-    const int khs[2] = {iy - 2 * oy0 + 1, 0}, kws[2] = {ix - 2 * ox0 + 1, 0};
-    const bool vy[2] = {oy0 < Ho, (iy & 1) && oy0 + 1 < Ho}, vx[2] = {ox0 < Wo, (ix & 1) && ox0 + 1 < Wo};
-#pragma unroll
-    for (int a = 0; a < 2; ++a)
-#pragma unroll
-      for (int b = 0; b < 2; ++b) {
-        if (vy[a] && vx[b]) {
-          const size_t o = (((size_t)n * Ho + oy0 + a) * Wo + ox0 + b) * C + (size_t)ch * CH;
-          float d[CH]; Chunk<T>::load(dy + o, d);
-          unsigned ab[CH]; load_bytes<CH>(arg + o, ab);
-          const unsigned code = (unsigned)(khs[a] * 3 + kws[b]);
-#pragma unroll
-          for (int e = 0; e < CH; ++e) if (ab[e] == code) g[e] += d[e];
-        }
-      }
-    Chunk<T>::store(dx + (((size_t)n * H + iy) * W + ix) * C + (size_t)ch * CH, g);
+    *reinterpret_cast<uint4*>(dx + (((size_t)n * H + iy) * W + ix) * C + (size_t)ch * CH) = unpool_chunk<T>(dy, arg, n, iy, ix, ch, Ho, Wo, C);
   }
 }
 
diff --git a/domain-adaptative-hand-pose-estimation_amd/mi355/__init__.py b/domain-adaptative-hand-pose-estimation_amd/mi355/__init__.py
--- a/domain-adaptative-hand-pose-estimation_amd/mi355/__init__.py
+++ b/domain-adaptative-hand-pose-estimation_amd/mi355/__init__.py
@@ -70,6 +70,9 @@
     'mi355_bn_workspace': (_Z, [_L, _I]),
     'mi355_bn_train_fwd': (_I, [_P, _P, _P, _P, _P, _P, _P, _P, _P, _P, _L, _I, _F, _F, _I, _I, _I, _P, _Z, _P, _P, _P, _P]),
     'mi355_bn_train_fwd_partials': (_I, [_P, _P, _P, _P, _P, _P, _P, _P, _P, _P, _L, _I, _F, _F, _I, _I, _I, _P, _I, _P, _P, _P, _P, _P]),
+    'mi355_bn_finalize_partials': (_I, [_P, _P, _P, _P, _P, _P, _P, _L, _I, _F, _F, _I, _P, _I, _P, _P]),
+    'mi355_bn_train_fwd_partials_res': (_I, [_P, _P, _P, _P, _P, _P, _P, _P, _P, _P, _P, _L, _I, _F, _F, _I, _I, _I, _P, _I, _P, _P, _P]),
+    'mi355_bn_apply_fwd': (_I, [_P, _P, _P, _P, _L, _I, _I, _I, _P, _P]),
     'mi355_bn_eval_fwd': (_I, [_P, _P, _P, _P, _P, _P, _P, _L, _I, _F, _I, _I, _P]),
     'mi355_bn_bwd_partials': (_I, [_P, _P, _P, _P, _P, _P, _P, _P, _P, _P, _P, _I, _L, _I, _I, _I, _P, _I, _P, _P, _P, _P, _P]),
     'mi355_bn_bwd': (_I, [_P, _P, _P, _P, _P, _P, _P, _P, _P, _P, _P, _I, _L, _I, _I, _I, _P, _Z, _P, _P, _P, _P]),
@@ -84,6 +87,7 @@
     'mi355_conv_fwd_act': (_I, [_P, _P, _P, _P, _P, _I, _P, _P]),
     'mi355_conv_dgrad_act': (_I, [_P, _P, _P, _P, _I, _P, _P]),
     'mi355_bn_relu_maxpool_fwd_partials': (_I, [_P, _P, _P, _P, _P, _P, _P, _P, _P, _P, _I, _I, _I, _I, _F, _F, _I, _I, _P, _I, _P, _P]),
+    'mi355_bn_bwd_unpool': (_I, [_P, _P, _P, _P, _P, _P, _P, _P, _P, _P, _I, _I, _I, _I, _I, _I, _P, _Z, _P]),
     'mi355_maxpool_fwd': (_I, [_P, _P, _P, _I, _I, _I, _I, _I, _P]),
     'mi355_maxpool_bwd': (_I, [_P, _P, _P, _I, _I, _I, _I, _I, _P]),
     'mi355_nchw_to_nhwc': (_I, [_P, _P, _I, _I, _I, _I, _I, _I, _P]),
diff --git a/domain-adaptative-hand-pose-estimation_amd/mi355/nn.py b/domain-adaptative-hand-pose-estimation_amd/mi355/nn.py
--- a/domain-adaptative-hand-pose-estimation_amd/mi355/nn.py
+++ b/domain-adaptative-hand-pose-estimation_amd/mi355/nn.py
@@ -132,13 +132,79 @@
         return (wt, st, self.bias) if deconv else (wf, sf, self.bias)
 
 
+class _BnApplyFn(torch.autograd.Function):
+
+    @staticmethod
+    def forward(ctx, raw, ss):
+        return ops.bn_apply(raw, ss)
+
+    @staticmethod
+    def backward(ctx, dy):
+        return dy, None
+
+
+class _LazyBn:
+    __slots__ = ('raw', 'ss', '_y')
+
+    def __init__(self, raw, ss):
+        self.raw, self.ss, self._y = raw, ss, None
+
+    def materialize(self):
+        if self._y is None:
+            self._y = _BnApplyFn.apply(self.raw, self.ss)
+        return self._y
+
+    @classmethod
+    def __torch_function__(cls, func, types, args=(), kwargs=None):
+        def mat(a):
+            if isinstance(a, _LazyBn):
+                return a.materialize()
+            if isinstance(a, (list, tuple)):
+                return type(a)(mat(b) for b in a)
+            return a
+        return func(*mat(tuple(args)), **{k: mat(v) for k, v in (kwargs or {}).items()})
+
+    @property
+    def requires_grad(self):
+        return self.raw.requires_grad
+
+    @property
+    def grad_fn(self):
+        return self.raw.grad_fn
+
+    def register_hook(self, fn):
+        return self.raw.register_hook(fn)
+
+    def __getattr__(self, name):
+        if name.startswith('_'):
+            raise AttributeError(name)
+        return getattr(self.materialize(), name)
+
+    def __add__(self, other):
+        return self.materialize() + other
+
+    def __radd__(self, other):
+        return other + self.materialize()
+
+    def __mul__(self, other):
+        return self.materialize() * other
+
+    def __rmul__(self, other):
+        return other * self.materialize()
+
+
+def link_downsample(seq):
+    if isinstance(seq, FusedSequential) and len(seq) >= 2 and isinstance(seq[-1], BatchNorm2d) and isinstance(seq[-2], Conv2d):
+        object.__setattr__(seq[-1], 'res_fold', True)
+
+
 def _lazy_ok(mod, residual=None):
     return (_EVAL_FOLD and mod.bn_follows and not mod.training and not torch.is_grad_enabled() and residual is None and
             getattr(mod, 'mode', 'mfma') == 'mfma' and not (_rt.fp8_convs() and _FP8_EVAL))
 
 
 def _as_feature(x, dtype):
-    if isinstance(x, _LazyConv):
+    if isinstance(x, (_LazyConv, _LazyBn)):
         x = x.materialize()
     if ops.is_nhwc(x) and x.dtype == dtype:
         return x
@@ -711,8 +777,16 @@
 
 class _BnFn(torch.autograd.Function):
     @staticmethod
-    def forward(ctx, x, gamma, beta, residual, mod, relu, partial=None, lazy_ok=False, tag_dx=False):
+    def forward(ctx, x, gamma, beta, residual, mod, relu, partial=None, lazy_ok=False, tag_dx=False, defer=False, res_ss=None):
         ctx.tag_dx = bool(tag_dx)
+        if defer:
+            _BN_GEN[0] += 1
+            mean, invstd, ss = ops.bn_finalize(x, gamma, beta, mod.running_mean, mod.running_var, mod.num_batches_tracked,
+                                               mod.eps, mod.momentum, _rt.bn_stat_updates, partial)
+            ctx.emit, ctx.relu, ctx.mask, ctx.lazy_ok, ctx.mod = False, False, None, False, mod
+            ctx.save_for_backward(x, None, mean, invstd, gamma, beta)
+            mod._last_q8, mod._last_src, mod._last_ss = None, None, ss
+            return x
         q8 = None
         emit = _FP8_BN_SIDE and _rt.fp8_convs() and x.dtype == torch.bfloat16 and mod.num_features % 128 == 0
         if emit and mod._q_out.ready(x.device):
@@ -724,7 +798,7 @@
         _BN_GEN[0] += 1
         y, mean, invstd = ops.bn_train_fwd(x, residual, gamma, beta, mod.running_mean, mod.running_var,
                                            mod.num_batches_tracked, mod.eps, mod.momentum, relu, _rt.bn_stat_updates,
-                                           partial=partial, relu_mask=mask, q8=q8)
+                                           partial=partial, relu_mask=mask, q8=q8, res_ss=res_ss)
         mod._last_q8 = q8 if q8 is not None else ('jit' if emit else None)
         ctx.relu = relu
         ctx.mask = mask
@@ -769,7 +843,7 @@
             if q8 is None:
                 q8 = stream.quantize(dx)
             _GRAD_Q8[dx.data_ptr()] = (dx, q8[0], q8[1], ops.E5M2, dx._version)
-        return (dx if ctx.needs_input_grad[0] else None), None, None, dres, None, None, None, None, None
+        return (dx if ctx.needs_input_grad[0] else None), None, None, dres, None, None, None, None, None, None, None
 
 
 class _BnReluPoolFn(torch.autograd.Function):
@@ -786,7 +860,7 @@
     @staticmethod
     def backward(ctx, dpool):
         x, arg, mean, invstd, gamma, beta = ctx.saved_tensors
-        dy = ops.maxpool_bwd(_as_grad(dpool, x.dtype), arg, ctx.in_shape)
+        dpool = _as_grad(dpool, x.dtype)
         dg = db = None
         acc = False
         if ctx.needs_input_grad[1]:
@@ -794,7 +868,11 @@
         if ctx.needs_input_grad[2]:
             db, acc_b = grad_slot(beta)
             acc = acc_b if dg is None else acc
-        dx, _ = ops.bn_bwd(dy, x, None, gamma, mean, invstd, dg, db, acc, True, False, beta=beta)
+        if ops.bn_bwd_unpool_ok(ctx.in_shape, x.dtype):
+            dx = ops.bn_bwd_unpool(dpool, arg, x, gamma, beta, mean, invstd, dg, db, acc)
+        else:
+            dy = ops.maxpool_bwd(dpool, arg, ctx.in_shape)
+            dx, _ = ops.bn_bwd(dy, x, None, gamma, mean, invstd, dg, db, acc, True, False, beta=beta)
         return (dx if ctx.needs_input_grad[0] else None), None, None, None, None
 
 
@@ -989,7 +1067,7 @@
         return dx, dhm, None, None, None, None, None, None, None, None
 
 
-_HANDOFF_SLOTS = frozenset(('_last_bias_ctx', '_last_partial', '_in_bn_src', '_last_q8', '_last_src', '_stem_tmp'))
+_HANDOFF_SLOTS = frozenset(('_last_bias_ctx', '_last_partial', '_in_bn_src', '_last_q8', '_last_src', '_last_ss', '_stem_tmp'))
 
 
 class _FastSlots:
@@ -1374,6 +1452,7 @@
         self.register_buffer('num_batches_tracked', torch.tensor(0, dtype=torch.long))
         self._q_out, self._q_dx = _Fp8Stream(ops.E4M3), _Fp8Stream(ops.E5M2)
         self._last_q8 = None
+        self.res_fold = False
 
     def extra_repr(self):
         return '{num_features}, eps={eps}, momentum={momentum}'.format(num_features=self.num_features, eps=self.eps, momentum=self.momentum)
@@ -1387,6 +1466,8 @@
         return pool(self(x, relu=True))
 
     def forward(self, x, residual=None, relu=False):
+        if isinstance(residual, _LazyBn) and not self.training:
+            residual = residual.materialize()
         if isinstance(x, _LazyConv):
             if not self.training and not torch.is_grad_enabled() and x.conv.weight.shape[0 if isinstance(x.conv, Conv2d) else 1] == self.num_features:
                 return x.conv.forward_folded(x.x, self, residual, relu)
@@ -1406,9 +1487,21 @@
                 elif cctx is not None:
                     cctx.bias_grad_zero = True
                     tag_dx = bool(getattr(cctx, 'has_bias', False))
+            fold = partial is not None and not _rt.fp8_convs() and not _rt.mx_convs()
+            res_ss = None
+            if isinstance(residual, _LazyBn):
+                raw = residual.raw
+                if fold and raw.shape == x.shape and raw.dtype == x.dtype and ops.is_nhwc(raw):
+                    residual, res_ss = raw, residual.ss
+                else:
+                    residual = residual.materialize()
+            defer = fold and self.res_fold and residual is None and not relu
             fn = getattr(residual, 'grad_fn', None) if residual is not None else None
             lazy_ok = fn is not None and type(fn).__name__ in ('_ConvSkipFnBackward', '_BnFnBackward')
-            y = _BnFn.apply(x, self.weight, self.bias, residual, self, bool(relu), partial, lazy_ok, tag_dx)
+            y = _BnFn.apply(x, self.weight, self.bias, residual, self, bool(relu), partial, lazy_ok, tag_dx, defer, res_ss)
+            if defer:
+                ss, self._last_ss = self._last_ss, None
+                return _LazyBn(y, ss)
             y._mi_bn_src, self._last_src = self._last_src, None
             q8, self._last_q8 = self._last_q8, None
             if q8 == 'jit':
diff --git a/domain-adaptative-hand-pose-estimation_amd/mi355/ops.py b/domain-adaptative-hand-pose-estimation_amd/mi355/ops.py
--- a/domain-adaptative-hand-pose-estimation_amd/mi355/ops.py
+++ b/domain-adaptative-hand-pose-estimation_amd/mi355/ops.py
@@ -468,7 +468,7 @@
 
 
 def bn_train_fwd(x, residual, gamma, beta, running_mean, running_var, nbt, eps, momentum, relu, stat_updates=1,
-                 partial=None, relu_mask=None, q8=None):
+                 partial=None, relu_mask=None, q8=None, res_ss=None):
     q8_out, q8_state = q8 if q8 is not None else (None, None)
     _chk_dev(x, gamma)
     N, C, H, W = x.shape
@@ -476,6 +476,16 @@
     y = nhwc_empty(N, C, H, W, x.dtype, x.device)
     mean = torch.empty(C, dtype=torch.float32, device=x.device)
     invstd = torch.empty(C, dtype=torch.float32, device=x.device)
+    if res_ss is not None:
+        if partial is None or q8 is not None or residual is None or residual.shape != x.shape or residual.dtype != x.dtype:
+            raise Mi355Error('bn_train_fwd: res_ss needs conv-fused statistics, a residual shaped like x and no fp8 side output')
+        _chk_dev(residual, res_ss)
+        buf, ns = partial
+        ss = torch.empty(2 * C, dtype=torch.float32, device=x.device)
+        call('mi355_bn_train_fwd_partials_res', ptr(x), ptr(residual), ptr(res_ss), ptr(y), ptr(gamma), ptr(beta),
+             ptr(running_mean), ptr(running_var), ptr(nbt), ptr(mean), ptr(invstd), rows, C, float(eps), float(momentum),
+             int(stat_updates), int(relu), dtype_code(x.dtype), ptr(buf), int(ns), ptr(ss), ptr(relu_mask), stream_ptr())
+        return y, mean, invstd
     if partial is not None:
         buf, ns = partial
         ss = torch.empty(2 * C, dtype=torch.float32, device=x.device)
@@ -488,6 +498,27 @@
          ptr(running_var), ptr(nbt), ptr(mean), ptr(invstd), rows, C, float(eps), float(momentum), int(stat_updates), int(relu),
          dtype_code(x.dtype), ptr(ws), ws.numel(), ptr(relu_mask), ptr(q8_out), ptr(q8_state), stream_ptr())
     return y, mean, invstd
+
+
+def bn_finalize(x, gamma, beta, running_mean, running_var, nbt, eps, momentum, stat_updates, partial):
+    _chk_dev(x, gamma)
+    N, C, H, W = x.shape
+    mean = torch.empty(C, dtype=torch.float32, device=x.device)
+    invstd = torch.empty(C, dtype=torch.float32, device=x.device)
+    ss = torch.empty(2 * C, dtype=torch.float32, device=x.device)
+    buf, ns = partial
+    call('mi355_bn_finalize_partials', ptr(gamma), ptr(beta), ptr(running_mean), ptr(running_var), ptr(nbt), ptr(mean), ptr(invstd),
+         N * H * W, C, float(eps), float(momentum), int(stat_updates), ptr(buf), int(ns), ptr(ss), stream_ptr())
+    return mean, invstd, ss
+
+
+def bn_apply(x, scale_shift, residual=None, relu=False, relu_mask=None):
+    _chk_dev(x, scale_shift)
+    N, C, H, W = x.shape
+    y = nhwc_empty(N, C, H, W, x.dtype, x.device)
+    call('mi355_bn_apply_fwd', ptr(x), ptr(residual), ptr(y), ptr(scale_shift), N * H * W, C, int(relu), dtype_code(x.dtype),
+         ptr(relu_mask), stream_ptr())
+    return y
 
 
 def bn_relu_maxpool_fwd(x, gamma, beta, running_mean, running_var, nbt, eps, momentum, stat_updates, partial):
@@ -534,6 +565,26 @@
          ptr(dgamma), ptr(dbeta), int(accumulate), rows, C, int(relu), dtype_code(x.dtype), ptr(ws), ws.numel(),
          ptr(relu_mask), ptr(q8_out), ptr(q8_state), stream_ptr())
     return dx, dres
+
+
+def bn_bwd_unpool_ok(in_shape, dtype):
+    N, C, H, W = in_shape
+    per = 8 if dtype == torch.bfloat16 else 4
+    Ho, Wo = (H + 2 - 3) // 2 + 1, (W + 2 - 3) // 2 + 1
+    return C % per == 0 and N * H * W * (C // per) < (1 << 31) and N * Ho * Wo * C * (16 // per) < (1 << 32)
+
+
+def bn_bwd_unpool(dpool, arg, x, gamma, beta, mean, invstd, dgamma, dbeta, accumulate):
+    _chk_dev(dpool, arg, x, gamma)
+    N, C, H, W = x.shape
+    Ho, Wo = (H + 2 - 3) // 2 + 1, (W + 2 - 3) // 2 + 1
+    if tuple(dpool.shape) != (N, C, Ho, Wo) or dpool.dtype != x.dtype or not is_nhwc(dpool) or arg.numel() != dpool.numel():
+        raise Mi355Error('bn_bwd_unpool: the pooled gradient / window bytes do not belong to a %s map' % (tuple(x.shape),))
+    dx = nhwc_empty(N, C, H, W, x.dtype, x.device)
+    ws = workspace(load().mi355_bn_workspace(N * H * W, C), x.device)
+    call('mi355_bn_bwd_unpool', ptr(dpool), ptr(arg), ptr(x), ptr(gamma), ptr(beta), ptr(mean), ptr(invstd), ptr(dx), ptr(dgamma),
+         ptr(dbeta), int(accumulate), N, H, W, C, dtype_code(x.dtype), ptr(ws), ws.numel(), stream_ptr())
+    return dx
 
 
 def bn_resident_timeouts():
diff --git a/domain-adaptative-hand-pose-estimation_amd/uda/model/resnet.py b/domain-adaptative-hand-pose-estimation_amd/uda/model/resnet.py
--- a/domain-adaptative-hand-pose-estimation_amd/uda/model/resnet.py
+++ b/domain-adaptative-hand-pose-estimation_amd/uda/model/resnet.py
@@ -5,7 +5,7 @@
 import torch
 import torch.nn as nn
 
-from mi355.nn import Conv2d, BatchNorm2d, ReLU, MaxPool2d, FusedSequential, link_conv_bn
+from mi355.nn import Conv2d, BatchNorm2d, ReLU, MaxPool2d, FusedSequential, link_conv_bn, link_downsample
 
 __all__ = ['ResNet', 'resnet18', 'resnet34', 'resnet50', 'resnet101', 'resnet152', 'resnext50_32x4d', 'resnext101_32x8d',
            'wide_resnet50_2', 'wide_resnet101_2']
@@ -26,6 +26,7 @@
         self.downsample = downsample
         self.stride = stride
         link_conv_bn(self)
+        link_downsample(downsample)
 
     def forward(self, x):
         out, skip = self.conv1.forward_skip(x)
@@ -50,6 +51,7 @@
         self.downsample = downsample
         self.stride = stride
         link_conv_bn(self)
+        link_downsample(downsample)
 
     def forward(self, x):
         out, skip = self.conv1.forward_skip(x)
diff --git a/include/mi355pose.h b/include/mi355pose.h
--- a/include/mi355pose.h
+++ b/include/mi355pose.h
@@ -106,6 +106,17 @@
                                 float* save_mean, float* save_invstd, long rows, int C, float eps, float momentum,
                                 int stat_updates, int relu, int dtype, const float* partial, int nslices,
                                 float* scale_shift, void* relu_mask, void* q8_out, float* q8_state, void* stream);
+int mi355_bn_finalize_partials(const float* gamma, const float* beta, float* running_mean, float* running_var,
+                               int64_t* num_batches_tracked, float* save_mean, float* save_invstd, long rows, int C,
+                               float eps, float momentum, int stat_updates, const float* partial, int nslices,
+                               float* scale_shift, void* stream);
+int mi355_bn_train_fwd_partials_res(const void* x, const void* residual, const float* res_scale_shift, void* y,
+                                    const float* gamma, const float* beta, float* running_mean, float* running_var,
+                                    int64_t* num_batches_tracked, float* save_mean, float* save_invstd, long rows, int C,
+                                    float eps, float momentum, int stat_updates, int relu, int dtype, const float* partial,
+                                    int nslices, float* scale_shift, void* relu_mask, void* stream);
+int mi355_bn_apply_fwd(const void* x, const void* residual, void* y, const float* scale_shift, long rows, int C, int relu,
+                       int dtype, void* relu_mask, void* stream);
 int mi355_bn_eval_fwd(const void* x, const void* residual, void* y, const float* gamma, const float* beta,
                       const float* running_mean, const float* running_var, long rows, int C, float eps,
                       int relu, int dtype, void* stream);
@@ -128,6 +139,9 @@
                                        float* save_invstd, int N, int H, int W, int C, float eps, float momentum,
                                        int stat_updates, int dtype, const float* partial, int nslices, float* scale_shift,
                                        void* stream);
+int mi355_bn_bwd_unpool(const void* dpool, const uint8_t* argidx, const void* x, const float* gamma, const float* beta,
+                        const float* save_mean, const float* save_invstd, void* dx, float* dgamma, float* dbeta,
+                        int accumulate, int N, int H, int W, int C, int dtype, void* ws, size_t ws_bytes, void* stream);
 
 int mi355_maxpool_fwd(const void* x, void* y, uint8_t* argidx, int N, int H, int W, int C, int dtype,
                       void* stream);
```

Measured after the change: 4349 images/s (median of 6 runs). No clear change (+0.3%).
